# pananananas/MVD

Hardware: AMD Instinct MI355X
Metric: UNet forward-passes/sec @512x512 SD2.1+MV adapter (higher is better)
Workload: dtype bf16; 1 GPU; cfg4: configs[3]/[4]: 8 objects x 4 target views per GPU (32 pairs), camera FiLM + cross-view adapter; pairs_per_gpu=32, global_pairs=32, latent=64x64x4, image=512x512, forward=cold, hip_graph=False, q2_statistics=replica-local, parallelism=dp1 (pairs sharded by object), weights=synthetic seeded, SD2.1 shapes (865.9M UNet x2 + 99.2M adapter + 19.1M camera), encoder_weights=distinct

## Files before the change

### include/mvd_hip.h

```cpp
#ifndef MVD_HIP_H
#define MVD_HIP_H
#include <stddef.h>
#include <stdint.h>

#ifdef __cplusplus
extern "C" {
#endif

#define MVD_MAX_LEVELS 4

typedef struct {
  int in_channels;
  int out_channels;
  int num_levels;
  int block_out_channels[MVD_MAX_LEVELS];
  int num_heads[MVD_MAX_LEVELS];
  int layers_per_block;
  int cross_attention_dim;
  int norm_num_groups;
  float norm_eps;
  int cam_output_dim;
  int cam_hidden_dim;
  int simple_cam_encoder;
  float cam_modulation_strength;
} mvd_config_t;

typedef struct mvd_engine mvd_engine_t;

const char* mvd_last_error(void);

int mvd_engine_create(const mvd_config_t* cfg, mvd_engine_t** out);
int mvd_engine_destroy(mvd_engine_t* e);

int mvd_engine_set_weight(mvd_engine_t* e, int set, const char* slot, const void* ptr, int64_t numel, int dtype);
int mvd_engine_clear_weights(mvd_engine_t* e, int set);

int64_t mvd_engine_workspace_bytes(mvd_engine_t* e, int batch, int height, int width, int text_len, int ref_batch);
int64_t mvd_engine_refcache_bytes(mvd_engine_t* e, int ref_batch, int height, int width, int keep_features);
int mvd_engine_bind_workspace(mvd_engine_t* e, void* ws, int64_t ws_bytes, void* refcache, int64_t refcache_bytes);

enum {
  MVD_USE_CAMERA = 1,
  MVD_USE_IMAGE = 2,
  MVD_REUSE_REF = 4,
  MVD_KEEP_FEATURES = 8
};

typedef struct {
  int batch;
  int height, width;
  int text_len;
  const float* sample;
  const float* timesteps;
  const float* text;
  const float* source_camera;
  const float* target_camera;
  int cam_rows;
  int cam_batch;
  const float* fourier_proj;
  const float* source_latents;
  const float* encoder_text;
  int ref_batch;
  int flags;
  float* out;
} mvd_forward_args_t;

int mvd_unet_forward(mvd_engine_t* e, const mvd_forward_args_t* args, void* stream);

int64_t mvd_engine_reference_pixels(mvd_engine_t* e, int height, int width);
int mvd_engine_reference_encode(mvd_engine_t* e, const mvd_forward_args_t* args, float* local_stats, void* stream);
int mvd_engine_reference_finish(mvd_engine_t* e, const float* mean_k, void* stream);

int mvd_engine_set_graph(mvd_engine_t* e, int enable);

int mvd_engine_share_encoder_weights(mvd_engine_t* e, int enable);

int mvd_engine_set_profiling(mvd_engine_t* e, int enable);
int mvd_engine_profile_summary(mvd_engine_t* e, int cap, int* cls, int* launches, double* ms, double* flops, double* bytes);
int mvd_engine_profile_shapes(mvd_engine_t* e, char* buf_host, int cap);

int mvd_engine_num_features(mvd_engine_t* e);
int mvd_engine_feature_shape(mvd_engine_t* e, int idx, int* channels, int* height, int* width);
int mvd_engine_get_feature(mvd_engine_t* e, int idx, float* out_nchw, void* stream);
int mvd_engine_encode_cameras(mvd_engine_t* e, const float* source_camera, const float* target_camera, int cam_rows,
                              int batch, const float* fourier_proj, float* out_emb, void* stream);
int mvd_engine_apply_modulation(mvd_engine_t* e, const char* name, const float* emb, int batch, const float* x_nchw,
                                int channels, int hw, float* out_nchw, void* stream);
int mvd_engine_get_camera_embedding(mvd_engine_t* e, float* out, void* stream);

int mvd_op_linear(const void* a, const void* a2, int k1, int k2, const void* w, const float* bias, const float* rowvec,
                  int ld_rowvec, int rows_per_batch, const void* res, float alpha, int geglu, void* out, int out_f32,
                  int m, int n, int force_cfg, int splitk, float* splitk_ws ,
                  void* stream);
int mvd_op_ln_linear(const void* x, int k, const void* w_folded, const float* c1, const float* c2, float eps, int geglu,
                     void* out, int m, int n, void* stream);
int mvd_op_linear_xs(const void* x, int ldx, const void* w_packed, int m, int k, int units, int geglu, int ln, float ln_eps,
                     const void* res, int ldres, void* out, int ldo, int csplit, void* stream);
int mvd_op_conv3x3_ws(const void* x, int batch, int h, int w, int c, const void* w_packed, const float* bias, const float* rowvec,
                      int ld_rowvec, const void* res, const void* sc, const void* sc2, int sc_c1, int sc_c2, void* out, int n,
                      int variant, void* stream);
int mvd_op_conv3x3(const void* x, int batch, int in_h, int in_w, int cin, int stride, int upsample, int asym_pad, const void* w,
                   const float* bias, const float* rowvec, int ld_rowvec, const void* res, const void* sc, const void* sc2,
                   int sc_c1, int sc_c2, void* out, int cout, int force_cfg, int splitk, float* splitk_ws, void* stream);
int mvd_op_attention(const void* q, const void* k, const void* v, void* o, int batch, int heads, int nq, int nk, int ldq,
                     int ldk, int ldv, int ldo, float scale, void* stream);
int64_t mvd_op_attention_split_ws_bytes(int batch, int heads, int nq, int nsplit);
int mvd_op_attention_split(const void* q, const void* k, const void* v, void* o, int batch, int heads, int nq, int nk, int ldq,
                           int ldk, int ldv, int ldo, int nsplit, void* ws, void* stream);
int mvd_op_groupnorm(const void* x0, const void* x1, int c0, int c1, int batch, int hw, int groups, float eps,
                     const float* gamma, const float* beta, int silu, void* y, float* ws, void* stream);
int mvd_op_layernorm(const void* x, int rows, int c, float eps, const float* gamma, const float* beta, void* y,
                     void* stream);
int mvd_op_refnorm(const void* x, int batch, int hw, int c, void* y, void* stream);
int mvd_op_film(const void* x, int batch, int hw, int c, const float* scale, const float* shift, void* y, void* stream);
int mvd_op_conv_in(const void* x, int batch, int h, int w, int cin, const float* wt, const float* bias, int cout, void* y,
                   void* stream);
int mvd_op_conv_out(const void* x, int batch, int h, int w, int c, const void* wt, const float* bias, int cout, float* y,
                    void* stream);
int mvd_op_nchw_to_nhwc(const float* x, int batch, int c, int hw, const float* scale, const float* shift, void* y,
                        void* stream);
int mvd_op_nhwc_to_nchw(const void* x, int batch, int hw, int c, float* y, void* stream);
int mvd_op_f32_to_bf16(const float* x, int64_t n, void* y, void* stream);
int mvd_op_skinny_linear(const float* x, int ldx, int batch, int k, const void* w, int wbf16, const float* bias, int n, int act_in,
                         float* y, int ldy, void* stream);
int mvd_gemm_num_configs(void);
int mvd_debug_last_gemm_plan(int* out);
int mvd_debug_last_attention_plan(int* out);
int mvd_debug_last_gemm_nowait(void);
int mvd_debug_pick_splitk(int m, int n, int k, int geglu);
int mvd_debug_pick_splitk_conv(int m, int n, int k);
int mvd_gemm_sm_num_tiles(void);
int mvd_debug_set_attention_nw(int nw_log2);
int mvd_debug_set_flags(int flags);

int mvd_op_ddpm_step(const float* model_out, const float* sample, const float* noise, float c0, float c1, float c2,
                     float c3, float sigma, float* out, int64_t n, void* stream);
int mvd_op_cfg_combine(const float* uncond_cond, float guidance_scale, float* out, int64_t n_half, void* stream);
int mvd_op_sampler_step(const float* model_out, int guided, float guidance_scale, const float* sample, const float* x0_prev,
                        const float* noise, float a0, float a1, float p, float q, float r, float sigma, float* out,
                        float* x0_out, int64_t n, void* stream);

typedef struct {
  int in_channels;
  int latent_channels;
  int num_levels;
  int block_out_channels[MVD_MAX_LEVELS];
  int layers_per_block;
  int norm_num_groups;
  float norm_eps;
} mvd_vae_config_t;
typedef struct mvd_vae mvd_vae_t;
int mvd_vae_create(const mvd_vae_config_t* cfg, mvd_vae_t** out);
int mvd_vae_destroy(mvd_vae_t* v);
int mvd_vae_set_weight(mvd_vae_t* v, const char* slot, const void* ptr, int64_t numel, int dtype);
int64_t mvd_vae_workspace_bytes(mvd_vae_t* v, int batch, int height, int width, int decode);
int mvd_vae_bind_workspace(mvd_vae_t* v, void* ws, int64_t ws_bytes);
int mvd_vae_encode(mvd_vae_t* v, const float* image_nchw, int batch, int height, int width, float* moments, void* stream);
int mvd_vae_decode(mvd_vae_t* v, const float* latents_nchw, int batch, int height, int width, float* image, void* stream);
int64_t mvd_vae_mid_attention_workspace_bytes(mvd_vae_t* v, int decoder, int batch, int height, int width);
int mvd_vae_mid_attention(mvd_vae_t* v, int decoder, const void* x_nhwc_bf16, int batch, int height, int width, void* out_nhwc_bf16,
                          void* stream);
int mvd_op_softmax_rows(const float* s, int rows, int n, void* p_bf16, void* stream);
int mvd_op_gaussian_sample(const float* moments, const float* noise, int batch, int channels, int hw, float scale, float* out,
                           void* stream);

#ifdef __cplusplus
}
#endif
#endif
```

### mvd_amd/_lib.py

```python
from __future__ import annotations

import ctypes as C
import os

HERE = os.path.dirname(os.path.abspath(__file__))
LIB_PATH = os.environ.get("MVD_HIP_LIB") or os.path.join(HERE, "libmvd_hip.so")

MVD_MAX_LEVELS = 4
MVD_USE_CAMERA, MVD_USE_IMAGE, MVD_REUSE_REF, MVD_KEEP_FEATURES = 1, 2, 4, 8


class MvdError(RuntimeError):
    pass


class mvd_config_t(C.Structure):
    _fields_ = [
        ("in_channels", C.c_int), ("out_channels", C.c_int), ("num_levels", C.c_int),
        ("block_out_channels", C.c_int * MVD_MAX_LEVELS), ("num_heads", C.c_int * MVD_MAX_LEVELS),
        ("layers_per_block", C.c_int), ("cross_attention_dim", C.c_int), ("norm_num_groups", C.c_int),
        ("norm_eps", C.c_float), ("cam_output_dim", C.c_int), ("cam_hidden_dim", C.c_int),
        ("simple_cam_encoder", C.c_int), ("cam_modulation_strength", C.c_float),
    ]


class mvd_vae_config_t(C.Structure):
    _fields_ = [
        ("in_channels", C.c_int), ("latent_channels", C.c_int), ("num_levels", C.c_int),
        ("block_out_channels", C.c_int * MVD_MAX_LEVELS), ("layers_per_block", C.c_int), ("norm_num_groups", C.c_int),
        ("norm_eps", C.c_float),
    ]


class mvd_forward_args_t(C.Structure):
    _fields_ = [
        ("batch", C.c_int), ("height", C.c_int), ("width", C.c_int), ("text_len", C.c_int),
        ("sample", C.c_void_p), ("timesteps", C.c_void_p), ("text", C.c_void_p),
        ("source_camera", C.c_void_p), ("target_camera", C.c_void_p), ("cam_rows", C.c_int), ("cam_batch", C.c_int),
        ("fourier_proj", C.c_void_p), ("source_latents", C.c_void_p), ("encoder_text", C.c_void_p),
        ("ref_batch", C.c_int), ("flags", C.c_int), ("out", C.c_void_p),
    ]


_SIGS = {
    "mvd_last_error": (C.c_char_p, []),
    "mvd_engine_create": (C.c_int, [C.POINTER(mvd_config_t), C.POINTER(C.c_void_p)]),
    "mvd_engine_destroy": (C.c_int, [C.c_void_p]),
    "mvd_engine_set_weight": (C.c_int, [C.c_void_p, C.c_int, C.c_char_p, C.c_void_p, C.c_int64, C.c_int]),
    "mvd_engine_clear_weights": (C.c_int, [C.c_void_p, C.c_int]),
    "mvd_engine_workspace_bytes": (C.c_int64, [C.c_void_p, C.c_int, C.c_int, C.c_int, C.c_int, C.c_int]),
    "mvd_engine_refcache_bytes": (C.c_int64, [C.c_void_p, C.c_int, C.c_int, C.c_int, C.c_int]),
    "mvd_engine_bind_workspace": (C.c_int, [C.c_void_p, C.c_void_p, C.c_int64, C.c_void_p, C.c_int64]),
    "mvd_unet_forward": (C.c_int, [C.c_void_p, C.POINTER(mvd_forward_args_t), C.c_void_p]),
    "mvd_engine_set_profiling": (C.c_int, [C.c_void_p, C.c_int]),
    "mvd_engine_profile_summary": (C.c_int, [C.c_void_p, C.c_int, C.POINTER(C.c_int), C.POINTER(C.c_int),
                                             C.POINTER(C.c_double), C.POINTER(C.c_double), C.POINTER(C.c_double)]),
    "mvd_engine_profile_shapes": (C.c_int, [C.c_void_p, C.c_char_p, C.c_int]),
    "mvd_engine_set_graph": (C.c_int, [C.c_void_p, C.c_int]),
    "mvd_engine_reference_pixels": (C.c_int64, [C.c_void_p, C.c_int, C.c_int]),
    "mvd_engine_reference_encode": (C.c_int, [C.c_void_p, C.POINTER(mvd_forward_args_t), C.c_void_p, C.c_void_p]),
    "mvd_engine_reference_finish": (C.c_int, [C.c_void_p, C.c_void_p, C.c_void_p]),
    "mvd_engine_share_encoder_weights": (C.c_int, [C.c_void_p, C.c_int]),
    "mvd_engine_num_features": (C.c_int, [C.c_void_p]),
    "mvd_engine_feature_shape": (C.c_int, [C.c_void_p, C.c_int, C.POINTER(C.c_int), C.POINTER(C.c_int), C.POINTER(C.c_int)]),
    "mvd_engine_get_feature": (C.c_int, [C.c_void_p, C.c_int, C.c_void_p, C.c_void_p]),
    "mvd_engine_encode_cameras": (C.c_int, [C.c_void_p, C.c_void_p, C.c_void_p, C.c_int, C.c_int, C.c_void_p, C.c_void_p, C.c_void_p]),
    "mvd_engine_apply_modulation": (C.c_int, [C.c_void_p, C.c_char_p, C.c_void_p, C.c_int, C.c_void_p, C.c_int, C.c_int, C.c_void_p, C.c_void_p]),
    "mvd_engine_get_camera_embedding": (C.c_int, [C.c_void_p, C.c_void_p, C.c_void_p]),
    "mvd_op_linear": (C.c_int, [C.c_void_p, C.c_void_p, C.c_int, C.c_int, C.c_void_p, C.c_void_p, C.c_void_p, C.c_int,
                                C.c_int, C.c_void_p, C.c_float, C.c_int, C.c_void_p, C.c_int, C.c_int, C.c_int, C.c_int,
                                C.c_int, C.c_void_p, C.c_void_p]),
    "mvd_op_ln_linear": (C.c_int, [C.c_void_p, C.c_int, C.c_void_p, C.c_void_p, C.c_void_p, C.c_float, C.c_int, C.c_void_p,
                                   C.c_int, C.c_int, C.c_void_p]),
    "mvd_op_linear_xs": (C.c_int, [C.c_void_p, C.c_int, C.c_void_p, C.c_int, C.c_int, C.c_int, C.c_int, C.c_int, C.c_float,
                                   C.c_void_p, C.c_int, C.c_void_p, C.c_int, C.c_int, C.c_void_p]),
    "mvd_op_conv3x3_ws": (C.c_int, [C.c_void_p, C.c_int, C.c_int, C.c_int, C.c_int, C.c_void_p, C.c_void_p, C.c_void_p, C.c_int,
                                    C.c_void_p, C.c_void_p, C.c_void_p, C.c_int, C.c_int, C.c_void_p, C.c_int, C.c_int, C.c_void_p]),
    "mvd_op_conv3x3": (C.c_int, [C.c_void_p, C.c_int, C.c_int, C.c_int, C.c_int, C.c_int, C.c_int, C.c_int, C.c_void_p, C.c_void_p,
                                 C.c_void_p, C.c_int, C.c_void_p, C.c_void_p, C.c_void_p, C.c_int, C.c_int, C.c_void_p,
                                 C.c_int, C.c_int, C.c_int, C.c_void_p, C.c_void_p]),
    "mvd_op_attention": (C.c_int, [C.c_void_p, C.c_void_p, C.c_void_p, C.c_void_p, C.c_int, C.c_int, C.c_int, C.c_int,
                                   C.c_int, C.c_int, C.c_int, C.c_int, C.c_float, C.c_void_p]),
    "mvd_op_attention_split_ws_bytes": (C.c_int64, [C.c_int, C.c_int, C.c_int, C.c_int]),
    "mvd_op_attention_split": (C.c_int, [C.c_void_p, C.c_void_p, C.c_void_p, C.c_void_p, C.c_int, C.c_int, C.c_int, C.c_int, C.c_int,
                                         C.c_int, C.c_int, C.c_int, C.c_int, C.c_void_p, C.c_void_p]),
    "mvd_op_groupnorm": (C.c_int, [C.c_void_p, C.c_void_p, C.c_int, C.c_int, C.c_int, C.c_int, C.c_int, C.c_float,
                                   C.c_void_p, C.c_void_p, C.c_int, C.c_void_p, C.c_void_p, C.c_void_p]),
    "mvd_op_layernorm": (C.c_int, [C.c_void_p, C.c_int, C.c_int, C.c_float, C.c_void_p, C.c_void_p, C.c_void_p, C.c_void_p]),
    "mvd_op_refnorm": (C.c_int, [C.c_void_p, C.c_int, C.c_int, C.c_int, C.c_void_p, C.c_void_p]),
    "mvd_op_film": (C.c_int, [C.c_void_p, C.c_int, C.c_int, C.c_int, C.c_void_p, C.c_void_p, C.c_void_p, C.c_void_p]),
    "mvd_op_conv_in": (C.c_int, [C.c_void_p, C.c_int, C.c_int, C.c_int, C.c_int, C.c_void_p, C.c_void_p, C.c_int, C.c_void_p, C.c_void_p]),
    "mvd_op_conv_out": (C.c_int, [C.c_void_p, C.c_int, C.c_int, C.c_int, C.c_int, C.c_void_p, C.c_void_p, C.c_int, C.c_void_p, C.c_void_p]),
    "mvd_op_nchw_to_nhwc": (C.c_int, [C.c_void_p, C.c_int, C.c_int, C.c_int, C.c_void_p, C.c_void_p, C.c_void_p, C.c_void_p]),
    "mvd_op_nhwc_to_nchw": (C.c_int, [C.c_void_p, C.c_int, C.c_int, C.c_int, C.c_void_p, C.c_void_p]),
    "mvd_op_f32_to_bf16": (C.c_int, [C.c_void_p, C.c_int64, C.c_void_p, C.c_void_p]),
    "mvd_op_skinny_linear": (C.c_int, [C.c_void_p, C.c_int, C.c_int, C.c_int, C.c_void_p, C.c_int, C.c_void_p, C.c_int, C.c_int,
                                        C.c_void_p, C.c_int, C.c_void_p]),
    "mvd_gemm_num_configs": (C.c_int, []),
    "mvd_debug_last_gemm_plan": (C.c_int, [C.POINTER(C.c_int)]),
    "mvd_debug_last_gemm_nowait": (C.c_int, []),
    "mvd_debug_last_attention_plan": (C.c_int, [C.POINTER(C.c_int)]),
    "mvd_debug_pick_splitk": (C.c_int, [C.c_int, C.c_int, C.c_int, C.c_int]),
    "mvd_debug_pick_splitk_conv": (C.c_int, [C.c_int, C.c_int, C.c_int]),
    "mvd_gemm_sm_num_tiles": (C.c_int, []),
    "mvd_debug_set_attention_nw": (C.c_int, [C.c_int]),
    "mvd_debug_set_flags": (C.c_int, [C.c_int]),
    "mvd_op_ddpm_step": (C.c_int, [C.c_void_p, C.c_void_p, C.c_void_p, C.c_float, C.c_float, C.c_float, C.c_float,
                                   C.c_float, C.c_void_p, C.c_int64, C.c_void_p]),
    "mvd_op_cfg_combine": (C.c_int, [C.c_void_p, C.c_float, C.c_void_p, C.c_int64, C.c_void_p]),
    "mvd_op_sampler_step": (C.c_int, [C.c_void_p, C.c_int, C.c_float, C.c_void_p, C.c_void_p, C.c_void_p, C.c_float, C.c_float,
                                      C.c_float, C.c_float, C.c_float, C.c_float, C.c_void_p, C.c_void_p, C.c_int64, C.c_void_p]),
    "mvd_vae_create": (C.c_int, [C.POINTER(mvd_vae_config_t), C.POINTER(C.c_void_p)]),
    "mvd_vae_destroy": (C.c_int, [C.c_void_p]),
    "mvd_vae_set_weight": (C.c_int, [C.c_void_p, C.c_char_p, C.c_void_p, C.c_int64, C.c_int]),
    "mvd_vae_workspace_bytes": (C.c_int64, [C.c_void_p, C.c_int, C.c_int, C.c_int, C.c_int]),
    "mvd_vae_bind_workspace": (C.c_int, [C.c_void_p, C.c_void_p, C.c_int64]),
    "mvd_vae_encode": (C.c_int, [C.c_void_p, C.c_void_p, C.c_int, C.c_int, C.c_int, C.c_void_p, C.c_void_p]),
    "mvd_vae_decode": (C.c_int, [C.c_void_p, C.c_void_p, C.c_int, C.c_int, C.c_int, C.c_void_p, C.c_void_p]),
    "mvd_vae_mid_attention_workspace_bytes": (C.c_int64, [C.c_void_p, C.c_int, C.c_int, C.c_int, C.c_int]),
    "mvd_vae_mid_attention": (C.c_int, [C.c_void_p, C.c_int, C.c_void_p, C.c_int, C.c_int, C.c_int, C.c_void_p, C.c_void_p]),
    "mvd_op_softmax_rows": (C.c_int, [C.c_void_p, C.c_int, C.c_int, C.c_void_p, C.c_void_p]),
    "mvd_op_gaussian_sample": (C.c_int, [C.c_void_p, C.c_void_p, C.c_int, C.c_int, C.c_int, C.c_float, C.c_void_p, C.c_void_p]),
}

EXPORTED_SYMBOLS = tuple(_SIGS)

_lib = None


def lib() -> C.CDLL:
    global _lib
    if _lib is None:
        if not os.path.exists(LIB_PATH):
            raise MvdError(
                f"{LIB_PATH} not found: build the HIP extension first "
                "(python -c 'import __graft_entry__ as g; g.build()' or python mvd_amd/_build.py)")
        import torch
        l = C.CDLL(LIB_PATH)
        for name, (res, args) in _SIGS.items():
            fn = getattr(l, name)
            fn.restype = res
            fn.argtypes = args
        _lib = l
    return _lib


def last_error() -> str:
    return lib().mvd_last_error().decode()


def check(rc: int, what: str = "") -> int:
    if rc is None or rc < 0 or (rc != 0 and what.startswith("!")):
        raise MvdError(f"{what.lstrip('!')}: rc={rc}: {last_error()}")
    return rc


def call(name: str, *args):
    rc = getattr(lib(), name)(*args)
    if rc != 0:
        raise MvdError(f"{name} failed (rc={rc}): {last_error()}")
    return rc
```

### mvd_amd/csrc/engine.hip

```cpp
#include <math.h>
#include <stdio.h>
#include <stdlib.h>
#include <string.h>

#include <string>
#include <unordered_map>
#include <vector>

#include "../../include/mvd_hip.h"
#include "kernels.h"

int mvd_launch_silu_to_bf16(const float* x, int64_t n, bf16_t* y, hipStream_t s);

static int g_debug_flags = 0;
extern "C" int mvd_debug_set_flags(int flags) { g_debug_flags = flags; return 0; }
int mvd_debug_flags() { return g_debug_flags; }

namespace {

struct Weight { const void* p; int64_t numel; int dtype; };

struct Arena {
  char* base = nullptr;
  size_t cap = 0, off = 0, high = 0;
// ... 69 lines not shown
  int dual_late_from = MVD_ENV_INT("MVD_DUAL_LATE_FROM", 99);
  bool graph_on = false;
  std::vector<GraphEntry> graphs;
  std::vector<std::string> graph_seen;
  void drop_graphs() {
    for (auto& ge : graphs) { (void)hipGraphExecDestroy(ge.x); (void)hipGraphDestroy(ge.g); }
    graphs.clear(); graph_seen.clear();
  }
  ~mvd_engine() {
    drop_graphs();
    for (hipEvent_t ev : ev_pool) (void)hipEventDestroy(ev);
    for (hipEvent_t ev : feat_ev) if (ev) (void)hipEventDestroy(ev);
    if (fork_ev) (void)hipEventDestroy(fork_ev);
    if (join_ev) (void)hipEventDestroy(join_ev);
    if (side) (void)hipStreamDestroy(side);
  }
  std::vector<int> temb_off;
  int temb_total = 0;
  std::vector<int> tkv_off;
  int tkv_total = 0;
  bool prof = false;
  bool prof_overlap = false;
  struct ProfRec { int cls; double flops; double bytes; hipEvent_t e0, e1; int M, N, K, tag; };
  int prof_M = 0, prof_N = 0, prof_K = 0, prof_tag = 0;
  std::vector<ProfRec> prof_recs;
  std::vector<hipEvent_t> ev_pool; size_t ev_used = 0;
  hipEvent_t get_event() {
    if (ev_used == ev_pool.size()) { hipEvent_t ev = nullptr; (void)hipEventCreate(&ev); ev_pool.push_back(ev); }
    return ev_pool[ev_used++];
  }
};

static inline int gemm_class(const MvdGemmArgs& g, int cfg, int splitk) {
  if (cfg == 8) return 12;
  if (cfg == 7) return splitk > 1 ? 14 : (g.seg[0].mode == MVD_A_CONV3 ? 13 : (g.ln_c1 ? 15 : 7));
  return cfg;
}
int mvd_attention_pick_nw(const MvdAttnArgs& a);

namespace {

#define CHECK(x) do { int _r = (x); if (_r) return _r; } while (0)

#ifdef MVD_PROBE
struct WsCheckRec { std::string slot; int set; bool side; const char* p[4]; size_t n[4]; };
static std::vector<WsCheckRec> g_ws_recs;
static unsigned long long* g_ws_cnt = nullptr;
__global__ void ws_check_kernel(const bf16_t* __restrict__ a, const bf16_t* __restrict__ b, long n, unsigned long long* cnt_l, unsigned long long* cnt, unsigned long long launch) {
  unsigned long long bad = 0;
  for (long i = (long)blockIdx.x * blockDim.x + threadIdx.x; i < n; i += (long)gridDim.x * blockDim.x) {
    const float va = bflo((unsigned)a[i]), vb = bflo((unsigned)b[i]);
    if (!(fabsf(va - vb) <= 0.03f * fabsf(vb) + 0.05f)) {
      ++bad;
      const unsigned long long k = __hip_atomic_fetch_add(cnt + 8192 * 2 - 1, 1ull, __ATOMIC_RELAXED, __HIP_MEMORY_SCOPE_SYSTEM);
      if (k < 4096) { cnt[8192 * 2 + 2 * k] = (unsigned long long)i | (launch << 40); cnt[8192 * 2 + 2 * k + 1] = ((unsigned long long)__float_as_uint(va) << 32) | __float_as_uint(vb); }
    }
  }
  if (bad) __hip_atomic_fetch_add(cnt_l, bad, __ATOMIC_RELAXED, __HIP_MEMORY_SCOPE_SYSTEM);
  if (blockIdx.x == 0 && threadIdx.x == 0) __hip_atomic_fetch_add(cnt_l + 1, (unsigned long long)n, __ATOMIC_RELAXED, __HIP_MEMORY_SCOPE_SYSTEM);
}
extern "C" void mvd_debug_ws_check_report(void);
static const char* g_ws_ptrs[4]; static size_t g_ws_lens[4];
static void ws_check_launch(const std::string& slot, int set, bool side, const bf16_t* a, const bf16_t* b, long n, hipStream_t s) {
  if (!g_ws_cnt) {
    (void)hipHostMalloc(&g_ws_cnt, (8192 * 2 + 8192) * sizeof(unsigned long long), hipHostMallocMapped); memset(g_ws_cnt, 0, (8192 * 2 + 8192) * sizeof(unsigned long long));
    atexit(mvd_debug_ws_check_report);
  }
  if (g_ws_recs.size() >= 4096) return;
  g_ws_recs.push_back({slot, set, side, {g_ws_ptrs[0], g_ws_ptrs[1], g_ws_ptrs[2], g_ws_ptrs[3]}, {g_ws_lens[0], g_ws_lens[1], g_ws_lens[2], g_ws_lens[3]}});
  hipLaunchKernelGGL(ws_check_kernel, dim3(64), dim3(256), 0, s, a, b, n, g_ws_cnt + 2 * (g_ws_recs.size() - 1), g_ws_cnt, (unsigned long long)(g_ws_recs.size() - 1));
}
extern "C" void mvd_debug_ws_check_report(void) {
  (void)hipDeviceSynchronize();
  int nbad = 0;
  for (size_t i = 0; i < g_ws_recs.size(); ++i)
    if (g_ws_cnt[2 * i]) { ++nbad; fprintf(stderr, "ws check: launch %zu %s (set %d, %s stream): %llu of %llu elements beyond tolerance\n", i, g_ws_recs[i].slot.c_str(), g_ws_recs[i].set, g_ws_recs[i].side ? "side" : "main", g_ws_cnt[2 * i], g_ws_cnt[2 * i + 1]); }
  {
    const unsigned long long nlog = g_ws_cnt[8192 * 2 - 1] < 4096 ? g_ws_cnt[8192 * 2 - 1] : 4096;
    std::unordered_map<unsigned long long, int> tiles;
    for (unsigned long long k = 0; k < nlog; ++k) {
      const unsigned long long v = g_ws_cnt[8192 * 2 + 2 * k], launch = v >> 40, idx = v & ((1ull << 40) - 1);
      const int N = 0; (void)N;
      tiles[(launch << 40) | idx] = 1;
    }
    for (unsigned long long k = 0; k < nlog && k < 24; ++k) {
      const unsigned long long v = g_ws_cnt[8192 * 2 + 2 * k], w = g_ws_cnt[8192 * 2 + 2 * k + 1];
      const unsigned ua = (unsigned)(w >> 32), ub = (unsigned)w; float fa, fb; memcpy(&fa, &ua, 4); memcpy(&fb, &ub, 4);
      fprintf(stderr, "ws check: mismatch launch %llu idx %llu: ws %g tiled %g\n", v >> 40, v & ((1ull << 40) - 1), fa, fb);
    }
  }
  static const char* kind[4] = {"x", "sc0", "sc1", "out"};
  int nov = 0;
  for (size_t i = 0; i < g_ws_recs.size() && nov < 12; ++i)
    for (size_t j = i + 1; j < g_ws_recs.size() && j < i + 40 && nov < 12; ++j) {
      if (g_ws_recs[i].side == g_ws_recs[j].side) continue;
      for (int u = 0; u < 4; ++u) for (int v = 0; v < 4; ++v) {
        const char* a0 = g_ws_recs[i].p[u]; const char* b0 = g_ws_recs[j].p[v];
        if (!a0 || !b0 || (u != 3 && v != 3)) continue;
        if (a0 < b0 + g_ws_recs[j].n[v] && b0 < a0 + g_ws_recs[i].n[u]) {
          ++nov; fprintf(stderr, "ws check: OVERLAP launch %zu %s (%s stream) %s [%p, +%zu) with launch %zu %s (%s stream) %s [%p, +%zu)\n", i, g_ws_recs[i].slot.c_str(), g_ws_recs[i].side ? "side" : "main", kind[u], (const void*)a0, g_ws_recs[i].n[u], j, g_ws_recs[j].slot.c_str(), g_ws_recs[j].side ? "side" : "main", kind[v], (const void*)b0, g_ws_recs[j].n[v]);
        }
      }
    }
  fprintf(stderr, "ws check: %d operand overlaps between the two passes\n", nov);
  fprintf(stderr, "ws check: %zu conv_ws launches compared with the tiled kernel, %d with elements beyond tolerance\n", g_ws_recs.size(), nbad);
}
#endif

struct Ctx {
  mvd_engine* e;
  hipStream_t s;
  int set;
  bool dry;
  int err = 0;
  bool nowait = false;

  const Weight* W(const std::string& name, int dtype, int64_t numel, int set_override = -1) {
    if (dry) return nullptr;
    const int st = set_override >= 0 ? set_override : set;
    auto it = e->w[st].find(name);
    if (it == e->w[st].end()) { mvd_set_error("missing weight slot '%s' in set %d", name.c_str(), st); err = -10; return nullptr; }
    if (it->second.dtype != dtype || it->second.numel != numel) {
      mvd_set_error("weight slot '%s' (set %d): expected dtype %d numel %lld, got dtype %d numel %lld", name.c_str(), st, dtype,
                    (long long)numel, it->second.dtype, (long long)it->second.numel);
      err = -11; return nullptr;
    }
    return &it->second;
  }
  const bf16_t* WB(const std::string& n, int64_t numel, int so = -1) { auto* w = W(n, 1, numel, so); return w ? (const bf16_t*)w->p : nullptr; }
  const float* WF(const std::string& n, int64_t numel, int so = -1) { auto* w = W(n, 0, numel, so); return w ? (const float*)w->p : nullptr; }
  bool has(const std::string& n, int so = -1) { const int st = so >= 0 ? so : set; return e->w[st].count(n) != 0; }

  template <class T> T* talloc(size_t n) { return (T*)e->tmp.alloc(n * sizeof(T)); }
  template <class T> T* aalloc(size_t n) { return (T*)e->act.alloc(n * sizeof(T)); }
  Act new_act(int B, int H, int W_, int C, bool longlived) {
    Act a; a.B = B; a.H = H; a.W = W_; a.C = C;
    a.p = longlived ? aalloc<bf16_t>((size_t)B * H * W_ * C) : talloc<bf16_t>((size_t)B * H * W_ * C);
    return a;
  }

  template <class F> int profiled(int cls, double flops, double bytes, F&& launch) {
    if (!e->prof) return launch();
    hipEvent_t e0 = e->get_event(), e1 = e->get_event();
    (void)hipEventRecord(e0, s);
    const int r = launch();
    (void)hipEventRecord(e1, s);
    e->prof_recs.push_back({cls, flops, bytes, e0, e1, e->prof_M, e->prof_N, e->prof_K, e->prof_tag});
    return r;
  }
  static bool sm_enabled() {
    static const bool use_sm = MVD_ENV_INT("MVD_GEMM_SM", 1) != 0;
    return use_sm && !(g_debug_flags & 4);
  }
  int gemm(MvdGemmArgs& g) {
    if (err) return err;
    int sm_tile = 0, sm_ns = 0, sm_S = 1;
    if (sm_enabled() && mvd_gemm_sm_plan(g, &sm_tile, &sm_ns, &sm_S)) {
      if (g_debug_flags & 2) sm_S = 1;
      const size_t mark = e->tmp.off;
      if (sm_S > 1) {
        g.splitk = sm_S; g.splitk_nowait = nowait ? 1 : 0; g.part = talloc<float>((size_t)sm_S * g.M * g.N);
        const int tiles = ((g.M + 63) / 64) * (g.N / 64);
        g.tile_cnt = e->cnt_base + e->cnt_used;
        e->cnt_used += tiles;
        if (!dry && e->cnt_used > e->cnt_cap) { mvd_set_error("forward: split-K tile counters exhausted (%d > %d)", e->cnt_used, e->cnt_cap); return err = -15; }
      }
      int r = 0;
      if (!dry) {
        const double fl = 2.0 * g.M * (double)g.N * g.Ktot;
        e->prof_M = g.M; e->prof_N = g.N; e->prof_K = g.Ktot; e->prof_tag = g.seg[0].mode * 100 + g.geglu * 10 + (sm_S > 1 ? sm_S : 0);
        r = profiled(20 + sm_tile, fl, 0.0, [&] { return mvd_launch_gemm_sm(g, s, sm_tile, sm_ns); });
      }
      e->tmp.off = mark;
      return r;
    }
    int S = mvd_gemm_pick_splitk(g);
    int fc = -1;
    if (e->dual_now && !e->dual_late && !(g_debug_flags & 32) && !g.geglu && !g.ln_c1 && !g.out_f32 && g.N % 320 == 0 && mvd_gemm_pp_applicable(g)) {
      const int cfg = mvd_gemm_pick_config(g);
      const long t7 = (long)((g.M + 255) / 256) * (g.N / 320);
      if (t7 >= 100) { S = 1; if (cfg != 7) fc = 7; }
    }
    const size_t mark = e->tmp.off;
    if (S > 1) { g.splitk = S; g.part = talloc<float>((size_t)S * g.M * g.N); } else g.splitk = 1;
    static const bool trace = MVD_ENV_INT("MVD_TRACE_GEMM", 0) != 0;
    if (trace && !dry) fprintf(stderr, "gemm M=%d N=%d K=%d mode=%d nseg=%d geglu=%d cfg=%d splitk=%d\n", g.M, g.N, g.Ktot, g.seg[0].mode, g.nseg, g.geglu, mvd_gemm_pick_config(g), S);
    int r = 0;
    if (!dry) {
      const double fl = 2.0 * g.M * (double)g.N * g.Ktot;
      e->prof_M = g.M; e->prof_N = g.N; e->prof_K = g.Ktot; e->prof_tag = g.seg[0].mode * 100 + g.geglu * 10 + (S > 1 ? S : 0);
      r = profiled(e->prof ? gemm_class(g, mvd_gemm_pick_config(g), S) : 0, fl, 0.0, [&] { return mvd_launch_gemm(g, s, fc); });
      if (!r && S > 1) r = mvd_launch_splitk_reduce(g, s);
    }
    e->tmp.off = mark;
    return r;
  }

  int try_xs(const bf16_t* x, int K, int M, const std::string& slot, int64_t n_full, int N, bool geglu, bool ln,
             const bf16_t* res, int ldres, void* out, int ldo, int set_override = -1) {
    if (err) return err;
    if (dry || (g_debug_flags & 128) || K != 320 || slot.empty() || !has(slot, set_override)) return 0;
    MvdXsArgs a; memset(&a, 0, sizeof(a));
    a.x = x; a.ldx = K; a.M = M; a.K = K; a.units = N / 32; a.geglu = geglu; a.ln = ln; a.ln_eps = 1e-5f;
    a.res = res; a.ldres = ldres; a.out = (bf16_t*)out; a.ldo = ldo;
    if (N % 64 || !mvd_gemm_xs_applicable(a)) return 0;
    if ((long)((M + 255) / 256) * mvd_gemm_xs_pick_csplit(a) < 448) return 0;
    a.w = WB(slot, (n_full / 32) * 21 * 512, set_override);
    if (!a.w) return err;
    e->prof_M = M; e->prof_N = N; e->prof_K = K; e->prof_tag = geglu * 10 + (ln ? 1 : 0);
    const int r = profiled(geglu ? 33 : (res ? 31 : (ln ? 32 : 30)), 2.0 * M * (double)N * K, 0.0, [&] { return mvd_launch_gemm_xs(a, s); });
    return r ? r : 1;
  }

  int linear(const bf16_t* a, const bf16_t* a2, int k1, int k2, int M, const bf16_t* w, const float* bias, int N,
             const bf16_t* res, int ldres, void* out, int ldo, bool geglu = false, bool out_f32 = false, int ldw = 0,
             const std::string& xs = std::string(), int xs_set = -1) {
    if (!xs.empty() && !a2 && !k2 && !geglu && !out_f32) {
      const int r = try_xs(a, k1, M, xs, N, N, false, false, res, ldres, out, ldo, xs_set);
      if (r) return r < 0 ? r : 0;
    }
    MvdGemmArgs g; memset(&g, 0, sizeof(g));
    g.ldw = ldw ? ldw : k1 + k2;
    g.seg[0].p0 = a; g.seg[0].p1 = a2; g.seg[0].c0 = k1; g.seg[0].c1 = k2; g.seg[0].mode = MVD_A_DENSE; g.seg[0].ksize = k1 + k2;
    g.nseg = 1; g.W = w; g.M = M; g.N = N; g.Ktot = k1 + k2; g.rows_per_batch = M; g.outH = 1; g.outW = M;
    g.bias = bias; g.res = res; g.ldres = ldres; g.alpha = 1.f; g.geglu = geglu; g.out = out; g.ldo = ldo; g.out_f32 = out_f32;
    return gemm(g);
  }

  int ln_linear(const bf16_t* x, int M, int C, const std::string& ln_key, const std::string& slot, int64_t n_full, int N,
                const float* bias, bf16_t* ln_tmp, void* out, int ldo, bool geglu) {
    MvdGemmArgs g; memset(&g, 0, sizeof(g));
    g.ldw = C; g.seg[0].p0 = x; g.seg[0].c0 = C; g.seg[0].mode = MVD_A_DENSE; g.seg[0].ksize = C; g.nseg = 1;
    g.M = M; g.N = N; g.Ktot = C; g.rows_per_batch = M; g.outH = 1; g.outW = M; g.alpha = 1.f; g.geglu = geglu; g.out = out; g.ldo = ldo;
    {
      const int r = try_xs(x, C, M, slot + ".wx", n_full, N, geglu, true, nullptr, 0, out, ldo);
      if (r) return r < 0 ? r : 0;
    }
    static const bool use_fold = MVD_ENV_INT("MVD_LN_FOLD", 1) != 0;
    auto sm_fold_ok = [&]() {
      MvdGemmArgs t = g;
      static const float dummy = 0.f;
      t.ln_c1 = &dummy; t.bias = &dummy; t.W = reinterpret_cast<const bf16_t*>(&dummy);
      int a_, b_, c_;
      return sm_enabled() && !(g_debug_flags & 1) && mvd_gemm_sm_plan(t, &a_, &b_, &c_);
    };
    if (use_fold && !dry && has(slot + ".wf") && has(slot + ".cf") && (mvd_gemm_ln_fold_ok(g) || sm_fold_ok())) {
      const float* cf = WF(slot + ".cf", 2 * n_full);
      g.W = WB(slot + ".wf", n_full * C);
      g.ln_c1 = cf; g.bias = cf ? cf + n_full : nullptr; g.ln_eps = 1e-5f;
      return gemm(g);
    }
    CHECK(layernorm(x, M, C, WF(ln_key + ".g", C), WF(ln_key + ".b", C), ln_tmp));
    g.seg[0].p0 = ln_tmp; g.W = WB(slot + ".w", n_full * C); g.bias = bias;
    return gemm(g);
  }

  int try_ws(const Act& x, int ups, const std::string& slot, const float* bias, const float* rowvec, int ld_rowvec, const bf16_t* res,
             const bf16_t* sc0, const bf16_t* sc1, int scc0, int scc1, Act& out) {
    if (err) return err;
    if (dry || (g_debug_flags & 256) || slot.empty() || !has(slot)) return 0;
    MvdWsArgs a; memset(&a, 0, sizeof(a));
    a.x = x.p; a.B = x.B; a.H = x.H; a.W = x.W; a.C = x.C; a.ups = ups; a.sc0 = sc0; a.sc1 = sc1; a.scc0 = scc0; a.scc1 = scc1;
    a.bias = bias; a.rowvec = rowvec; a.ld_rowvec = ld_rowvec; a.res = res; a.ldres = out.C; a.out = out.p; a.ldo = out.C;
    a.M = out.rows(); a.N = out.C;
    if ((g_debug_flags & 512) && a.M > 256) return 0;
    if (g_debug_flags & 1024) a.variant = 1;
    if ((g_debug_flags & 2048) && scc0) return 0;
    if ((g_debug_flags & 4096) && nowait) return 0;
    if ((g_debug_flags & 8192) && !nowait) return 0;
    if (out.H != (ups ? 2 : 1) * x.H || out.W != (ups ? 2 : 1) * x.W || out.B != x.B || a.M > 1024) return 0;
    if ((long)(a.M / 64) * (a.N / 16) > 1000) return 0;
    a.w = reinterpret_cast<const bf16_t*>(&a);
    if (!mvd_conv_ws_applicable(a)) return 0;
    a.w = WB(slot, (int64_t)mvd_conv_ws_packed_elems(x.C, scc0 + scc1, out.C));
    if (!a.w) return err;
    e->prof_M = a.M; e->prof_N = a.N; e->prof_K = 9 * x.C + scc0 + scc1; e->prof_tag = 100 + (scc0 ? 1 : 0);
    const int r = profiled(34, 2.0 * a.M * (double)a.N * (9.0 * x.C + scc0 + scc1), 0.0, [&] { return mvd_launch_conv_ws(a, s); });
    if (!r && (g_debug_flags & 16384)) return 0;
#ifdef MVD_PROBE
    if (!r && (g_debug_flags & 32768)) {
      const size_t mark = e->tmp.off;
      Act chk = new_act(out.B, out.H, out.W, out.C, false);
      const bf16_t* wold = WB(slot.substr(0, slot.size() - 1), (int64_t)out.C * (9 * x.C + scc0 + scc1));
      if (wold) {
        const int saved = g_debug_flags; g_debug_flags |= 256;
        conv3(x, 1, ups, wold, bias, rowvec, ld_rowvec, res, sc0, sc1, scc0, scc1, chk);
        g_debug_flags = saved;
        g_ws_ptrs[0] = (const char*)x.p; g_ws_lens[0] = (size_t)x.rows() * x.C * 2;
        g_ws_ptrs[1] = (const char*)sc0; g_ws_lens[1] = (size_t)out.rows() * scc0 * 2;
        g_ws_ptrs[2] = (const char*)sc1; g_ws_lens[2] = (size_t)out.rows() * scc1 * 2;
        g_ws_ptrs[3] = (const char*)out.p; g_ws_lens[3] = (size_t)out.rows() * out.C * 2;
        ws_check_launch(slot, set, nowait, out.p, chk.p, (long)out.rows() * out.C, s);
      }
      e->tmp.off = mark;
    }
#endif
    return r ? r : 1;
  }

  int conv3(const Act& x, int stride, int ups, const bf16_t* w, const float* bias, const float* rowvec, int ld_rowvec,
            const bf16_t* res, const bf16_t* sc0, const bf16_t* sc1, int scc0, int scc1, Act& out, const std::string& ws = std::string()) {
    if (!ws.empty() && stride == 1) {
      const int r = try_ws(x, ups, ws, bias, rowvec, ld_rowvec, res, sc0, sc1, scc0, scc1, out);
      if (r) return r < 0 ? r : 0;
    }
    MvdGemmArgs g; memset(&g, 0, sizeof(g));
    g.seg[0].p0 = x.p; g.seg[0].c0 = x.C; g.seg[0].mode = MVD_A_CONV3; g.seg[0].ksize = 9 * x.C;
    g.seg[0].inH = x.H; g.seg[0].inW = x.W; g.seg[0].stride = stride; g.seg[0].ups = ups;
    g.nseg = 1; g.Ktot = 9 * x.C;
    if (sc0) {
      g.seg[1].p0 = sc0; g.seg[1].p1 = sc1; g.seg[1].c0 = scc0; g.seg[1].c1 = scc1; g.seg[1].mode = MVD_A_DENSE;
      g.seg[1].ksize = scc0 + scc1; g.nseg = 2; g.Ktot += scc0 + scc1;
    }
    g.W = w; g.ldw = g.Ktot; g.M = out.rows(); g.N = out.C; g.rows_per_batch = out.hw(); g.outH = out.H; g.outW = out.W;
    g.bias = bias; g.rowvec = rowvec; g.ld_rowvec = ld_rowvec; g.res = res; g.ldres = out.C; g.alpha = 1.f;
    g.out = out.p; g.ldo = out.C;
    return gemm(g);
  }

  int groupnorm(const bf16_t* x0, const bf16_t* x1, int c0, int c1, int B, int hw, float eps, const float* g, const float* b,
                int silu, bf16_t* y) {
    if (err) return err;
    const int groups = e->cfg.norm_num_groups;
    float* ws = talloc<float>((size_t)B * MVD_GN_MAXCHUNK * groups * 2);
    if (dry) return 0;
    const double by = 3.0 * B * (double)hw * (c0 + c1) * 2;
    e->prof_M = B * hw; e->prof_N = c0 + c1; e->prof_K = 0; e->prof_tag = 2000 + silu;
    return profiled(16, 0.0, by, [&] { return mvd_launch_groupnorm(x0, x1, c0, c1, B, hw, groups, eps, g, b, silu, y, ws, s); });
  }
  int layernorm(const bf16_t* x, int rows, int c, const float* g, const float* b, bf16_t* y) {
    if (err) return err; if (dry) return 0;
    e->prof_M = rows; e->prof_N = c; e->prof_K = 0; e->prof_tag = 3000;
    return profiled(17, 0.0, 2.0 * rows * (double)c * 2, [&] { return mvd_launch_layernorm(x, rows, c, 1e-5f, g, b, y, s); });
  }
  int attention(MvdAttnArgs& a) {
    if (err) return err;
    const size_t mark = e->tmp.off;
    const int ns = (g_debug_flags & 8) ? 1 : mvd_attention_pick_split(a);
    if (ns > 1) {
      a.nsplit = ns;
      a.split_ws = e->tmp.alloc(mvd_attention_split_ws_bytes(a, ns));
      a.split_cnt = e->cnt_base + e->cnt_used;
      e->cnt_used += mvd_attention_split_counters(a);
      if (!dry && e->cnt_used > e->cnt_cap) { mvd_set_error("forward: tile counters exhausted (%d > %d)", e->cnt_used, e->cnt_cap); return err = -15; }
    }
    e->tmp.off = mark;
    if (dry) return 0;
    double fl = 0;
    for (int i = 0; i < a.nprob; ++i) fl += 4.0 * a.batch * a.heads * (double)a.p[i].nq * a.p[i].nk * 64;
    e->prof_M = a.p[0].nq; e->prof_N = a.p[0].nk; e->prof_K = a.heads; e->prof_tag = 1000 + a.nprob;
    return profiled(e->prof ? 8 + mvd_attention_pick_nw(a) : 8, fl, 0.0, [&] { return mvd_launch_attention(a, s); });
  }
};

struct ResnetDesc { std::string key; int cin0, cin1, cout; };

std::vector<ResnetDesc> enumerate_resnets(const mvd_config_t& c) {
  std::vector<ResnetDesc> v;
  const int n = c.num_levels, L = c.layers_per_block;
  int prev = c.block_out_channels[0];
  for (int i = 0; i < n; ++i) {
    const int co = c.block_out_channels[i];
    for (int j = 0; j < L; ++j) v.push_back({"down_blocks." + std::to_string(i) + ".resnets." + std::to_string(j), j == 0 ? prev : co, 0, co});
    prev = co;
  }
  const int cm = c.block_out_channels[n - 1];
  v.push_back({"mid_block.resnets.0", cm, 0, cm});
  v.push_back({"mid_block.resnets.1", cm, 0, cm});
  int prev_out = cm;
  for (int i = 0; i < n; ++i) {
    const int out_c = c.block_out_channels[n - 1 - i];
    const int in_c = c.block_out_channels[n - 1 - (i + 1 < n ? i + 1 : n - 1)];
    for (int j = 0; j <= L; ++j) {
      const int skip = (j == L) ? in_c : out_c;
      const int hid = (j == 0) ? prev_out : out_c;
      v.push_back({"up_blocks." + std::to_string(i) + ".resnets." + std::to_string(j), hid, skip, out_c});
    }
    prev_out = out_c;
  }
  return v;
}

std::vector<FeatureInfo> enumerate_features(const mvd_config_t& c) {
  std::vector<FeatureInfo> f;
  const int n = c.num_levels, L = c.layers_per_block;
  for (int i = 0; i + 1 < n; ++i)
    for (int j = 0; j < L; ++j) f.push_back({"down_block_" + std::to_string(i) + "_attn_" + std::to_string(j), i, c.block_out_channels[i], c.num_heads[i],
                   "down_blocks." + std::to_string(i) + ".attentions." + std::to_string(j)});
  f.push_back({"mid_block_attn_0", n - 1, c.block_out_channels[n - 1], c.num_heads[n - 1], "mid_block.attentions.0"});
  for (int i = 1; i < n; ++i)
    for (int j = 0; j <= L; ++j) f.push_back({"up_block_" + std::to_string(i) + "_attn_" + std::to_string(j), n - 1 - i, c.block_out_channels[n - 1 - i], c.num_heads[n - 1 - i],
                   "up_blocks." + std::to_string(i) + ".attentions." + std::to_string(j)});
  return f;
}

struct PassOpts {
  bool adapter = false;
  bool film = false;
  bool capture = false;
  bool defer_norm = false;
  float* stats = nullptr;
  int ref_batch = 0;
  const std::unordered_map<std::string, std::pair<float*, float*>>* film_ss = nullptr;
};

struct UNetPass {
  Ctx& c;
  const mvd_config_t& cfg;
  PassOpts o;
  int B, H0, W0, L;
  const bf16_t* text;
  const float* tproj;
  bf16_t* tkv = nullptr;
  int resnet_idx = 0;
  int feat_idx = 0;

  int resnet(const std::string& key, const Act& x0, const Act* x1, int cout, Act& out) {
    const int cin0 = x0.C, cin1 = x1 ? x1->C : 0, cin = cin0 + cin1;
    const int B_ = x0.B, hw = x0.hw();
    const size_t mark = c.e->tmp.off;
    Act t1 = c.new_act(B_, x0.H, x0.W, cin, false);
    CHECK(c.groupnorm(x0.p, x1 ? x1->p : nullptr, cin0, cin1, B_, hw, cfg.norm_eps, c.WF(key + ".norm1.g", cin), c.WF(key + ".norm1.b", cin), 1, t1.p));
    Act h1 = c.new_act(B_, x0.H, x0.W, cout, false);
    const int toff = c.e->temb_off[resnet_idx++];
    CHECK(c.conv3(t1, 1, 0, c.WB(key + ".conv1.w", (int64_t)cout * 9 * cin), c.WF(key + ".conv1.b", cout), tproj + toff, c.e->temb_total,
                  nullptr, nullptr, nullptr, 0, 0, h1, key + ".conv1.ws"));
    Act t2 = c.new_act(B_, x0.H, x0.W, cout, false);
    CHECK(c.groupnorm(h1.p, nullptr, cout, 0, B_, hw, cfg.norm_eps, c.WF(key + ".norm2.g", cout), c.WF(key + ".norm2.b", cout), 1, t2.p));
    if (cin != cout) {
      CHECK(c.conv3(t2, 1, 0, c.WB(key + ".conv2.w", (int64_t)cout * (9 * cout + cin)), c.WF(key + ".conv2.b", cout), nullptr, 0, nullptr,
                    x0.p, x1 ? x1->p : nullptr, cin0, cin1, out, key + ".conv2.ws"));
    } else {
      CHECK(c.conv3(t2, 1, 0, c.WB(key + ".conv2.w", (int64_t)cout * 9 * cout), c.WF(key + ".conv2.b", cout), nullptr, 0, x0.p, nullptr,
                    nullptr, 0, 0, out, key + ".conv2.ws"));
    }
    c.e->tmp.off = mark;
    return c.err;
  }

  int transformer(const std::string& key, const Act& x, int heads, Act& out) {
    const int C = x.C, M = x.rows(), hw = x.hw(), B_ = x.B;
    const FeatureInfo& fi = c.e->feats[feat_idx];
    const bool ad = o.adapter;
    const bool packed = c.set == 0 && (c.dry || c.has(key + ".ref_kv.w", 0));
    if (ad && !packed) { mvd_set_error("adapter requested but no adapter weights registered for %s", key.c_str()); return -14; }
    const int ld_out = packed ? 2 * C : C;
    const char* bias_slot = (packed && !ad) ? ".out.b0" : ".out.b";
    const size_t mark = c.e->tmp.off;
    bf16_t* n0 = c.talloc<bf16_t>((size_t)M * C);
    CHECK(c.groupnorm(x.p, nullptr, C, 0, B_, hw, 1e-6f, c.WF(key + ".norm.g", C), c.WF(key + ".norm.b", C), 0, n0));
    bf16_t* h = c.talloc<bf16_t>((size_t)M * C);
    CHECK(c.linear(n0, nullptr, C, 0, M, c.WB(key + ".proj_in.w", (int64_t)C * C), c.WF(key + ".proj_in.b", C), C, nullptr, 0, h, C, false, false, 0, key + ".proj_in.wx"));
    bf16_t* ln = n0;
    const float scale = 0.125f;
    bf16_t* o_self = c.talloc<bf16_t>((size_t)M * C);
    bf16_t* o_ref = ad ? c.talloc<bf16_t>((size_t)M * C) : nullptr;
    const bf16_t* rkv = ad ? c.e->refkv[feat_idx] : nullptr;
    const int ref_nk = ad ? (int)((int64_t)o.ref_batch * hw / B_) : 0;
    if (ad && (int64_t)ref_nk * B_ != (int64_t)o.ref_batch * hw) { mvd_set_error("adapter: ref tokens %d x %d not divisible by batch %d", o.ref_batch, hw, B_); return -12; }

    if (ad && c.e->dual_now && !c.dry && !c.err && hipStreamWaitEvent(c.s, c.e->feat_ev[feat_idx], 0) != hipSuccess) { mvd_set_error("forward: hipStreamWaitEvent failed"); return -3; }
    {
      const int nq = ad ? 4 * C : 3 * C;
      bf16_t* qkv = c.talloc<bf16_t>((size_t)M * nq);
      CHECK(c.ln_linear(h, M, C, key + ".ln1", key + ".attn1.qkv", (int64_t)(packed ? 4 : 3) * C, nq, nullptr, ln, qkv, nq, false));
      MvdAttnArgs a; memset(&a, 0, sizeof(a));
      a.batch = B_; a.heads = heads; a.scale = scale; a.prescaled = 1; a.nprob = ad ? 2 : 1;
      a.p[0] = {qkv, qkv + C, qkv + 2 * C, o_self, nq, nq, nq, C, (int64_t)hw * nq, (int64_t)hw * nq, (int64_t)hw * nq, (int64_t)hw * C, hw, hw};
      if (ad) a.p[1] = {qkv + 3 * C, rkv, rkv + C, o_ref, nq, 4 * C, 4 * C, C, (int64_t)hw * nq, (int64_t)ref_nk * 4 * C, (int64_t)ref_nk * 4 * C, (int64_t)hw * C, hw, ref_nk};
      CHECK(c.attention(a));
      const int kout = ad ? 2 * C : C;
      (void)kout;
      CHECK(c.linear(o_self, o_ref, C, ad ? C : 0, M, c.WB(key + ".attn1.out.w", (int64_t)C * ld_out), c.WF(key + ".attn1" + bias_slot, C), C, h, C, h, C, false, false, ld_out,
                     ad ? std::string() : key + ".attn1.out.wx"));
    }
    {
      const int nq = ad ? 2 * C : C;
      bf16_t* q2 = c.talloc<bf16_t>((size_t)M * nq);
      const bf16_t* kv2 = tkv + c.e->tkv_off[feat_idx];
      const int ldkv = c.e->tkv_total;
      CHECK(c.ln_linear(h, M, C, key + ".ln2", key + ".attn2.q", (int64_t)(packed ? 2 : 1) * C, nq, nullptr, ln, q2, nq, false));
      MvdAttnArgs a; memset(&a, 0, sizeof(a));
      a.batch = B_; a.heads = heads; a.scale = scale; a.prescaled = 1; a.nprob = ad ? 2 : 1;
      a.p[0] = {q2, kv2, kv2 + C, o_self, nq, ldkv, ldkv, C, (int64_t)hw * nq, (int64_t)L * ldkv, (int64_t)L * ldkv, (int64_t)hw * C, hw, L};
      if (ad) a.p[1] = {q2 + C, rkv + 2 * C, rkv + 3 * C, o_ref, nq, 4 * C, 4 * C, C, (int64_t)hw * nq, (int64_t)ref_nk * 4 * C, (int64_t)ref_nk * 4 * C, (int64_t)hw * C, hw, ref_nk};
      CHECK(c.attention(a));
      const int kout = ad ? 2 * C : C;
      (void)kout;
      CHECK(c.linear(o_self, o_ref, C, ad ? C : 0, M, c.WB(key + ".attn2.out.w", (int64_t)C * ld_out), c.WF(key + ".attn2" + bias_slot, C), C, h, C, h, C, false, false, ld_out,
                     ad ? std::string() : key + ".attn2.out.wx"));
    }
    {
      bf16_t* ff = c.talloc<bf16_t>((size_t)M * 4 * C);
      CHECK(c.ln_linear(h, M, C, key + ".ln3", key + ".ff1", (int64_t)8 * C, 8 * C, c.WF(key + ".ff1.b", 8 * C), ln, ff, 4 * C, true));
      CHECK(c.linear(ff, nullptr, 4 * C, 0, M, c.WB(key + ".ff2.w", (int64_t)C * 4 * C), c.WF(key + ".ff2.b", C), C, h, C, h, C));
    }
    CHECK(c.linear(h, nullptr, C, 0, M, c.WB(key + ".proj_out.w", (int64_t)C * C), c.WF(key + ".proj_out.b", C), C, x.p, C, out.p, C, false, false, 0, key + ".proj_out.wx"));
    c.e->tmp.off = mark;

    if (o.capture) {
      const size_t mk = c.e->tmp.off;
      bf16_t* rn = c.talloc<bf16_t>((size_t)M * C);
      if (o.defer_norm) {
        if (!c.dry && !c.err) CHECK(mvd_launch_refstats(out.p, B_, hw, C, o.stats + 2 * c.e->feat_pixel_off(feat_idx), c.s));
      } else {
        if (!c.dry && !c.err) CHECK(mvd_launch_refnorm(out.p, B_, hw, C, rn, c.s));
        CHECK(c.linear(rn, nullptr, C, 0, M, c.WB(key + ".ref_kv.w", (int64_t)4 * C * C, 0), nullptr, 4 * C, nullptr, 0, c.e->refkv[feat_idx], 4 * C, false, false, 0,
                       key + ".ref_kv.wx", 0));
        if (c.e->dual_now && !c.dry && !c.err && hipEventRecord(c.e->feat_ev[feat_idx], c.s) != hipSuccess) { mvd_set_error("forward: hipEventRecord failed"); return -3; }
      }
      if (c.e->rc_keep && !c.dry && !c.err)
        CHECK((int)hipMemcpyAsync(c.e->feat_keep[feat_idx], out.p, (size_t)M * C * sizeof(bf16_t), hipMemcpyDeviceToDevice, c.s));
      c.e->tmp.off = mk;
    }
    (void)fi;
    ++feat_idx;
    return c.err;
  }

  int film(const std::string& name, const Act& x, Act& out) {
    auto it = o.film_ss->find(name);
    if (it == o.film_ss->end()) { out = x; return 0; }
    if (c.dry || c.err) return c.err;
    return mvd_launch_film(x.p, x.B, x.hw(), x.C, it->second.first, it->second.second, x.C, out.p, c.s);
  }

  int run(const Act& x_in, float* out_nchw) {
    const int n = cfg.num_levels, Lb = cfg.layers_per_block;
    const int C0 = cfg.block_out_channels[0];
    std::vector<Act> skips;
    tkv = c.aalloc<bf16_t>((size_t)B * L * c.e->tkv_total);
    CHECK(c.linear(text, nullptr, cfg.cross_attention_dim, 0, B * L, c.WB("text_kv.w", (int64_t)c.e->tkv_total * cfg.cross_attention_dim), nullptr,
                   c.e->tkv_total, nullptr, 0, tkv, c.e->tkv_total));
    Act h = c.new_act(B, H0, W0, C0, true);
    CHECK(c.linear(x_in.p, nullptr, 64, 0, B * H0 * W0, c.WB("conv_in.w", (int64_t)C0 * 64), c.WF("conv_in.b", C0), C0, nullptr, 0, h.p, C0));
    skips.push_back(h);
    for (int i = 0; i < n; ++i) {
      const int co = cfg.block_out_channels[i];
      const std::string bk = "down_blocks." + std::to_string(i);
      for (int j = 0; j < Lb; ++j) {
        Act r = c.new_act(B, h.H, h.W, co, true);
        CHECK(resnet(bk + ".resnets." + std::to_string(j), h, nullptr, co, r));
        h = r;
        if (i + 1 < n) {
          Act t = c.new_act(B, h.H, h.W, co, true);
          CHECK(transformer(bk + ".attentions." + std::to_string(j), h, cfg.num_heads[i], t));
          h = t;
        }
        skips.push_back(h);
      }
      if (i + 1 < n) {
        Act d = c.new_act(B, (h.H + 1) / 2, (h.W + 1) / 2, co, true);
        CHECK(c.conv3(h, 2, 0, c.WB(bk + ".down.w", (int64_t)co * 9 * co), c.WF(bk + ".down.b", co), nullptr, 0, nullptr, nullptr, nullptr, 0, 0, d));
        h = d;
        skips.push_back(h);
      }
      if (o.film) {
        Act m = c.new_act(B, h.H, h.W, h.C, true);
        Act res = m;
        CHECK(film("down_" + std::to_string(i), h, res));
        h = res;
      }
    }
    {
      const int cm = cfg.block_out_channels[n - 1];
      Act r = c.new_act(B, h.H, h.W, cm, true);
      CHECK(resnet("mid_block.resnets.0", h, nullptr, cm, r));
      Act t = c.new_act(B, h.H, h.W, cm, true);
      CHECK(transformer("mid_block.attentions.0", r, cfg.num_heads[n - 1], t));
      Act r2 = c.new_act(B, h.H, h.W, cm, true);
      CHECK(resnet("mid_block.resnets.1", t, nullptr, cm, r2));
      h = r2;
      if (o.film) { Act res = h; CHECK(film("mid_0", h, res)); h = res; }
    }
    for (int i = 0; i < n; ++i) {
      const int co = cfg.block_out_channels[n - 1 - i];
      const std::string bk = "up_blocks." + std::to_string(i);
      if (!o.capture && i >= c.e->dual_late_from) c.e->dual_late = true;
      for (int j = 0; j <= Lb; ++j) {
        Act skip = skips.back(); skips.pop_back();
        if (skip.H != h.H || skip.W != h.W) { mvd_set_error("up block %d: skip %dx%d vs hidden %dx%d (odd latent size unsupported)", i, skip.H, skip.W, h.H, h.W); return -13; }
        Act r = c.new_act(B, h.H, h.W, co, true);
        CHECK(resnet(bk + ".resnets." + std::to_string(j), h, &skip, co, r));
        h = r;
        if (i > 0) {
          Act t = c.new_act(B, h.H, h.W, co, true);
          CHECK(transformer(bk + ".attentions." + std::to_string(j), h, cfg.num_heads[n - 1 - i], t));
          h = t;
        }
      }
      if (i + 1 < n) {
        Act u = c.new_act(B, h.H * 2, h.W * 2, co, true);
        CHECK(c.conv3(h, 1, 1, c.WB(bk + ".up.w", (int64_t)co * 9 * co), c.WF(bk + ".up.b", co), nullptr, 0, nullptr, nullptr, nullptr, 0, 0, u, bk + ".up.ws"));
        h = u;
      }
      if (o.film) { Act res = h; CHECK(film("up_" + std::to_string(i), h, res)); h = res; }
    }
    if (out_nchw) {
      Act t = c.new_act(B, h.H, h.W, C0, false);
      CHECK(c.groupnorm(h.p, nullptr, C0, 0, B, h.hw(), cfg.norm_eps, c.WF("conv_norm_out.g", C0), c.WF("conv_norm_out.b", C0), 1, t.p));
      const bf16_t* wo = c.WB("conv_out.w", (int64_t)cfg.out_channels * 9 * C0);
      const float* bo = c.WF("conv_out.b", cfg.out_channels);
      if (!c.dry && !c.err) CHECK(mvd_launch_conv_out(t.p, B, h.H, h.W, C0, wo, bo, cfg.out_channels, out_nchw, c.s));
    }
    return c.err;
  }
};

int time_path(Ctx& c, const float* timesteps, int B, const float** tproj_out) {
  const mvd_config_t& cfg = c.e->cfg;
  const int C0 = cfg.block_out_channels[0], TD = 4 * C0;
  float* sinus = c.talloc<float>((size_t)B * C0);
  float* t1 = c.talloc<float>((size_t)B * TD);
  float* emb = c.talloc<float>((size_t)B * TD);
  bf16_t* act = c.talloc<bf16_t>((size_t)B * TD);
  float* tproj = c.aalloc<float>((size_t)B * c.e->temb_total);
  const bf16_t* w1 = c.WB("time.l1.w", (int64_t)TD * C0);
  const float* b1 = c.WF("time.l1.b", TD);
  const bf16_t* w2 = c.WB("time.l2.w", (int64_t)TD * TD);
  const float* b2 = c.WF("time.l2.b", TD);
  const bf16_t* wp = c.WB("temb_proj.w", (int64_t)c.e->temb_total * TD);
  const float* bp = c.WF("temb_proj.b", c.e->temb_total);
  *tproj_out = tproj;
  if (c.err) return c.err;
  if (c.dry) return 0;
  CHECK(mvd_launch_timestep_embedding(timesteps, B, C0, sinus, c.s));
  CHECK(mvd_launch_skinny_linear(sinus, C0, B, C0, w1, 1, b1, TD, 0, t1, TD, c.s));
  CHECK(mvd_launch_skinny_linear(t1, TD, B, TD, w2, 1, b2, TD, 1, emb, TD, c.s));
  CHECK(mvd_launch_silu_to_bf16(emb, (int64_t)B * TD, act, c.s));
  CHECK(c.linear(act, nullptr, TD, 0, B, wp, bp, c.e->temb_total, nullptr, 0, tproj, c.e->temb_total, false, true));
  return 0;
}

int camera_embed(Ctx& c, const float* src, const float* tgt, int cam_rows, const float* proj, int B, float* emb) {
  const mvd_config_t& cfg = c.e->cfg;
  const int D = cfg.cam_output_dim, Hd = cfg.cam_hidden_dim;
  const int nfreq = (D / 2) / 3, encd = 6 * nfreq;
  const bool simple = cfg.simple_cam_encoder != 0;
  float* rflat = c.talloc<float>((size_t)B * 9);
  float* enc = c.talloc<float>((size_t)B * encd);
  float* encp = c.talloc<float>((size_t)B * D);
  float* cat = c.talloc<float>((size_t)B * 2 * D);
  float* bufa = c.talloc<float>((size_t)B * (D > Hd ? D : Hd));
  float* bufb = c.talloc<float>((size_t)B * (D > Hd ? D : Hd));
  auto lin = [&](const std::string& k, const float* x, int ldx, int kin, int nout, float* y, int ldy) -> int {
    const float* w = c.WF("cam." + k + ".weight", (int64_t)nout * kin, 0);
    const float* b = c.WF("cam." + k + ".bias", nout, 0);
    if (c.err) return c.err; if (c.dry) return 0;
    return mvd_launch_skinny_linear(x, ldx, B, kin, w, 0, b, nout, 0, y, ldy, c.s);
  };
  auto lnorm = [&](const std::string& k, const float* x, int n, int silu, float* y) -> int {
    const float* g = c.WF("cam." + k + ".weight", n, 0);
    const float* b = c.WF("cam." + k + ".bias", n, 0);
    if (c.err) return c.err; if (c.dry) return 0;
    return mvd_launch_layernorm_f32(x, B, n, 1e-5f, g, b, silu, y, c.s);
  };
  if (!c.dry && !c.err) {
    CHECK(mvd_launch_camera_features(src, tgt, B, cam_rows, nfreq, 10.0f, rflat, enc, c.s));
    CHECK(mvd_launch_skinny_linear(enc, encd, B, encd, proj, 0, nullptr, D, 0, encp, D, c.s));
  }
  const char* encs[2] = {"rotation_encoder", "translation_encoder"};
  for (int t = 0; t < 2; ++t) {
    const std::string p = encs[t];
    const float* x = t == 0 ? rflat : encp;
    const int kin = t == 0 ? 9 : D;
    CHECK(lin(p + ".0", x, kin, kin, Hd, bufa, Hd));
    CHECK(lnorm(p + ".1", bufa, Hd, 1, bufb));
    if (simple) {
      CHECK(lin(p + ".3", bufb, Hd, Hd, D, cat + t * D, 2 * D));
    } else {
      CHECK(lin(p + ".3", bufb, Hd, Hd, Hd, bufa, Hd));
      CHECK(lnorm(p + ".4", bufa, Hd, 1, bufb));
      CHECK(lin(p + ".6", bufb, Hd, Hd, D, cat + t * D, 2 * D));
    }
  }
  CHECK(lin("final_projection.0", cat, 2 * D, 2 * D, D, bufa, D));
  CHECK(lnorm("final_projection.1", bufa, D, 1, bufb));
  CHECK(lin("final_projection.3", bufb, D, D, D, bufa, D));
  CHECK(lnorm("final_projection.4", bufa, D, 0, bufb));
  CHECK(lnorm("output_norm", bufb, D, 0, emb));
  return c.err;
}

int modulator(Ctx& c, const std::string& name, int dim, const float* emb, int B, float* sc, float* sh, int out_rows = 0) {
  const mvd_config_t& cfg = c.e->cfg;
  const int D = cfg.cam_output_dim;
  float* mh = c.talloc<float>((size_t)B * (D / 2));
  float* mh2 = c.talloc<float>((size_t)B * (D / 2));
  float* raw = c.talloc<float>((size_t)B * 2 * dim);
  const std::string k = "cam.modulators." + name;
  const float* w0 = c.WF(k + ".0.weight", (int64_t)(D / 2) * D, 0);
  const float* b0 = c.WF(k + ".0.bias", D / 2, 0);
  const float* g1 = c.WF(k + ".1.weight", D / 2, 0);
  const float* b1 = c.WF(k + ".1.bias", D / 2, 0);
  const float* w3 = c.WF(k + ".3.weight", (int64_t)2 * dim * (D / 2), 0);
  const float* b3 = c.WF(k + ".3.bias", 2 * dim, 0);
  if (c.err) return c.err;
  if (c.dry) return 0;
  CHECK(mvd_launch_skinny_linear(emb, D, B, D, w0, 0, b0, D / 2, 0, mh, D / 2, c.s));
  CHECK(mvd_launch_layernorm_f32(mh, B, D / 2, 1e-5f, g1, b1, 1, mh2, c.s));
  CHECK(mvd_launch_skinny_linear(mh2, D / 2, B, D / 2, w3, 0, b3, 2 * dim, 0, raw, 2 * dim, c.s));
  return mvd_launch_film_params(raw, B, dim, cfg.cam_modulation_strength, sc, sh, out_rows > B ? out_rows : B, c.s);
}

std::vector<std::pair<std::string, int>> modulator_dims(const mvd_config_t& cfg, bool include_mid) {
  std::vector<std::pair<std::string, int>> mods;
  for (int i = 0; i < cfg.num_levels; ++i) mods.push_back({"down_" + std::to_string(i), cfg.block_out_channels[i]});
  for (int i = 0; i < cfg.num_levels; ++i) mods.push_back({"up_" + std::to_string(i), cfg.block_out_channels[cfg.num_levels - 1 - i]});
  if (include_mid) mods.push_back({"mid", cfg.block_out_channels[cfg.num_levels - 1]});
  mods.push_back({"output", 4});
  return mods;
}

int camera_path(Ctx& c, const mvd_forward_args_t& a, std::unordered_map<std::string, std::pair<float*, float*>>& ss) {
  const mvd_config_t& cfg = c.e->cfg;
  const int B = a.batch, D = cfg.cam_output_dim;
  const int Bc = a.cam_batch > 0 ? a.cam_batch : B;
  float* emb = c.aalloc<float>((size_t)Bc * D);
  c.e->cam_emb = emb; c.e->cam_batch = Bc;
  CHECK(camera_embed(c, a.source_camera, a.target_camera, a.cam_rows, a.fourier_proj, Bc, emb));
  const auto mods = modulator_dims(cfg, false);
  if ((c.dry || c.has("cam.modcat.w0", 0)) && mods.size() <= 16) {
    const int nm = (int)mods.size(), Hh = D / 2;
    MvdSegTable seg; memset(&seg, 0, sizeof(seg));
    seg.n = nm;
    int tot = 0;
    for (int i = 0; i < nm; ++i) { tot += 2 * mods[i].second; seg.end[i] = tot; }
    float* ssbuf = c.aalloc<float>((size_t)B * tot);
    const size_t mk = c.e->tmp.off;
    float* h1 = c.talloc<float>((size_t)Bc * nm * Hh);
    float* h2 = c.talloc<float>((size_t)Bc * nm * Hh);
    float* raw = c.talloc<float>((size_t)Bc * tot);
    const float* w0 = c.WF("cam.modcat.w0", (int64_t)nm * Hh * D, 0);
    const float* b0 = c.WF("cam.modcat.b0", (int64_t)nm * Hh, 0);
    const float* g1 = c.WF("cam.modcat.g1", (int64_t)nm * Hh, 0);
    const float* be1 = c.WF("cam.modcat.be1", (int64_t)nm * Hh, 0);
    const float* w3 = c.WF("cam.modcat.w3", (int64_t)tot * Hh, 0);
    const float* b3 = c.WF("cam.modcat.b3", tot, 0);
    if (!c.dry && !c.err) {
      CHECK(mvd_launch_skinny_linear(emb, D, Bc, D, w0, 0, b0, nm * Hh, 0, h1, nm * Hh, c.s));
      CHECK(mvd_launch_layernorm_f32(h1, Bc * nm, Hh, 1e-5f, g1, be1, 1, h2, c.s, nm));
      CHECK(mvd_launch_skinny_linear_grouped(h2, nm * Hh, Hh, Bc, Hh, w3, b3, tot, seg, raw, tot, c.s));
      CHECK(mvd_launch_film_params_grouped(raw, Bc, seg, cfg.cam_modulation_strength, ssbuf, B, c.s));
    }
    c.e->tmp.off = mk;
    int c0 = 0;
// ... 405 lines not shown
  for (auto& r : e->prof_recs) {
    if (hipEventSynchronize(r.e1) != hipSuccess) { mvd_set_error("profile_shapes: event sync failed"); return -2; }
    float t = 0.f; (void)hipEventElapsedTime(&t, r.e0, r.e1);
    size_t j = 0;
    while (j < v.size() && !(v[j].cls == r.cls && v[j].M == r.M && v[j].N == r.N && v[j].K == r.K && v[j].tag == r.tag)) ++j;
    if (j == v.size()) v.push_back({r.cls, r.M, r.N, r.K, r.tag, 0, 0.0, 0.0});
    v[j].n++; v[j].ms += t; v[j].fl += r.flops;
  }
  int off = 0;
  for (auto& x : v) {
    const int w = snprintf(buf + off, (size_t)(cap - off), "cls=%d M=%d N=%d K=%d tag=%d launches=%d ms=%.3f tflops=%.0f\n", x.cls, x.M, x.N, x.K,
                           x.tag, x.n, x.ms, x.ms > 0 ? x.fl / x.ms / 1e9 : 0.0);
    if (w < 0 || off + w >= cap) break;
    off += w;
  }
  return off;
}

int mvd_engine_share_encoder_weights(mvd_engine_t* e, int enable) {
  if (e) e->drop_graphs();
  if (!e) { mvd_set_error("share_encoder_weights: null engine"); return -1; }
  e->share_encoder = enable != 0;
  return 0;
}

int mvd_engine_num_features(mvd_engine_t* e) { return e ? (int)e->feats.size() : -1; }
int mvd_engine_feature_shape(mvd_engine_t* e, int idx, int* channels, int* height, int* width) {
  if (!e || idx < 0 || idx >= (int)e->feats.size() || !e->rc_h) { mvd_set_error("feature_shape: bad index or no reference pass yet"); return -1; }
  *channels = e->feats[idx].C; *height = e->rc_h >> e->feats[idx].level; *width = e->rc_w >> e->feats[idx].level;
  return 0;
}
int mvd_engine_get_feature(mvd_engine_t* e, int idx, float* out_nchw, void* stream) {
  if (!e || idx < 0 || idx >= (int)e->feats.size() || !out_nchw) { mvd_set_error("get_feature: bad argument"); return -1; }
  if (!e->rc_valid || !e->rc_keep || !e->feat_keep[idx]) { mvd_set_error("get_feature: no kept features (run forward with MVD_KEEP_FEATURES)"); return -1; }
  const int lv = e->feats[idx].level;
  return mvd_launch_nhwc_to_nchw_f32(e->feat_keep[idx], e->rc_batch, (e->rc_h >> lv) * (e->rc_w >> lv), e->feats[idx].C, out_nchw, (hipStream_t)stream);
}
int mvd_engine_encode_cameras(mvd_engine_t* e, const float* source_camera, const float* target_camera, int cam_rows,
                              int batch, const float* fourier_proj, float* out_emb, void* stream) {
  if (!e || !source_camera || !target_camera || !fourier_proj || !out_emb || batch <= 0 || (cam_rows != 3 && cam_rows != 4)) { mvd_set_error("encode_cameras: bad argument"); return -1; }
  if (!e->ws_ptr) { mvd_set_error("encode_cameras: workspace not bound"); return -1; }
  {
    e->tmp.dry = true; e->tmp.off = e->tmp.high = 0;
    Ctx d{e, nullptr, 0, true};
    if (int r = camera_embed(d, source_camera, target_camera, cam_rows, fourier_proj, batch, out_emb)) return r;
    if (e->tmp.high > (size_t)e->ws_bytes) { mvd_set_error("encode_cameras: workspace too small (%zu > %lld bytes)", e->tmp.high, (long long)e->ws_bytes); return -4; }
  }
  e->tmp.dry = false; e->tmp.base = (char*)e->ws_ptr; e->tmp.cap = (size_t)e->ws_bytes; e->tmp.off = e->tmp.high = 0;
  Ctx c{e, (hipStream_t)stream, 0, false};
  return camera_embed(c, source_camera, target_camera, cam_rows, fourier_proj, batch, out_emb);
}

int mvd_engine_apply_modulation(mvd_engine_t* e, const char* name, const float* emb, int batch, const float* x_nchw,
                                int channels, int hw, float* out_nchw, void* stream) {
  if (!e || !name || !emb || !x_nchw || !out_nchw || batch <= 0 || channels <= 0 || hw <= 0) { mvd_set_error("apply_modulation: bad argument"); return -1; }
  if (!e->ws_ptr) { mvd_set_error("apply_modulation: workspace not bound"); return -1; }
  int dim = -1;
  for (auto& m : modulator_dims(e->cfg, true)) if (m.first == name) dim = m.second;
  if (dim < 0) return 1;
  if (dim != channels) { mvd_set_error("apply_modulation: modulator '%s' has %d channels, tensor has %d", name, dim, channels); return -1; }
  {
    e->tmp.dry = true; e->tmp.off = e->tmp.high = 0;
    Ctx d{e, nullptr, 0, true};
    float* sc0 = d.talloc<float>((size_t)batch * dim);
    float* sh0 = d.talloc<float>((size_t)batch * dim);
    if (int r = modulator(d, name, dim, emb, batch, sc0, sh0)) return r;
    if (e->tmp.high > (size_t)e->ws_bytes) { mvd_set_error("apply_modulation: workspace too small (%zu > %lld bytes)", e->tmp.high, (long long)e->ws_bytes); return -4; }
  }
  e->tmp.dry = false; e->tmp.base = (char*)e->ws_ptr; e->tmp.cap = (size_t)e->ws_bytes; e->tmp.off = e->tmp.high = 0;
  Ctx c{e, (hipStream_t)stream, 0, false};
  float* sc = c.talloc<float>((size_t)batch * dim);
  float* sh = c.talloc<float>((size_t)batch * dim);
  if (int r = modulator(c, name, dim, emb, batch, sc, sh)) return r;
  return mvd_launch_film_nchw_f32(x_nchw, batch, channels, hw, sc, sh, out_nchw, (hipStream_t)stream);
}

int mvd_engine_get_camera_embedding(mvd_engine_t* e, float* out, void* stream) {
  if (!e || !out || !e->cam_emb) { mvd_set_error("get_camera_embedding: no camera pass yet"); return -1; }
  return (int)hipMemcpyAsync(out, e->cam_emb, (size_t)e->cam_batch * e->cfg.cam_output_dim * sizeof(float), hipMemcpyDeviceToDevice, (hipStream_t)stream);
}

static int op_sm_splitk(MvdGemmArgs& g, hipStream_t s, int force_cfg) {
  g.tile_cnt = reinterpret_cast<unsigned int*>(g.part + (size_t)g.splitk * g.M * g.N);
  hipError_t e = hipMemsetAsync(g.tile_cnt, 0, MVD_OP_SPLITK_COUNTERS * sizeof(unsigned int), s);
  if (e != hipSuccess) { mvd_set_error("op split-K: hipMemsetAsync: %s", hipGetErrorString(e)); return -3; }
  if ((long)((g.M + 63) / 64) * (g.N / 64) > MVD_OP_SPLITK_COUNTERS) { mvd_set_error("op split-K: more than %d output tiles", MVD_OP_SPLITK_COUNTERS); return -1; }
  return mvd_launch_gemm(g, s, force_cfg);
}
int mvd_op_linear(const void* a, const void* a2, int k1, int k2, const void* w, const float* bias, const float* rowvec,
                  int ld_rowvec, int rows_per_batch, const void* res, float alpha, int geglu, void* out, int out_f32, int m,
                  int n, int force_cfg, int splitk, float* splitk_ws, void* stream) {
  MvdGemmArgs g; memset(&g, 0, sizeof(g));
  g.seg[0].p0 = (const bf16_t*)a; g.seg[0].p1 = (const bf16_t*)a2; g.seg[0].c0 = k1; g.seg[0].c1 = k2;
  g.seg[0].mode = MVD_A_DENSE; g.seg[0].ksize = k1 + k2; g.nseg = 1;
  g.W = (const bf16_t*)w; g.M = m; g.N = n; g.Ktot = k1 + k2; g.ldw = k1 + k2;
  g.rows_per_batch = rows_per_batch > 0 ? rows_per_batch : m; g.outH = 1; g.outW = g.rows_per_batch;
  g.bias = bias; g.rowvec = rowvec; g.ld_rowvec = ld_rowvec; g.res = (const bf16_t*)res;
  const int on = geglu ? n / 2 : n;
  g.ldres = on; g.alpha = alpha; g.geglu = geglu; g.out = out; g.ldo = on; g.out_f32 = out_f32;
  g.part = splitk_ws;
  if (splitk > 1) {
    g.splitk = splitk; g.part = splitk_ws;
    if (force_cfg >= 100) return op_sm_splitk(g, (hipStream_t)stream, force_cfg);
    if (int r = mvd_launch_gemm(g, (hipStream_t)stream, force_cfg)) return r;
    return mvd_launch_splitk_reduce(g, (hipStream_t)stream);
  }
  g.splitk = 1;
  return mvd_launch_gemm(g, (hipStream_t)stream, force_cfg);
}

int mvd_op_ln_linear(const void* x, int k, const void* w_folded, const float* c1, const float* c2, float eps, int geglu,
                     void* out, int m, int n, void* stream) {
  MvdGemmArgs g; memset(&g, 0, sizeof(g));
  g.seg[0].p0 = (const bf16_t*)x; g.seg[0].c0 = k; g.seg[0].mode = MVD_A_DENSE; g.seg[0].ksize = k; g.nseg = 1;
  g.W = (const bf16_t*)w_folded; g.M = m; g.N = n; g.Ktot = k; g.ldw = k; g.rows_per_batch = m; g.outH = 1; g.outW = m;
  g.bias = c2; g.ln_c1 = c1; g.ln_eps = eps; g.alpha = 1.f; g.geglu = geglu; g.out = out; g.ldo = geglu ? n / 2 : n; g.ldres = g.ldo;
  if (!c1 || !c2) { mvd_set_error("mvd_op_ln_linear: c1 and c2 are required"); return -1; }
  if (!mvd_gemm_ln_fold_ok(g)) {
    int tile = 0, ns = 0, S = 1;
    if (mvd_gemm_sm_plan(g, &tile, &ns, &S) && S == 1) return mvd_launch_gemm_sm(g, (hipStream_t)stream, tile, ns);
    mvd_set_error("mvd_op_ln_linear: M=%d N=%d K=%d geglu=%d is not a shape of the fused LayerNorm GEMMs", m, n, k, geglu);
    return -1;
  }
  return mvd_launch_gemm(g, (hipStream_t)stream);
}

int mvd_op_conv3x3(const void* x, int batch, int in_h, int in_w, int cin, int stride, int upsample, int asym_pad, const void* w,
                   const float* bias, const float* rowvec, int ld_rowvec, const void* res, const void* sc, const void* sc2,
                   int sc_c1, int sc_c2, void* out, int cout, int force_cfg, int splitk, float* splitk_ws, void* stream) {
  MvdGemmArgs g; memset(&g, 0, sizeof(g));
  const int oh = upsample ? in_h * 2 : (stride == 2 ? (in_h + 1) / 2 : in_h);
  const int ow = upsample ? in_w * 2 : (stride == 2 ? (in_w + 1) / 2 : in_w);
  g.seg[0].p0 = (const bf16_t*)x; g.seg[0].c0 = cin; g.seg[0].mode = MVD_A_CONV3; g.seg[0].ksize = 9 * cin;
  g.seg[0].inH = in_h; g.seg[0].inW = in_w; g.seg[0].stride = stride; g.seg[0].ups = upsample; g.seg[0].asym = asym_pad;
  g.nseg = 1; g.Ktot = 9 * cin;
  if (sc) {
    g.seg[1].p0 = (const bf16_t*)sc; g.seg[1].p1 = (const bf16_t*)sc2; g.seg[1].c0 = sc_c1; g.seg[1].c1 = sc_c2;
    g.seg[1].mode = MVD_A_DENSE; g.seg[1].ksize = sc_c1 + sc_c2; g.nseg = 2; g.Ktot += sc_c1 + sc_c2;
  }
  g.W = (const bf16_t*)w; g.ldw = g.Ktot; g.M = batch * oh * ow; g.N = cout; g.rows_per_batch = oh * ow; g.outH = oh; g.outW = ow;
  g.bias = bias; g.rowvec = rowvec; g.ld_rowvec = ld_rowvec; g.res = (const bf16_t*)res; g.ldres = cout; g.alpha = 1.f;
  g.out = out; g.ldo = cout;
  g.part = splitk_ws;
  if (splitk > 1) {
    g.splitk = splitk; g.part = splitk_ws;
    if (force_cfg >= 100) return op_sm_splitk(g, (hipStream_t)stream, force_cfg);
    if (int r = mvd_launch_gemm(g, (hipStream_t)stream, force_cfg)) return r;
    return mvd_launch_splitk_reduce(g, (hipStream_t)stream);
  }
  g.splitk = 1;
  return mvd_launch_gemm(g, (hipStream_t)stream, force_cfg);
}

int mvd_op_attention(const void* q, const void* k, const void* v, void* o, int batch, int heads, int nq, int nk, int ldq,
                     int ldk, int ldv, int ldo, float scale, void* stream) {
  MvdAttnArgs a; memset(&a, 0, sizeof(a));
  a.nprob = 1; a.batch = batch; a.heads = heads; a.scale = scale;
  a.prescaled = scale == 0.f;
  a.p[0] = {(const bf16_t*)q, (const bf16_t*)k, (const bf16_t*)v, (bf16_t*)o, ldq, ldk, ldv, ldo,
            (int64_t)nq * ldq, (int64_t)nk * ldk, (int64_t)nk * ldv, (int64_t)nq * ldo, nq, nk};
  return mvd_launch_attention(a, (hipStream_t)stream);
}

int64_t mvd_op_attention_split_ws_bytes(int batch, int heads, int nq, int nsplit) {
  MvdAttnArgs a; memset(&a, 0, sizeof(a));
  a.nprob = 1; a.batch = batch; a.heads = heads; a.p[0].nq = nq;
  return (int64_t)mvd_attention_split_ws_bytes(a, nsplit) + (int64_t)mvd_attention_split_counters(a) * 4 + 256;
}
int mvd_op_attention_split(const void* q, const void* k, const void* v, void* o, int batch, int heads, int nq, int nk, int ldq,
                           int ldk, int ldv, int ldo, int nsplit, void* ws, void* stream) {
  MvdAttnArgs a; memset(&a, 0, sizeof(a));
  a.nprob = 1; a.batch = batch; a.heads = heads; a.scale = 0.f; a.prescaled = 1;
  a.p[0] = {(const bf16_t*)q, (const bf16_t*)k, (const bf16_t*)v, (bf16_t*)o, ldq, ldk, ldv, ldo,
            (int64_t)nq * ldq, (int64_t)nk * ldk, (int64_t)nk * ldv, (int64_t)nq * ldo, nq, nk};
  if (nsplit > 1) {
    if (!ws) { mvd_set_error("op_attention_split: null workspace"); return -1; }
    const size_t pb = (mvd_attention_split_ws_bytes(a, nsplit) + 255) & ~size_t(255);
    a.nsplit = nsplit; a.split_ws = ws; a.split_cnt = reinterpret_cast<unsigned int*>(reinterpret_cast<char*>(ws) + pb);
    if (hipMemsetAsync(a.split_cnt, 0, (size_t)mvd_attention_split_counters(a) * 4, (hipStream_t)stream) != hipSuccess) { mvd_set_error("op_attention_split: hipMemsetAsync failed"); return -3; }
  }
  return mvd_launch_attention(a, (hipStream_t)stream);
}

int mvd_op_groupnorm(const void* x0, const void* x1, int c0, int c1, int batch, int hw, int groups, float eps,
                     const float* gamma, const float* beta, int silu, void* y, float* ws, void* stream) {
  return mvd_launch_groupnorm((const bf16_t*)x0, (const bf16_t*)x1, c0, c1, batch, hw, groups, eps, gamma, beta, silu, (bf16_t*)y, ws, (hipStream_t)stream);
}
int mvd_op_layernorm(const void* x, int rows, int c, float eps, const float* gamma, const float* beta, void* y, void* stream) {
  return mvd_launch_layernorm((const bf16_t*)x, rows, c, eps, gamma, beta, (bf16_t*)y, (hipStream_t)stream);
}
int mvd_op_refnorm(const void* x, int batch, int hw, int c, void* y, void* stream) {
  return mvd_launch_refnorm((const bf16_t*)x, batch, hw, c, (bf16_t*)y, (hipStream_t)stream);
}
int mvd_op_film(const void* x, int batch, int hw, int c, const float* scale, const float* shift, void* y, void* stream) {
  return mvd_launch_film((const bf16_t*)x, batch, hw, c, scale, shift, c, (bf16_t*)y, (hipStream_t)stream);
}
int mvd_op_conv_in(const void* x, int batch, int h, int w, int cin, const float* wt, const float* bias, int cout, void* y, void* stream) {
  return mvd_launch_conv_in((const bf16_t*)x, batch, h, w, cin, wt, bias, cout, (bf16_t*)y, (hipStream_t)stream);
}
int mvd_op_conv_out(const void* x, int batch, int h, int w, int c, const void* wt, const float* bias, int cout, float* y, void* stream) {
  return mvd_launch_conv_out((const bf16_t*)x, batch, h, w, c, (const bf16_t*)wt, bias, cout, y, (hipStream_t)stream);
}
int mvd_op_nchw_to_nhwc(const float* x, int batch, int c, int hw, const float* scale, const float* shift, void* y, void* stream) {
  return mvd_launch_nchw_to_nhwc(x, batch, c, hw, scale, shift, c, (bf16_t*)y, (hipStream_t)stream);
}
int mvd_op_nhwc_to_nchw(const void* x, int batch, int hw, int c, float* y, void* stream) {
  return mvd_launch_nhwc_to_nchw_f32((const bf16_t*)x, batch, hw, c, y, (hipStream_t)stream);
}
int mvd_op_f32_to_bf16(const float* x, int64_t n, void* y, void* stream) {
  return mvd_launch_f32_to_bf16(x, n, (bf16_t*)y, (hipStream_t)stream);
}
int mvd_op_skinny_linear(const float* x, int ldx, int batch, int k, const void* w, int wbf16, const float* bias, int n, int act_in,
                         float* y, int ldy, void* stream) {
  return mvd_launch_skinny_linear(x, ldx, batch, k, w, wbf16, bias, n, act_in, y, ldy, (hipStream_t)stream);
}

}
```

### mvd_amd/csrc/gemm.hip

```cpp
#include <stdlib.h>
#include <string.h>
#include "kernels.h"

thread_local MvdLaunchPlan g_mvd_last_gemm = {-1, 1, 0, 0, 0, 0};

namespace {

template <int BM_, int BN_, int WM_, int WN_>
struct Cfg {
  static constexpr int BM = BM_, BN = BN_, WM = WM_, WN = WN_;
  static constexpr int NT = 64 * WM * WN;
  static constexpr int WTM = BM / WM, WTN = BN / WN;
  static constexpr int TM = WTM / 16, TN = WTN / 16;
  static constexpr int A_CHUNKS = BM * 8, B_CHUNKS = BN * 8;
  static constexpr int A_IT = (A_CHUNKS + NT - 1) / NT;
  static constexpr int B_IT = (B_CHUNKS + NT - 1) / NT;
  static constexpr int ROWS_PER_IT = NT / 8;
  static constexpr int A_BYTES = BM * 128, B_BYTES = BN * 128;
  static constexpr int STAGE_BYTES = A_BYTES + B_BYTES;
  static constexpr int LDS_BYTES = 2 * STAGE_BYTES;
  static constexpr int WG_PER_CU = (160 * 1024 / LDS_BYTES) > 4 ? 4 : (160 * 1024 / LDS_BYTES);
  static constexpr int MIN_WAVES = (WG_PER_CU * NT / 256) < 1 ? 1 : (WG_PER_CU * NT / 256 > 4 ? 4 : WG_PER_CU * NT / 256);
  static_assert(WTM % 16 == 0 && WTN % 16 == 0, "wave tile must be a multiple of the MFMA tile");
  static_assert(A_CHUNKS % NT == 0, "A slab must divide evenly over the threads");
// ... 331 lines not shown
            if (q + 1 < 2 * NP) { n0 = w_at(q + 1, 0); n1 = w_at(q + 1, 1); }
            __builtin_amdgcn_sched_barrier(0);
            __builtin_amdgcn_s_setprio(1);
#pragma unroll
            for (int i = 0; i < C::TM; ++i) acc[i][j] = __builtin_amdgcn_mfma_f32_16x16x32_bf16(w0, af[i], acc[i][j], 0, 0, 0);
#pragma unroll
            for (int i = 0; i < C::TM; ++i) {
              acc[i][j + 1] = __builtin_amdgcn_mfma_f32_16x16x32_bf16(w1, af[i], acc[i][j + 1], 0, 0, 0);
              if (q == NP - 1)
                af[i] = *reinterpret_cast<const bf16x8*>(sa + swz_off(wm * C::WTM + i * 16 + fr, 4 + fq));
            }
            __builtin_amdgcn_s_setprio(0);
            __builtin_amdgcn_sched_barrier(0);
            w0 = n0; w1 = n1;
          }
          continue;
        }
        bf16x8 af[C::TM], wf[C::TN];
#pragma unroll
        for (int i = 0; i < C::TM; ++i)
          af[i] = *reinterpret_cast<const bf16x8*>(sa + swz_off(wm * C::WTM + i * 16 + fr, s2 * 4 + fq));
#pragma unroll
        for (int j = 0; j < C::TN; ++j)
          wf[j] = *reinterpret_cast<const bf16x8*>(sb + swz_off(wn * C::WTN + j * 16 + fr, s2 * 4 + fq));
        if (!(DBG && (a.dbg & 2))) {
#pragma unroll
          for (int i = 0; i < C::TM; ++i)
#pragma unroll
            for (int j = 0; j < C::TN; ++j)
              acc[i][j] = __builtin_amdgcn_mfma_f32_16x16x32_bf16(wf[j], af[i], acc[i][j], 0, 0, 0);
        } else {
#pragma unroll
          for (int i = 0; i < C::TM; ++i) asm volatile("" :: "v"(af[i]));
#pragma unroll
          for (int j = 0; j < C::TN; ++j) asm volatile("" :: "v"(wf[j]));
        }
      }
      if (last_k) {
        epilogue(m0, n0, ks);
        if (have_next) {
          const int tn = S == 1 ? next_tile : next_tile / S;
          init_acc((tn / ntn) * C::BM, (tn % ntn) * C::BN);
        }
      }
      if (more) commit_slab(cur ^ 1);
      __syncthreads();
      cur ^= 1;
    }
    if (!have_next) break;
    tile = next_tile; kt0 = nkt0; kt1 = nkt1;
  }
}

__global__ __launch_bounds__(256) void splitk_reduce_kernel(const MvdGemmArgs a) {
  const long nvec = (long)a.M * (a.N >> 2);
  const int nv = a.N >> 2;
  for (long e = (long)blockIdx.x * blockDim.x + threadIdx.x; e < nvec; e += (long)gridDim.x * blockDim.x) {
    const int m = (int)(e / nv), n = (int)(e - (long)m * nv) * 4;
    f32x4 v = *reinterpret_cast<const f32x4*>(a.part + (size_t)m * a.N + n);
    for (int s = 1; s < a.splitk; ++s) v += *reinterpret_cast<const f32x4*>(a.part + ((size_t)s * a.M + m) * a.N + n);
    if (a.bias) v += *reinterpret_cast<const f32x4*>(a.bias + n);
    if (a.rowvec) v += *reinterpret_cast<const f32x4*>(a.rowvec + (size_t)(m / a.rows_per_batch) * a.ld_rowvec + n);
    v *= a.alpha;
    if (a.res) {
      const u32x2 r = *reinterpret_cast<const u32x2*>(a.res + (size_t)m * a.ldres + n);
      v[0] += bflo(r[0]); v[1] += bfhi(r[0]); v[2] += bflo(r[1]); v[3] += bfhi(r[1]);
    }
    if (a.out_f32) {
      *reinterpret_cast<f32x4*>(reinterpret_cast<float*>(a.out) + (size_t)m * a.ldo + n) = v;
    } else {
      u32x2 o = {pack2bf(v[0], v[1]), pack2bf(v[2], v[3])};
      *reinterpret_cast<u32x2*>(reinterpret_cast<bf16_t*>(a.out) + (size_t)m * a.ldo + n) = o;
    }
  }
}

struct CfgInfo { int bm, bn, tn_even; };

template <class C, int AMODE, bool GLDS, bool SPLITK, bool DBG>
int launch_mode3(const MvdGemmArgs& a, hipStream_t s) {
  static int per_cu = 0;
  if (!per_cu) {
    hipError_t e = hipFuncSetAttribute(reinterpret_cast<const void*>(&gemm_kernel<C, AMODE, GLDS, SPLITK, DBG>),
                                       hipFuncAttributeMaxDynamicSharedMemorySize, C::LDS_BYTES);
    if (e != hipSuccess) { mvd_set_error("gemm: hipFuncSetAttribute: %s", hipGetErrorString(e)); return -2; }
    int nb = 0;
    e = hipOccupancyMaxActiveBlocksPerMultiprocessor(&nb, gemm_kernel<C, AMODE, GLDS, SPLITK, DBG>, C::NT, C::LDS_BYTES);
    if (e != hipSuccess || nb < 1) nb = 1;
    per_cu = nb > 4 ? 4 : nb;
  }
  const int ntm = (a.M + C::BM - 1) / C::BM, ntn = a.N / C::BN;
  int grid = 256 * per_cu;
  const int ntiles = ntm * ntn * (a.splitk > 1 ? a.splitk : 1);
  if (ntiles < grid) grid = ((ntiles + 7) / 8) * 8;
  g_mvd_last_gemm.tiles = ntiles; g_mvd_last_gemm.grid = grid; g_mvd_last_gemm.per_cu = per_cu;
  hipLaunchKernelGGL((gemm_kernel<C, AMODE, GLDS, SPLITK, DBG>), dim3(grid), dim3(C::NT), C::LDS_BYTES, s, a);
  hipError_t e = hipGetLastError();
  if (e != hipSuccess) { mvd_set_error("gemm launch: %s", hipGetErrorString(e)); return -3; }
  return 0;
}

template <class C, int AMODE, bool GLDS, bool SPLITK>
int launch_mode2(const MvdGemmArgs& a, hipStream_t s) {
#ifdef MVD_PROBE
  if (a.dbg) return launch_mode3<C, AMODE, GLDS, SPLITK, true>(a, s);
#endif
  return launch_mode3<C, AMODE, GLDS, SPLITK, false>(a, s);
}

template <class C, int AMODE, bool GLDS>
int launch_mode(const MvdGemmArgs& a, hipStream_t s) {
  if constexpr (GLDS) { if (a.splitk > 1) return launch_mode2<C, AMODE, true, true>(a, s); }
  return launch_mode2<C, AMODE, GLDS, false>(a, s);
}

template <class C, bool DMA_ONLY = false>
int launch_cfg(const MvdGemmArgs& a, hipStream_t s, bool glds) {
  if (a.splitk > 1) glds = true;
  if (glds || DMA_ONLY) {
    if (a.seg[0].mode == MVD_A_DENSE) return launch_mode<C, 0, true>(a, s);
    return a.nseg == 1 ? launch_mode<C, 1, true>(a, s) : launch_mode<C, 2, true>(a, s);
  }
  if constexpr (!DMA_ONLY) {
    if (a.seg[0].mode == MVD_A_DENSE) return launch_mode<C, 0, false>(a, s);
    return a.nseg == 1 ? launch_mode<C, 1, false>(a, s) : launch_mode<C, 2, false>(a, s);
  }
  return -1;
}

using C0 = Cfg<256, 160, 4, 2>;
using C1 = Cfg<256, 128, 4, 2>;
using C2 = Cfg<128, 160, 2, 2>;
using C3 = Cfg<128, 128, 2, 2>;
using C4 = Cfg<128, 64, 2, 2>;
using C5 = Cfg<64, 64, 2, 2>;
using C7 = Cfg<256, 320, 2, 4>;
using C6 = Cfg<256, 320, 4, 2>;
using C8 = Cfg<128, 320, 2, 4>;
const CfgInfo kCfgs[] = {{256, 160, 0}, {256, 128, 1}, {128, 160, 0}, {128, 128, 1}, {128, 64, 1}, {64, 64, 1}, {256, 320, 1}, {256, 320, 0},
                         {128, 320, 0}};
constexpr int kNumCfgs = 9;

}

extern "C" int mvd_gemm_num_configs(void) { return kNumCfgs; }

extern "C" int mvd_debug_last_gemm_plan(int* out) {
  if (!out) { mvd_set_error("last_gemm_plan: null argument"); return -1; }
  out[0] = g_mvd_last_gemm.cfg; out[1] = g_mvd_last_gemm.splitk; out[2] = g_mvd_last_gemm.tiles;
  out[3] = g_mvd_last_gemm.grid; out[4] = g_mvd_last_gemm.per_cu;
  return 0;
}

extern "C" int mvd_debug_last_gemm_nowait(void) { return g_mvd_last_gemm.nowait; }

static int deep_conv_split(const MvdGemmArgs& a, long t7) {
  static const int on = MVD_ENV_INT("MVD_GEMM_DEEP_CONV_SPLIT", 1);
  if (!on || (mvd_debug_flags() & 262144) || a.seg[0].mode == MVD_A_DENSE || a.geglu || a.out_f32 || t7 < 24 || t7 > 64 || a.Ktot < 8192 || (a.splitk > 0 && a.splitk < 4)) return 1;
  int s = (int)(256 / t7);
  while (s > 1 && a.Ktot / 64 / s < 16) --s;
  return s > 16 ? 16 : s;
}

int mvd_gemm_pick_config(const MvdGemmArgs& a) {
  static const int use7 = MVD_ENV_INT("MVD_GEMM_BIG", 1);
  static const int split_min_slabs = MVD_ENV_INT("MVD_GEMM_SPLIT_MINK", 4096) / 64;
  static const int use8 = MVD_ENV_INT("MVD_GEMM_C8", 0);
  if (use7 && a.N % 320 == 0 && a.M >= 1024) {
    const long t7 = (long)((a.M + 255) / 256) * (a.N / 320);
    if (a.geglu) { if (t7 >= 200) return 6; }
    else if (t7 >= 200) return 7;
    else if (use8 && t7 * 2 >= 200) return 8;
    else if (a.Ktot / 64 >= split_min_slabs && t7 * 2 >= 200) return 7;
    else if (deep_conv_split(a, t7) > 1) return 7;
  }
  static const int order[] = {2, 3, 4, 5};
  int cfg = -1, first_valid = -1;
  long best_blocks = -1;
  for (int c : order) {
    if (a.N % kCfgs[c].bn) continue;
    if (a.geglu && !kCfgs[c].tn_even) continue;
    const long blocks = (long)((a.M + kCfgs[c].bm - 1) / kCfgs[c].bm) * (a.N / kCfgs[c].bn);
    if (first_valid < 0) {
      first_valid = c;
      if (blocks < 300 && !a.geglu && a.Ktot / 64 >= 16 && c <= 3 && a.M >= 512) return c;
    }
    if (blocks >= 300) return c;
    if (blocks > best_blocks) { best_blocks = blocks; cfg = c; }
  }
  return cfg;
}

int mvd_launch_gemm(const MvdGemmArgs& a, hipStream_t s, int force_cfg) {
  if (a.M <= 0 || a.N <= 0 || a.Ktot <= 0 || a.nseg < 1 || a.nseg > 2) { mvd_set_error("gemm: bad dims M=%d N=%d K=%d nseg=%d", a.M, a.N, a.Ktot, a.nseg); return -1; }
  int ksum = 0;
  for (int i = 0; i < a.nseg; ++i) {
    const MvdASeg& g = a.seg[i];
    if (g.mode == MVD_A_DENSE) {
      if (g.c0 % 64 || g.c1 % 64 || g.ksize != g.c0 + g.c1 || !g.p0 || (g.c1 && !g.p1)) { mvd_set_error("gemm: bad dense segment %d (c0=%d c1=%d ksize=%d)", i, g.c0, g.c1, g.ksize); return -1; }
    } else if (g.mode == MVD_A_CONV3) {
      if (g.c0 % 64 || g.c1 != 0 || g.ksize != 9 * g.c0 || !g.p0 || (g.stride != 1 && g.stride != 2) || (g.ups && g.stride != 1)) { mvd_set_error("gemm: bad conv segment %d", i); return -1; }
      if (g.asym && (g.asym != 1 || g.stride != 2 || (g.inH & 1) || (g.inW & 1))) { mvd_set_error("gemm: bottom/right-only padding needs stride 2 and an even input size"); return -1; }
      const int eh = g.ups ? 2 * g.inH : (g.stride == 2 ? (g.inH + 1) / 2 : g.inH);
      const int ew = g.ups ? 2 * g.inW : (g.stride == 2 ? (g.inW + 1) / 2 : g.inW);
      if (eh != a.outH || ew != a.outW || a.rows_per_batch != a.outH * a.outW || a.M % a.rows_per_batch) { mvd_set_error("gemm: conv geometry mismatch (in %dx%d out %dx%d rpb %d M %d)", g.inH, g.inW, a.outH, a.outW, a.rows_per_batch, a.M); return -1; }
    } else { mvd_set_error("gemm: bad mode"); return -1; }
    ksum += g.ksize;
  }
  if (a.nseg == 2 && !(a.seg[0].mode == MVD_A_CONV3 && a.seg[1].mode == MVD_A_DENSE)) { mvd_set_error("gemm: a second segment must be a dense segment after a conv segment"); return -1; }
  if (ksum != a.Ktot) { mvd_set_error("gemm: segment K sum %d != Ktot %d", ksum, a.Ktot); return -1; }
  if (a.ldw < a.Ktot || (a.ldw % 8) || !a.W) { mvd_set_error("gemm: bad weight stride ldw=%d (K=%d)", a.ldw, a.Ktot); return -1; }
  if (a.rows_per_batch <= 0) { mvd_set_error("gemm: rows_per_batch must be > 0"); return -1; }
  if (a.N % 64) { mvd_set_error("gemm: N=%d must be a multiple of 64", a.N); return -1; }
  if (a.splitk > 1 && (!a.part || a.geglu || a.splitk > (force_cfg >= 100 ? 64 : 16) || a.splitk > a.Ktot / 64)) { mvd_set_error("gemm: bad split-K request (splitk=%d)", a.splitk); return -1; }
  if (a.geglu && (a.out_f32 || a.res || a.rowvec)) { mvd_set_error("gemm: unsupported GEGLU epilogue combination"); return -1; }
  const int on = a.geglu ? a.N / 2 : a.N;
  if (a.ldo < on || (a.ldo % 4) || (a.res && (a.ldres % 4))) { mvd_set_error("gemm: bad leading dims"); return -1; }

  static const int default_glds = MVD_ENV_INT("MVD_GEMM_GLDS", 1);
  bool glds = default_glds != 0;
#ifdef MVD_PROBE
  static const int dbg = MVD_ENV_INT("MVD_GEMM_DEBUG", 0);
  if (dbg) const_cast<MvdGemmArgs&>(a).dbg = dbg;
#endif
  int cfg = force_cfg;
  if (cfg >= 1000) { const_cast<MvdGemmArgs&>(a).w_blocked = 1; cfg -= 1000; }
  if (a.w_blocked && cfg < 100) { mvd_set_error("gemm: the blocked weight layout is read by the small-M kernels only"); return -1; }
  if (cfg >= 100) {
    const int tile = (cfg - 100) / 10, ns = (cfg - 100) % 10;
    if (a.splitk > 1 && !a.tile_cnt) { mvd_set_error("gemm: the small-M kernels combine split-K in the kernel and need tile counters"); return -1; }
    g_mvd_last_gemm.cfg = cfg; g_mvd_last_gemm.splitk = a.splitk > 1 ? a.splitk : 1;
    return mvd_launch_gemm_sm(a, s, tile, ns ? ns : 4);
  }
#ifdef MVD_PROBE
  static const int use_ring = MVD_ENV_INT("MVD_GEMM_RING", 0);
  if (cfg == 15) {
    if (a.N % 320 || a.geglu || a.out_f32) { mvd_set_error("gemm: the ring kernel needs N %% 320 == 0, bf16 output, no GEGLU"); return -1; }
    return mvd_launch_gemm_ring(a, s);
  }
#endif
  bool legacy = MVD_ENV_INT("MVD_GEMM_LEGACY", 0) != 0;
  if (cfg == 16 || cfg == 17) { legacy = true; cfg -= 10; }
  if (cfg == 14) { glds = true; cfg = 8; }
  else if (cfg >= 8 && cfg < 14) { glds = true; cfg -= 8; } else if (cfg >= 0 && cfg < 6) { glds = false; }
  if (cfg < 0) cfg = mvd_gemm_pick_config(a);
  if (a.ln_c1) {
    if ((cfg != 6 && cfg != 7) || legacy || a.dbg || !mvd_gemm_ln_fold_ok(a)) { mvd_set_error("gemm: LayerNorm fold not available for M=%d N=%d K=%d cfg=%d", a.M, a.N, a.Ktot, cfg); return -1; }
  }
  if (cfg < 0 || cfg >= kNumCfgs || a.N % kCfgs[cfg].bn || (a.geglu && !kCfgs[cfg].tn_even)) { mvd_set_error("gemm: no tile config for N=%d geglu=%d cfg=%d", a.N, a.geglu, cfg); return -1; }
  g_mvd_last_gemm.cfg = cfg; g_mvd_last_gemm.splitk = a.splitk > 1 ? a.splitk : 1;
#ifndef MVD_PROBE
  if (cfg == 0 || cfg == 1 || cfg == 8 || force_cfg == 16 || force_cfg == 17) { mvd_set_error("gemm: tile config %d exists in probe builds only", force_cfg >= 0 ? force_cfg : cfg); return -1; }
#endif
  switch (cfg) {
#ifdef MVD_PROBE
    case 0: return launch_cfg<C0>(a, s, glds);
    case 1: return launch_cfg<C1>(a, s, glds);
    case 8: return launch_cfg<C8>(a, s, true);
#endif
    case 2: return launch_cfg<C2>(a, s, glds);
    case 3: return launch_cfg<C3>(a, s, glds);
    case 4: return launch_cfg<C4>(a, s, glds);
    case 6:
      if (!a.geglu || a.seg[0].mode != MVD_A_DENSE || a.splitk > 1) { mvd_set_error("gemm: tile config 6 is GEGLU-only"); return -1; }
      if (!legacy && !(a.dbg & ~32) && mvd_gemm_pp_applicable(a)) return mvd_launch_gemm_pp(a, s);
      return launch_mode2<C6, 0, true, false>(a, s);
    case 7:
      if (!legacy && !(a.dbg & ~32) && !a.geglu && mvd_gemm_pp_applicable(a)) return mvd_launch_gemm_pp(a, s);
#ifdef MVD_PROBE
      if (use_ring && !a.out_f32 && !a.dbg) return mvd_launch_gemm_ring(a, s);
#endif
      return launch_cfg<C7, true>(a, s, true);
    default: return launch_cfg<C5>(a, s, glds);
  }
}

int mvd_gemm_pick_splitk(const MvdGemmArgs& a) {
  if (a.geglu) return 1;
  const int cfg = mvd_gemm_pick_config(a);
  if (cfg < 0) return 1;
  const long tiles = (long)((a.M + kCfgs[cfg].bm - 1) / kCfgs[cfg].bm) * (a.N / kCfgs[cfg].bn);
  const int nkt = a.Ktot / 64;
  if (cfg == 7 && deep_conv_split(a, tiles) > 1) return deep_conv_split(a, tiles);
  if (cfg == 7 || cfg == 8) return (tiles >= 200 || nkt < 16) ? 1 : 2;
  if (tiles >= 256 || nkt < 16) return 1;
  long s = 512 / tiles;
  if (s > nkt / 8) s = nkt / 8;
  long cap = (long)a.Ktot / (4L * a.M);
  cap = cap < 4 ? 4 : (cap > 16 ? 16 : cap);
  if (s > cap) s = cap;
  return s < 2 ? 1 : (int)s;
}

extern "C" int mvd_debug_pick_splitk(int m, int n, int k, int geglu) {
  MvdGemmArgs a; memset(&a, 0, sizeof(a));
  a.M = m; a.N = n; a.Ktot = k; a.geglu = geglu;
  return mvd_gemm_pick_splitk(a);
}
extern "C" int mvd_debug_pick_splitk_conv(int m, int n, int k) {
  MvdGemmArgs a; memset(&a, 0, sizeof(a));
  a.M = m; a.N = n; a.Ktot = k; a.seg[0].mode = MVD_A_CONV3;
  return mvd_gemm_pick_splitk(a);
}

int mvd_launch_splitk_reduce(const MvdGemmArgs& a, hipStream_t s) {
  if (a.splitk < 2 || !a.part || (a.N & 3)) { mvd_set_error("splitk_reduce: bad arguments"); return -1; }
  const long nvec = (long)a.M * (a.N >> 2);
  int grid = (int)((nvec + 255) / 256);
  if (grid > 2048) grid = 2048;
  hipLaunchKernelGGL(splitk_reduce_kernel, dim3(grid), dim3(256), 0, s, a);
  hipError_t e = hipGetLastError();
  if (e != hipSuccess) { mvd_set_error("splitk_reduce launch: %s", hipGetErrorString(e)); return -3; }
  return 0;
}
```

### mvd_amd/csrc/gemm_pp.hip

```cpp
#include <stdlib.h>
#include <string.h>
#include "kernels.h"

namespace {

constexpr int BN = 320, NT = 512;
constexpr int B_BYTES = BN * 128, B_IT = BN * 8 / NT;
constexpr unsigned OOB = 0x80000000u;

typedef __attribute__((address_space(3))) void lds_void;

MVD_DEVINL int fresh_lane() {
  int l = (int)__builtin_amdgcn_mbcnt_hi(~0u, __builtin_amdgcn_mbcnt_lo(~0u, 0u));
  asm volatile("" : "+v"(l));
  return l;
}

MVD_DEVINL void store16(u32x4 v, __amdgpu_buffer_rsrc_t rsrc, int voff, int soff) {
  __builtin_amdgcn_raw_buffer_store_b128(v, rsrc, voff, soff, 0);
  asm volatile("s_nop 1" :: "v"(v));
}

MVD_DEVINL int swz_off(int row, int chunk) { return row * 128 + ((chunk ^ ((row >> 1) & 7)) << 4); }

MVD_DEVINL void dma16(__amdgpu_buffer_rsrc_t rsrc, unsigned char* lds_wave_base, unsigned voff, unsigned soff) {
  __builtin_amdgcn_raw_ptr_buffer_load_lds(rsrc, (lds_void*)lds_wave_base, 16, (int)voff, (int)soff, 0, 0);
}

constexpr int XCH_C1 = 0, XCH_C2 = 2048, XCH_STATS = 4096, XCH_BYTES = 6144;

template <int BM, int WM, int WN, int AMODE, bool SPLITK, bool LNF = false>
__global__ __launch_bounds__(NT, 2) void gemm_pp_kernel(const MvdGemmArgs a) {
  static_assert(!LNF || (AMODE == 0 && !SPLITK), "the LayerNorm fold is a dense, unsplit form");
  constexpr int A_BYTES = BM * 128, STAGE_BYTES = A_BYTES + B_BYTES;
  constexpr int A_IT = BM * 8 / NT;
  static_assert(A_IT == 4, "the A loader below is written for 256-row tiles");
  constexpr int WTM = BM / WM, WTN = BN / WN, TM = WTM / 16, TN = WTN / 16;
  constexpr bool GEGLU = WM == 4;
  constexpr bool HAS_CONV = AMODE != 0;
  constexpr bool UPS = AMODE == 3;
  static_assert((WTM * 128) % 2048 == 0 && (WTN % 16) == 0, "fragment rows of a wave share one swizzle pattern");
  extern __shared__ __attribute__((aligned(16))) unsigned char smem[];
  const int tid = threadIdx.x, lane = tid & 63;
  const int wave = __builtin_amdgcn_readfirstlane(tid >> 6);
  const int grp = wave >> 2;
  const int wm = wave / WN, wn = wave % WN;
  const int ntn = a.N / BN;
  const int ntm = (a.M + BM - 1) / BM;
  const int lrow = tid >> 3;
  const int kc = (tid & 7) ^ ((lrow >> 1) & 7);
  const int w4 = wave & 3;
  const int arow = w4 * 8 + (lane >> 3);

  const int S = SPLITK ? a.splitk : 1;
  const int ntiles = ntn * ntm * S;
  const int xcd = blockIdx.x & 7, xj = blockIdx.x >> 3;
  const int gx = (gridDim.x >> 3) + ((int)(gridDim.x & 7) > xcd ? 1 : 0);
  const int tq = ntiles >> 3, tr = ntiles & 7;
  const int tstart = xcd < tr ? xcd * (tq + 1) : tr * (tq + 1) + (xcd - tr) * tq;
  const int tend = tstart + tq + (xcd < tr ? 1 : 0);
  const int wcg = SPLITK ? 0 : a.walk_cg;
  const int xrows = (tend - tstart) / ntn, xrow0 = tstart / ntn;
  auto tile_mn = [&](int t, int& m0, int& n0) {
    if (wcg) {
      const int li = t - tstart, per = xrows * wcg;
      const int g = li / per, rem = li - g * per;
      const int r = rem / wcg;
      m0 = (xrow0 + r) * BM; n0 = (g * wcg + (rem - r * wcg)) * BN;
    } else { m0 = (t / ntn) * BM; n0 = (t % ntn) * BN; }
  };
  const int tile_first = tstart + xj, tile_end = tend, tile_step = gx;
  int tile = tile_first;
  if (tile >= tile_end) return;

  const MvdASeg& cs = a.seg[0];
  const MvdASeg& ds = a.seg[AMODE == 2 ? 1 : 0];
  const int nkt_conv = HAS_CONV ? (9 * cs.c0) / 64 : 0;
  const int nkt = a.Ktot / 64;
  const int conv_c2 = cs.c0 * 2;
  const int conv_rowB = cs.inW * conv_c2;
  constexpr bool conv_ups = UPS;
  const int limH = conv_ups ? 2 * cs.inH : cs.inH, limW = conv_ups ? 2 * cs.inW : cs.inW;
  const int dc0 = ds.c0, dc1 = LNF ? 0 : ds.c1;

  __amdgpu_buffer_rsrc_t rs_w = __builtin_amdgcn_make_buffer_rsrc(const_cast<bf16_t*>(a.W), 0, (int)((size_t)a.N * a.ldw * 2), 0x00020000);
  __amdgpu_buffer_rsrc_t rs_c = rs_w, rs_d0 = rs_w, rs_d1 = rs_w;
  if (HAS_CONV) {
    const int shift = conv_rowB + conv_c2;
    const size_t bytes = (size_t)(a.M / a.rows_per_batch) * cs.inH * cs.inW * conv_c2;
    rs_c = __builtin_amdgcn_make_buffer_rsrc(reinterpret_cast<char*>(const_cast<bf16_t*>(cs.p0)) - shift, 0, (int)(bytes + shift), 0x00020000);
  }
  if (AMODE == 0 || AMODE == 2) {
    rs_d0 = __builtin_amdgcn_make_buffer_rsrc(const_cast<bf16_t*>(ds.p0), 0, (int)((size_t)a.M * dc0 * 2), 0x00020000);
    if (dc1) rs_d1 = __builtin_amdgcn_make_buffer_rsrc(const_cast<bf16_t*>(ds.p1), 0, (int)((size_t)a.M * dc1 * 2), 0x00020000);
  }
  const unsigned voff_w = (unsigned)lrow * (unsigned)a.ldw * 2u + kc * 16;
  const unsigned voff_d0 = (unsigned)arow * (unsigned)dc0 * 2u + kc * 16;
  const unsigned voff_d1 = (unsigned)arow * (unsigned)dc1 * 2u + kc * 16;

  int ld_m0 = 0, ld_n0 = 0;
  unsigned a_base[A_IT];
  int a_yx[A_IT];
  auto setup_loader = [&](int work) {
    const int t = S == 1 ? work : work / S;
    tile_mn(t, ld_m0, ld_n0);
    if (HAS_CONV) {
#pragma unroll
      for (int i = 0; i < A_IT; ++i) {
        int m = ld_m0 + (2 * grp + (i & 1)) * 64 + arow + (i >> 1) * 32;
        m = m < a.M ? m : a.M - 1;
        const int b = m / a.rows_per_batch;
        const int rem = m - b * a.rows_per_batch;
        const int oy = rem / a.outW, ox = rem - oy * a.outW;
        const int ys = oy * cs.stride + cs.asym, xs = ox * cs.stride + cs.asym;
        int okm = 0;
#pragma unroll
        for (int t = 0; t < 9; ++t) {
          const int iy = ys - 1 + t / 3, ix = xs - 1 + t % 3;
          okm |= ((unsigned)iy < (unsigned)limH && (unsigned)ix < (unsigned)limW) ? (1 << t) : 0;
        }
        a_yx[i] = (ys & 0x7ff) | ((xs & 0x7ff) << 11) | (okm << 22);
        const int ty = conv_ups ? ((ys - 1) >> 1) : ys - 1, tx = conv_ups ? ((xs - 1) >> 1) : xs - 1;
        a_base[i] = (unsigned)((b * cs.inH * cs.inW + (ty + 1) * cs.inW + (tx + 1)) * conv_c2 + kc * 16);
      }
    }
  };

  auto issue_a = [&](int st, int lk, int i0, int i1) {
    unsigned char* sa = smem + st * STAGE_BYTES + (2 * grp) * 8192 + w4 * 1024;
    if (HAS_CONV && (AMODE != 2 || lk < nkt_conv)) {
      const int sl = lk / 9, tap = lk - sl * 9;
#ifdef PP_ABLATE_A_TAPS
      if (tap != 0) return;
#endif
      const int dy = tap / 3, dx = tap - dy * 3;
      unsigned soff = (unsigned)(sl * 128);
      if (!conv_ups) soff += (unsigned)(dy * conv_rowB + dx * conv_c2);
      else soff += (unsigned)((dy == 2 ? conv_rowB : 0) + (dx == 2 ? conv_c2 : 0));
#pragma unroll
      for (int i = 0; i < A_IT; ++i) {
        const bool ok = (a_yx[i] >> (22 + tap)) & 1;
        unsigned vo = a_base[i];
        if (conv_ups) {
          if (dy == 1) vo += (a_yx[i] & 1) ? 0u : (unsigned)conv_rowB;
          if (dx == 1) vo += (a_yx[i] & 0x800) ? 0u : (unsigned)conv_c2;
        }
        if (i >= i0 && i < i1) dma16(rs_c, sa + (i & 1) * 8192 + (i >> 1) * 4096, ok ? vo : OOB, soff);
      }
    } else {
      const int cc = (lk - nkt_conv) << 6;
      const bool first = LNF || cc < dc0;
      const int pitch = (first ? dc0 : dc1) * 2;
      const unsigned col2 = (unsigned)((first ? cc : cc - dc0) * 2);
#pragma unroll
      for (int i = 0; i < A_IT; ++i) {
        if (i < i0 || i >= i1) continue;
        const unsigned soff = (unsigned)(ld_m0 + (2 * grp + (i & 1)) * 64 + (i >> 1) * 32) * (unsigned)pitch + col2;
        if (first) dma16(rs_d0, sa + (i & 1) * 8192 + (i >> 1) * 4096, voff_d0, soff);
        else dma16(rs_d1, sa + (i & 1) * 8192 + (i >> 1) * 4096, voff_d1, soff);
      }
    }
  };
  constexpr int W_Q = 2 * B_IT, W_Q_R0 = 3;
  auto issue_w = [&](int st, int lk, int q0, int q1) {
    unsigned char* sb = smem + st * STAGE_BYTES + A_BYTES + wave * 1024;
    const unsigned ldw2 = (unsigned)a.ldw * 2u;
    const unsigned so = (unsigned)ld_n0 * ldw2 + (unsigned)lk * 128u;
#pragma unroll
    for (int q = 0; q < W_Q; ++q)
      if (q >= q0 && q < q1) dma16(rs_w, sb + (q >> 1) * 8192 + (q & 1) * 4096, voff_w, so + (unsigned)((q >> 1) * 64 + (q & 1) * 32) * ldw2);
  };

  f32x4 acc[TM][TN];
  constexpr int TS = TM / WN;
  static_assert(!LNF || (TS * WN == TM && WM * TM * 16 * 8 <= XCH_BYTES - XCH_STATS && BN * 4 <= XCH_C2 - XCH_C1), "exchange area layout");
  float row_s[LNF ? TS : 1], row_q[LNF ? TS : 1];
  unsigned char* const xch = smem + 2 * STAGE_BYTES;
  const int fr = lane & 15, fq = lane >> 4;
  const float alpha = a.alpha;

  auto init_acc = [&]() {
#pragma unroll
    for (int i = 0; i < TM; ++i)
#pragma unroll
      for (int j = 0; j < TN; ++j) acc[i][j] = f32x4{0.f, 0.f, 0.f, 0.f};
    if constexpr (LNF) {
#pragma unroll
      for (int t = 0; t < TS; ++t) { row_s[t] = 0.f; row_q[t] = 0.f; }
    }
  };
  auto issue_consts = [&](int n0) {
    if constexpr (LNF) {
      if (wave < 2) {
        __amdgpu_buffer_rsrc_t rs_k = __builtin_amdgcn_make_buffer_rsrc(const_cast<float*>(wave == 0 ? a.ln_c1 : a.bias), 0, a.N * 4, 0x00020000);
        unsigned char* dst = xch + (wave == 0 ? XCH_C1 : XCH_C2);
        const unsigned vo = (unsigned)fresh_lane() * 16u;
        dma16(rs_k, dst, vo, n0 * 4);
        dma16(rs_k, dst + 1024, vo, n0 * 4 + 1024);
      }
    }
  };
  auto stats_publish = [&]() {
    if constexpr (LNF) {
      const float invk = __builtin_bit_cast(float, __builtin_amdgcn_readfirstlane(__builtin_bit_cast(int, 1.f / (float)a.Ktot)));
#pragma unroll
      for (int t = 0; t < TS; ++t) {
        float sm = row_s[t], sq = row_q[t];
        sm += __shfl_xor(sm, 16); sq += __shfl_xor(sq, 16);
        sm += __shfl_xor(sm, 32); sq += __shfl_xor(sq, 32);
        const float mean = sm * invk;
        const float var = fmaxf(sq * invk - mean * mean, 0.f);
        const float sc = rsqrtf(var + a.ln_eps);
        if (fq == 0) *reinterpret_cast<float2*>(xch + XCH_STATS + (((wm * TM + wn * TS + t) * 16 + fr) << 3)) = float2{sc, -sc * mean};
      }
      asm volatile("s_waitcnt lgkmcnt(0)" ::: "memory");
    }
  };
  auto load_colconst = [&](int m0, int n0, f32x4 (&cb)[TN]) {
    const int nb = n0 + wn * WTN + fq * 4;
#pragma unroll
    for (int j = 0; j < TN; ++j) cb[j] = f32x4{0.f, 0.f, 0.f, 0.f};
    if (a.bias) {
#pragma unroll
      for (int j = 0; j < TN; ++j) cb[j] = *reinterpret_cast<const f32x4*>(a.bias + nb + j * 16);
    }
    if (!GEGLU && a.rowvec && a.rows_per_batch % BM == 0) {
      const float* rv = a.rowvec + (size_t)(m0 / a.rows_per_batch) * a.ld_rowvec + nb;
#pragma unroll
      for (int j = 0; j < TN; ++j) cb[j] += *reinterpret_cast<const f32x4*>(rv + j * 16);
    }
  };

  auto swap_pair = [&](u32x2& x, u32x2& y) {
    auto r0 = __builtin_amdgcn_permlane16_swap(x[0], y[0], false, false);
    auto r1 = __builtin_amdgcn_permlane16_swap(x[1], y[1], false, false);
    x[0] = r0[0]; y[0] = r0[1]; x[1] = r1[0]; y[1] = r1[1];
  };
  const int pair_col = (fq & 1) * 16 + (fq >> 1) * 8;
  auto epilogue = [&](int m0, int n0, int ks) {
    asm volatile("" : "+s"(m0), "+s"(n0));
    const int row0 = m0 + wm * WTM;
    if (SPLITK) {
      __amdgpu_buffer_rsrc_t rs_p = __builtin_amdgcn_make_buffer_rsrc(a.part + (size_t)ks * a.M * a.N, 0, (int)((size_t)a.M * a.N * 4), 0x00020000);
      const int vo = (fr * a.N + fq * 4) * 4;
#pragma unroll
      for (int i = 0; i < TM; ++i)
#pragma unroll
        for (int j = 0; j < TN; ++j)
          store16(__builtin_bit_cast(u32x4, acc[i][j]), rs_p, vo, ((row0 + i * 16) * a.N + n0 + wn * WTN + j * 16) * 4);
      return;
    }
    __amdgpu_buffer_rsrc_t rs_o = __builtin_amdgcn_make_buffer_rsrc(a.out, 0, (int)((size_t)a.M * a.ldo * 2), 0x00020000);
    int vo16, vo8, efr = fr, efq = fq;
    if constexpr (LNF) {
      const int el = fresh_lane();
      efr = el & 15; efq = el >> 4;
      vo16 = (efr * a.ldo + (efq & 1) * 16 + (efq >> 1) * 8) * 2; vo8 = (efr * a.ldo + efq * 4) * 2;
    } else {
      vo16 = (fr * a.ldo + pair_col) * 2; vo8 = (fr * a.ldo + fq * 4) * 2;
    }
    if constexpr (GEGLU) {
      constexpr int NO = TN / 2;
      const int oc0 = (n0 + wn * WTN) / 2;
      auto gate = [&](const f32x4& v, const f32x4& g) -> u32x2 {
        return u32x2{pack2bf(v[0] * gelu_erf_f(g[0]), v[1] * gelu_erf_f(g[1])), pack2bf(v[2] * gelu_erf_f(g[2]), v[3] * gelu_erf_f(g[3]))};
      };
      if constexpr (LNF) {
        const unsigned char* cc = xch + (wn * WTN + efq * 4) * 4;
#pragma unroll
        for (int i = 0; i < TM; ++i) {
          const float2 st = *reinterpret_cast<const float2*>(xch + XCH_STATS + (((wm * TM + i) * 16 + efr) << 3));
          auto lin = [&](int j) -> f32x4 {
            return acc[i][j] * st.x + (*reinterpret_cast<const f32x4*>(cc + XCH_C1 + j * 64) * st.y + *reinterpret_cast<const f32x4*>(cc + XCH_C2 + j * 64));
          };
          u32x2 o[NO];
#pragma unroll
          for (int q = 0; q < NO; ++q) o[q] = gate(lin(2 * q), lin(2 * q + 1));
          const int so = ((row0 + i * 16) * a.ldo + oc0) * 2;
#pragma unroll
          for (int q = 0; q + 1 < NO; q += 2) {
            swap_pair(o[q], o[q + 1]);
            store16(u32x4{o[q][0], o[q][1], o[q + 1][0], o[q + 1][1]}, rs_o, vo16, so + q * 32);
          }
          if (NO & 1) __builtin_amdgcn_raw_buffer_store_b64(o[NO - 1], rs_o, vo8, so + (NO - 1) * 32, 0);
        }
      } else {
        f32x4 cb[TN];
        load_colconst(m0, n0, cb);
#pragma unroll
        for (int i = 0; i < TM; ++i) {
          u32x2 o[NO];
#pragma unroll
          for (int q = 0; q < NO; ++q) o[q] = gate(acc[i][2 * q] + cb[2 * q], acc[i][2 * q + 1] + cb[2 * q + 1]);
          const int so = ((row0 + i * 16) * a.ldo + oc0) * 2;
#pragma unroll
          for (int q = 0; q + 1 < NO; q += 2) {
            swap_pair(o[q], o[q + 1]);
            store16(u32x4{o[q][0], o[q][1], o[q + 1][0], o[q + 1][1]}, rs_o, vo16, so + q * 32);
          }
          if (NO & 1) __builtin_amdgcn_raw_buffer_store_b64(o[NO - 1], rs_o, vo8, so + (NO - 1) * 32, 0);
        }
      }
    } else if constexpr (LNF) {
      const unsigned char* cc = xch + (wn * WTN + efq * 4) * 4;
      f32x4 k1[TN], k2[TN];
#pragma unroll
      for (int j = 0; j < TN; ++j) {
        k1[j] = *reinterpret_cast<const f32x4*>(cc + XCH_C1 + j * 64);
        k2[j] = *reinterpret_cast<const f32x4*>(cc + XCH_C2 + j * 64);
      }
#pragma unroll
      for (int i = 0; i < TM; ++i) {
        const float2 st = *reinterpret_cast<const float2*>(xch + XCH_STATS + (((wm * TM + i) * 16 + efr) << 3));
        const int so = ((row0 + i * 16) * a.ldo + n0 + wn * WTN) * 2;
        auto one = [&](int j) -> u32x2 {
          const f32x4 v = (acc[i][j] * st.x + (k1[j] * st.y + k2[j])) * alpha;
          return u32x2{pack2bf(v[0], v[1]), pack2bf(v[2], v[3])};
        };
#pragma unroll
        for (int j = 0; j + 1 < TN; j += 2) {
          u32x2 oa = one(j), ob = one(j + 1);
          swap_pair(oa, ob);
          store16(u32x4{oa[0], oa[1], ob[0], ob[1]}, rs_o, vo16, so + j * 32);
        }
        if (TN & 1) __builtin_amdgcn_raw_buffer_store_b64(one(TN - 1), rs_o, vo8, so + (TN - 1) * 32, 0);
      }
    } else {
      const bool has_res = a.res != nullptr;
      __amdgpu_buffer_rsrc_t rs_r = rs_o;
      if (has_res) rs_r = __builtin_amdgcn_make_buffer_rsrc(const_cast<bf16_t*>(a.res), 0, (int)((size_t)a.M * a.ldres * 2), 0x00020000);
      const int vr16 = (fr * a.ldres + pair_col) * 2, vr8 = (fr * a.ldres + fq * 4) * 2;
      constexpr int NP = TN / 2;
      f32x4 cb[TN];
      load_colconst(m0, n0, cb);
      const bool row_rv = a.rowvec && a.rows_per_batch % BM != 0;
      constexpr int RG = HAS_CONV ? 2 : 4;
#pragma unroll
      for (int i0 = 0; i0 < TM; i0 += RG) {
        u32x4 rp[RG][NP > 0 ? NP : 1];
        u32x2 rs1[RG];
        if (has_res) {
#pragma unroll
          for (int g = 0; g < RG; ++g) {
            const int so = ((row0 + (i0 + g) * 16) * a.ldres + n0 + wn * WTN) * 2;
#pragma unroll
            for (int q = 0; q < NP; ++q) rp[g][q] = __builtin_amdgcn_raw_buffer_load_b128(rs_r, vr16, so + q * 64, 0);
            if (TN & 1) rs1[g] = __builtin_amdgcn_raw_buffer_load_b64(rs_r, vr8, so + (TN - 1) * 32, 0);
          }
        }
#pragma unroll
        for (int g = 0; g < RG; ++g) {
          const int i = i0 + g;
          const int so = ((row0 + i * 16) * a.ldo + n0 + wn * WTN) * 2;
          int mrow = row0 + i * 16 + fr;
          mrow = mrow < a.M ? mrow : a.M - 1;
          const float* rvp = row_rv ? a.rowvec + (size_t)(mrow / a.rows_per_batch) * a.ld_rowvec + n0 + wn * WTN + fq * 4 : nullptr;
          auto finish = [&](f32x4 v, int j, u32x2 r) -> u32x2 {
            v += cb[j];
            if (row_rv) v += *reinterpret_cast<const f32x4*>(rvp + j * 16);
            v *= alpha;
            if (has_res) { v[0] += bflo(r[0]); v[1] += bfhi(r[0]); v[2] += bflo(r[1]); v[3] += bfhi(r[1]); }
            return u32x2{pack2bf(v[0], v[1]), pack2bf(v[2], v[3])};
          };
#pragma unroll
          for (int q = 0; q < NP; ++q) {
            u32x2 ra = {0u, 0u}, rb = {0u, 0u};
            if (has_res) {
              ra = u32x2{rp[g][q][0], rp[g][q][1]}; rb = u32x2{rp[g][q][2], rp[g][q][3]};
              swap_pair(ra, rb);
            }
            u32x2 oa = finish(acc[i][2 * q], 2 * q, ra), ob = finish(acc[i][2 * q + 1], 2 * q + 1, rb);
            swap_pair(oa, ob);
            store16(u32x4{oa[0], oa[1], ob[0], ob[1]}, rs_o, vo16, so + q * 64);
          }
          if (TN & 1) __builtin_amdgcn_raw_buffer_store_b64(finish(acc[i][TN - 1], TN - 1, has_res ? rs1[g] : u32x2{0u, 0u}), rs_o, vo8, so + (TN - 1) * 32, 0);
        }
      }
    }
  };

  auto slab_range = [&](int work, int& k0, int& k1) {
    if (S == 1) { k0 = 0; k1 = nkt; return; }
    const int ks = work % S;
    k0 = (ks * nkt) / S;
    k1 = ((ks + 1) * nkt) / S;
  };

  bf16x8 af[TM], wf[TN];
  u32x4 sf[LNF ? TS : 1];
  const int frag_off = fr * 128 + ((fq ^ ((fr >> 1) & 7)) << 4);
  auto read_frags = [&](int st, int half) {
    const unsigned char* sa = smem + st * STAGE_BYTES + wm * (WTM * 128) + (frag_off ^ (half * 64));
    const unsigned char* sb = smem + st * STAGE_BYTES + A_BYTES + wn * (WTN * 128) + (frag_off ^ (half * 64));
#pragma unroll
    for (int j = 0; j < TN; ++j) wf[j] = *reinterpret_cast<const bf16x8*>(sb + j * 2048);
#pragma unroll
    for (int i = 0; i < TM; ++i) af[i] = *reinterpret_cast<const bf16x8*>(sa + i * 2048);
    if constexpr (LNF) {
#pragma unroll
      for (int t = 0; t < TS; ++t) sf[t] = *reinterpret_cast<const u32x4*>(sa + (wn * TS + t) * 2048);
    }
  };
  auto mfma_half = [&]() {
    __builtin_amdgcn_s_setprio(1);
#pragma unroll
    for (int i = 0; i < TM; ++i)
#pragma unroll
      for (int j = 0; j < TN; ++j)
        acc[i][j] = __builtin_amdgcn_mfma_f32_16x16x32_bf16(wf[j], af[i], acc[i][j], 0, 0, 0);
    if constexpr (LNF) {
      typedef __attribute__((ext_vector_type(2))) __bf16 bf16x2;
      const bf16x2 ones = __builtin_bit_cast(bf16x2, 0x3f803f80u);
#pragma unroll
      for (int t = 0; t < TS; ++t) {
        const unsigned d[4] = {sf[t].x, sf[t].y, sf[t].z, sf[t].w};
#pragma unroll
        for (int e = 0; e < 4; ++e) {
          const bf16x2 x = __builtin_bit_cast(bf16x2, d[e]);
          row_q[t] = __builtin_amdgcn_fdot2_f32_bf16(x, x, row_q[t], false);
          row_s[t] = __builtin_amdgcn_fdot2_f32_bf16(x, ones, row_s[t], false);
        }
        asm volatile("" : "+v"(row_q[t]), "+v"(row_s[t]));
      }
    }
    __builtin_amdgcn_s_setprio(0);
  };
#ifdef MVD_PROBE
  int stamp_n = 0;
  long long* stamp_p = ((a.dbg & 32) && a.part && blockIdx.x < 64 && (wave & 3) == 0 && lane == 0)
                           ? reinterpret_cast<long long*>(a.part) + ((size_t)blockIdx.x * 2 + grp) * 512 : nullptr;
#endif
  auto phase_end = [&]() {
    __builtin_amdgcn_sched_barrier(0);
#ifdef MVD_PROBE
    if (stamp_p && stamp_n < 511) stamp_p[1 + stamp_n++] = (long long)__builtin_amdgcn_s_memtime();
#endif
    __builtin_amdgcn_s_barrier();
#ifdef MVD_PROBE
    if (stamp_p && stamp_n < 511) { stamp_p[1 + stamp_n++] = (long long)__builtin_amdgcn_s_memtime(); stamp_p[0] = stamp_n; }
#endif
    __builtin_amdgcn_sched_barrier(0);
  };

  int kt0, kt1;
  slab_range(tile, kt0, kt1);
  setup_loader(tile);
  issue_a(0, kt0, 0, A_IT);
  if (grp == 0) issue_w(0, kt0, 0, W_Q);
  issue_consts(ld_n0);
  init_acc();
  asm volatile("s_waitcnt vmcnt(0)" ::: "memory");
  phase_end();
  if (grp == 1) phase_end();

  int cur = 0;
  bool pend = false;
  int pm0 = 0, pn0 = 0, pks = 0;
  for (;;) {
    const int tl = S == 1 ? tile : tile / S;
    const int ks = S == 1 ? 0 : tile - tl * S;
    int m0, n0;
    tile_mn(tl, m0, n0);
    const int next_tile = tile + tile_step;
    const bool have_next = next_tile < tile_end;
    int nkt0 = 0, nkt1 = 0;
    if (have_next) slab_range(next_tile, nkt0, nkt1);
    for (int kt = kt0; kt < kt1; ++kt) {
      const bool last_k = kt + 1 == kt1;
      const bool more = !last_k || have_next;
      const int nlk = last_k ? nkt0 : kt + 1;
      if (pend) {
        if (grp == 0) phase_end();
        if constexpr (LNF) { stats_publish(); phase_end(); }
        epilogue(pm0, pn0, pks);
        init_acc();
        phase_end();
        if (grp == 1) phase_end();
        pend = false;
      }
      if (LNF && kt == kt0 && tile != tile_first) issue_consts(n0);
      read_frags(cur, 0);
      if (more) {
        if (last_k) setup_loader(next_tile);
        if (grp == 0) { issue_a(cur ^ 1, nlk, 0, A_IT); issue_w(cur ^ 1, nlk, 0, W_Q_R0); }
        else issue_a(cur ^ 1, nlk, 0, A_IT / 2);
      }
      asm volatile("s_waitcnt lgkmcnt(0)" ::: "memory");
      phase_end();
      mfma_half();
      phase_end();
      read_frags(cur, 1);
      if (grp == 0) {
        if (more) issue_w(cur ^ 1, nlk, W_Q_R0, W_Q);
        asm volatile("s_waitcnt lgkmcnt(0)" ::: "memory");
      } else {
        if (more) issue_a(cur ^ 1, nlk, A_IT / 2, A_IT);
        asm volatile("s_waitcnt lgkmcnt(0)" ::: "memory");
      }
      phase_end();
      mfma_half();
      asm volatile("s_waitcnt vmcnt(0)" ::: "memory");
      phase_end();
      if (last_k) { pend = true; pm0 = m0; pn0 = n0; pks = ks; }
      cur ^= 1;
    }
    if (!have_next) break;
    tile = next_tile; kt0 = nkt0; kt1 = nkt1;
  }
  if constexpr (LNF) { stats_publish(); phase_end(); }
  epilogue(pm0, pn0, pks);
  if (grp == 0) phase_end();
}

template <int BM, int WM, int WN, int AMODE, bool SPLITK, bool LNF = false>
int launch_pp(const MvdGemmArgs& a, hipStream_t s) {
  constexpr int LDS_BYTES = 2 * (BM * 128 + B_BYTES) + (LNF ? XCH_BYTES : 0);
  static bool init[16] = {};
  int dev = 0;
  (void)hipGetDevice(&dev);
  if (!init[dev & 15]) {
    hipError_t e = hipFuncSetAttribute(reinterpret_cast<const void*>(&gemm_pp_kernel<BM, WM, WN, AMODE, SPLITK, LNF>),
                                       hipFuncAttributeMaxDynamicSharedMemorySize, LDS_BYTES);
    if (e != hipSuccess) { mvd_set_error("gemm_pp: hipFuncSetAttribute: %s", hipGetErrorString(e)); return -2; }
    init[dev & 15] = true;
  }
  const int ntm = (a.M + BM - 1) / BM, ntn = a.N / BN;
  MvdGemmArgs b = a;
  b.walk_cg = SPLITK ? 0 : mvd_gemm_pp_walk(a);
  int grid = 256;
  const int ntiles = ntm * ntn * (a.splitk > 1 ? a.splitk : 1);
  if (ntiles < grid) grid = ((ntiles + 7) / 8) * 8;
  g_mvd_last_gemm.tiles = ntiles; g_mvd_last_gemm.grid = grid; g_mvd_last_gemm.per_cu = 1;
  hipLaunchKernelGGL((gemm_pp_kernel<BM, WM, WN, AMODE, SPLITK, LNF>), dim3(grid), dim3(NT), LDS_BYTES, s, b);
  hipError_t e = hipGetLastError();
  if (e != hipSuccess) { mvd_set_error("gemm_pp launch: %s", hipGetErrorString(e)); return -3; }
  return 0;
}

template <int BM, int WM, int WN>
int launch_pp_mode(const MvdGemmArgs& a, hipStream_t s) {
  const bool sk = a.splitk > 1;
  if (a.seg[0].mode == MVD_A_DENSE) return sk ? launch_pp<BM, WM, WN, 0, true>(a, s) : launch_pp<BM, WM, WN, 0, false>(a, s);
  if (a.seg[0].ups) {
    if (a.nseg != 1) { mvd_set_error("gemm_pp: an upsampling convolution takes no shortcut segment"); return -1; }
    return sk ? launch_pp<BM, WM, WN, 3, true>(a, s) : launch_pp<BM, WM, WN, 3, false>(a, s);
  }
  if (a.nseg == 1) return sk ? launch_pp<BM, WM, WN, 1, true>(a, s) : launch_pp<BM, WM, WN, 1, false>(a, s);
  return sk ? launch_pp<BM, WM, WN, 2, true>(a, s) : launch_pp<BM, WM, WN, 2, false>(a, s);
}

}

int mvd_gemm_pp_walk(const MvdGemmArgs& a) {
  static const int on = MVD_ENV_INT("MVD_GEMM_PP_WALK", 1);
  if (!on || (mvd_debug_flags() & 131072) || a.walk_cg < 0) return 0;
  if (a.walk_cg > 0) return a.walk_cg;
  if (a.seg[0].mode != MVD_A_DENSE || a.nseg != 1 || a.splitk > 1) return 0;
  const int ntm = (a.M + 255) / 256, ntn = a.N / BN;
  if (ntm % 8 || ntm < 64 || ntn < 8) return 0;
  const size_t panel = (size_t)BN * a.Ktot * 2;
  if (panel * ntn <= (size_t)(5 << 19)) return 0;
  int c = (int)(((size_t)7 << 18) / panel);
  if (c < 2) return 0;
  while (c > 1 && (ntn % c || 32 % c)) --c;
  return c >= 2 ? c : 0;
}

bool mvd_gemm_pp_applicable(const MvdGemmArgs& a) {
  constexpr int BM = 256;
  const size_t lim = (size_t)1 << 31;
  if (a.N % BN || a.Ktot % 64 || a.out_f32) return false;
  if ((size_t)a.N * a.ldw * 2 >= lim) return false;
  if ((size_t)(a.M + BM) * a.ldo * 2 >= lim || (a.res && (size_t)(a.M + BM) * a.ldres * 2 >= lim)) return false;
  if (a.splitk > 1 && (size_t)(a.M + BM) * a.N * 4 >= lim) return false;
  for (int i = 0; i < a.nseg; ++i) {
    const MvdASeg& g = a.seg[i];
    if (g.mode == MVD_A_DENSE) {
      if ((size_t)(a.M + BM) * (g.c0 > g.c1 ? g.c0 : g.c1) * 2 >= lim) return false;
    } else {
      const size_t bytes = (size_t)(a.M / a.rows_per_batch) * g.inH * g.inW * g.c0 * 2 + (size_t)(g.inW + 1) * g.c0 * 2;
      if (bytes + (size_t)3 * g.inW * g.c0 * 2 >= lim) return false;
      if (2 * g.inH >= 32768 || 2 * g.inW >= 32768) return false;
    }
  }
  return true;
}

int mvd_launch_gemm_pp(const MvdGemmArgs& a, hipStream_t s) {
  if (a.ln_c1) {
    const MvdASeg& g = a.seg[0];
    if (a.nseg != 1 || g.mode != MVD_A_DENSE || g.c1 || a.splitk > 1 || a.res || a.rowvec || !a.bias) {
      mvd_set_error("gemm_pp: the LayerNorm fold takes one dense source, a bias, no residual / row vector / split-K"); return -1;
    }
    return a.geglu ? launch_pp<256, 4, 2, 0, false, true>(a, s) : launch_pp<256, 2, 4, 0, false, true>(a, s);
  }
  if (a.geglu) {
    if (a.seg[0].mode != MVD_A_DENSE || a.splitk > 1) { mvd_set_error("gemm_pp: GEGLU needs a dense, unsplit problem"); return -1; }
    return launch_pp<256, 4, 2, 0, false>(a, s);
  }
  return launch_pp_mode<256, 2, 4>(a, s);
}

bool mvd_gemm_ln_fold_ok(const MvdGemmArgs& a) {
  const MvdASeg& g = a.seg[0];
  if (a.nseg != 1 || g.mode != MVD_A_DENSE || g.c1 || a.splitk > 1 || a.res || a.rowvec || a.out_f32) return false;
  if (a.Ktot != g.c0 || a.Ktot > 640) return false;
  if (a.geglu && a.Ktot > 320) return false;
  const int cfg = mvd_gemm_pick_config(a);
  return (a.geglu ? cfg == 6 : cfg == 7) && mvd_gemm_pp_applicable(a);
}
```

### mvd_amd/csrc/kernels.h

```cpp
#pragma once
#include <hip/hip_runtime.h>
#include <stdint.h>
#include "common.h"

enum { MVD_A_DENSE = 0, MVD_A_CONV3 = 1 };

struct MvdASeg {
  const bf16_t* p0;
  const bf16_t* p1;
  int c0, c1;
  int mode;
  int ksize;
  int inH, inW;
  int stride;
  int ups;
  int asym;
};

struct MvdGemmArgs {
  MvdASeg seg[2];
  int nseg;
  const bf16_t* W;
  int ldw;
  int M, N, Ktot;
  int rows_per_batch;
  int outH, outW;
  const float* bias;
  const float* rowvec;
  int ld_rowvec;
  const bf16_t* res;
  int ldres;
  float alpha;
  int geglu;
  void* out;
  int ldo;
  int out_f32;
  int splitk;
  float* part;
  int w_blocked;
  int splitk_nowait;
  unsigned int* tile_cnt;
  int dbg;
  const float* ln_c1;
  float ln_eps;
  int walk_cg;
};

int mvd_launch_gemm(const MvdGemmArgs& a, hipStream_t s, int force_cfg = -1);
int mvd_gemm_pick_config(const MvdGemmArgs& a);
struct MvdLaunchPlan { int cfg, splitk, tiles, grid, per_cu, nowait; };
extern thread_local MvdLaunchPlan g_mvd_last_gemm;
bool mvd_gemm_pp_applicable(const MvdGemmArgs& a);
int mvd_gemm_pp_walk(const MvdGemmArgs& a);
int mvd_debug_flags();
bool mvd_gemm_ln_fold_ok(const MvdGemmArgs& a);
int mvd_launch_gemm_pp(const MvdGemmArgs& a, hipStream_t s);
int mvd_launch_gemm_ring(const MvdGemmArgs& a, hipStream_t s);
bool mvd_gemm_sm_applicable(const MvdGemmArgs& a, int tile);
int mvd_launch_gemm_sm(const MvdGemmArgs& a, hipStream_t s, int tile, int nstage);
bool mvd_gemm_sm_plan(const MvdGemmArgs& a, int* tile, int* nstage, int* splitk);
struct MvdXsArgs {
  const bf16_t* x; int ldx;
  const bf16_t* w;
  int M, K, units;
  int geglu;
  int ln; float ln_eps;
  const bf16_t* res; int ldres;
  bf16_t* out; int ldo;
  int csplit;
};
bool mvd_gemm_xs_applicable(const MvdXsArgs& a);
int mvd_gemm_xs_pick_csplit(const MvdXsArgs& a);
int mvd_launch_gemm_xs(const MvdXsArgs& a, hipStream_t s);
struct MvdWsArgs {
  const bf16_t* x; int B, H, W, C;
  int ups;
  const bf16_t* sc0; const bf16_t* sc1; int scc0, scc1;
  const bf16_t* w;
  const float* bias;
  const float* rowvec; int ld_rowvec;
  const bf16_t* res; int ldres;
  bf16_t* out; int ldo;
  int M, N;
  int variant;
};
bool mvd_conv_ws_applicable(const MvdWsArgs& a);
size_t mvd_conv_ws_packed_elems(int C, int sc, int N);
int mvd_launch_conv_ws(const MvdWsArgs& a, hipStream_t s);
#define MVD_OP_SPLITK_COUNTERS 4096
int mvd_launch_splitk_reduce(const MvdGemmArgs& a, hipStream_t s);
int mvd_gemm_pick_splitk(const MvdGemmArgs& a);

struct MvdAttnProblem {
  const bf16_t* q; const bf16_t* k; const bf16_t* v; bf16_t* o;
  int ldq, ldk, ldv, ldo;
  int64_t bsq, bsk, bsv, bso;
  int nq, nk;
};
struct MvdAttnArgs {
  MvdAttnProblem p[2];
  int nprob;
  int batch, heads;
  float scale;
  int prescaled;
  int dbg;
  int nsplit;
  void* split_ws;
  unsigned int* split_cnt;
};
int mvd_attention_pick_split(const MvdAttnArgs& a);
size_t mvd_attention_split_ws_bytes(const MvdAttnArgs& a, int nsplit);
int mvd_attention_split_counters(const MvdAttnArgs& a);
int mvd_launch_attention(const MvdAttnArgs& a, hipStream_t s);

#define MVD_GN_MAXCHUNK 256
int mvd_launch_groupnorm(const bf16_t* x0, const bf16_t* x1, int c0, int c1, int batch, int hw, int groups,
                         float eps, const float* gamma, const float* beta, int silu, bf16_t* y, float* ws,
                         hipStream_t s);
int mvd_launch_layernorm(const bf16_t* x, int rows, int c, float eps, const float* gamma, const float* beta,
                         bf16_t* y, hipStream_t s);
int mvd_launch_refnorm(const bf16_t* x, int batch, int hw, int c, bf16_t* y, hipStream_t s);
int mvd_launch_refstats(const bf16_t* x, int batch, int hw, int c, float* stats , hipStream_t s);
int mvd_launch_refapply(const bf16_t* x, int batch, int hw, int c, const float* mean_k , bf16_t* y, hipStream_t s);

int mvd_launch_nchw_to_nhwc(const float* x, int batch, int c, int hw, const float* scale, const float* shift,
                            int ld_ss, bf16_t* y, hipStream_t s);
int mvd_launch_film(const bf16_t* x, int batch, int hw, int c, const float* scale, const float* shift, int ld_ss,
                    bf16_t* y, hipStream_t s);
int mvd_launch_conv_in(const bf16_t* x, int batch, int h, int w, int cin, const float* wt, const float* bias,
                       int cout, bf16_t* y, hipStream_t s);
int mvd_launch_conv_out(const bf16_t* x, int batch, int h, int w, int c, const bf16_t* wt, const float* bias,
                        int cout, float* y, hipStream_t s);
int mvd_launch_im2col_in(const float* x, int batch, int c, int h, int w, const float* scale, const float* shift, int ld_ss,
                         bf16_t* y, hipStream_t s);
int mvd_launch_f32_to_bf16(const float* x, int64_t n, bf16_t* y, hipStream_t s);
int mvd_launch_nhwc_to_nchw_f32(const bf16_t* x, int batch, int hw, int c, float* y, hipStream_t s);

int mvd_launch_skinny_linear(const float* x, int ldx, int batch, int k, const void* w, int wbf16, const float* bias,
                             int n, int act_in, float* y, int ldy, hipStream_t s);
struct MvdSegTable { int n; int end[16]; };
int mvd_launch_skinny_linear_grouped(const float* x, int ldx, int xseg, int batch, int k, const float* w, const float* bias, int n,
                                     const MvdSegTable& seg, float* y, int ldy, hipStream_t s);
int mvd_launch_film_params_grouped(const float* raw, int batch, const MvdSegTable& seg, float strength, float* out, int out_rows,
                                   hipStream_t s);
int mvd_launch_layernorm_f32(const float* x, int rows, int c, float eps, const float* gamma, const float* beta,
                             int silu, float* y, hipStream_t s, int nseg = 1);
int mvd_launch_timestep_embedding(const float* t, int batch, int dim, float* y, hipStream_t s);
int mvd_launch_camera_features(const float* src, const float* tgt, int batch, int cam_rows, int nfreq,
                               float max_freq, float* rflat, float* enc, hipStream_t s);
int mvd_launch_film_params(const float* raw, int batch, int dim, float strength, float* scale, float* shift, int out_rows,
                           hipStream_t s);

int mvd_launch_film_nchw_f32(const float* x, int batch, int c, int hw, const float* scale, const float* shift, float* y,
                             hipStream_t s);

void mvd_set_error(const char* fmt, ...);
```

### mvd_amd/ops.py

```python
from __future__ import annotations

import ctypes as C
from typing import Optional

import torch

from . import _lib as L


def _p(t: Optional[torch.Tensor]):
    if t is None:
        return None
    assert t.is_cuda and t.is_contiguous(), "ops expect contiguous CUDA tensors"
    return C.c_void_p(t.data_ptr())


def _s():
    return C.c_void_p(torch.cuda.current_stream().cuda_stream)


def _bf16(*ts):
    for t in ts:
        if t is not None:
            assert t.dtype == torch.bfloat16, "expected bf16"


def linear(a, w, bias=None, a2=None, rowvec=None, rows_per_batch=0, res=None, alpha=1.0, geglu=False,
           out_f32=False, force_cfg=-1, splitk=1):
    _bf16(a, a2, w, res)
    m, k1 = a.shape
    k2 = a2.shape[1] if a2 is not None else 0
    n = w.shape[0]
    assert w.shape[1] == k1 + k2
    on = n // 2 if geglu else n
    out = torch.empty(m, on, device=a.device, dtype=torch.float32 if out_f32 else torch.bfloat16)
    ws = torch.empty(splitk * m * n + 4096, device=a.device, dtype=torch.float32) if splitk > 1 else None
    L.call("mvd_op_linear", _p(a), _p(a2), k1, k2, _p(w), _p(bias), _p(rowvec),
           rowvec.shape[1] if rowvec is not None else 0, rows_per_batch, _p(res), float(alpha), int(geglu),
           _p(out), int(out_f32), m, n, force_cfg, splitk, _p(ws), _s())
    return out


def ln_linear(x, w_folded, cf, eps=1e-5, geglu=False):
    _bf16(x, w_folded)
    m, k = x.shape
    n = w_folded.shape[0]
    assert w_folded.shape[1] == k and cf.shape == (2, n) and cf.dtype == torch.float32 and cf.is_contiguous()
    out = torch.empty(m, n // 2 if geglu else n, device=x.device, dtype=torch.bfloat16)
    L.call("mvd_op_ln_linear", _p(x), k, _p(w_folded), _p(cf[0]), _p(cf[1]), float(eps), int(geglu), _p(out), m, n, _s())
    return out


def linear_xs(x, w_packed, geglu=False, ln=False, eps=1e-5, res=None, csplit=0, k=None):
    _bf16(x, w_packed, res)
    m = x.shape[0]
    units, ks1 = w_packed.shape[0], w_packed.shape[1]
    k = (ks1 - 1) * 16 if k is None else k
    n_out = units * 16 if geglu else units * 32
    out = torch.empty(m, n_out, device=x.device, dtype=torch.bfloat16)
    assert x.stride(1) == 1 and (res is None or res.stride(1) == 1)
    L.call("mvd_op_linear_xs", C.c_void_p(x.data_ptr()), x.stride(0), _p(w_packed), m, k, units, int(geglu), int(ln), float(eps),
           C.c_void_p(res.data_ptr()) if res is not None else None, res.stride(0) if res is not None else 0, _p(out), n_out,
           csplit, _s())
    return out


def conv3x3_ws(x, w_packed, bias, n, rowvec=None, res=None, shortcut=None, shortcut2=None, variant=0, upsample=False):
    _bf16(x, w_packed, res, shortcut, shortcut2)
    b, h, w, c = x.shape
    out = torch.empty(b, 2 * h if upsample else h, 2 * w if upsample else w, n, device=x.device, dtype=torch.bfloat16)
    assert bias.dtype == torch.float32 and bias.numel() == n and x.is_contiguous()
    assert rowvec is None or (rowvec.dtype == torch.float32 and rowvec.stride(1) == 1)
    pp = lambda t: C.c_void_p(t.data_ptr()) if t is not None else None
    L.call("mvd_op_conv3x3_ws", _p(x), b, h, w, c, _p(w_packed), _p(bias), pp(rowvec), rowvec.stride(0) if rowvec is not None else 0,
           pp(res), pp(shortcut), pp(shortcut2), shortcut.shape[-1] if shortcut is not None else 0,
           shortcut2.shape[-1] if shortcut2 is not None else 0, _p(out), n, int(variant) + (16 if upsample else 0), _s())
    return out


def conv3x3(x, w_packed, bias=None, stride=1, upsample=False, rowvec=None, res=None, shortcut=None,
            shortcut2=None, force_cfg=-1, splitk=1, asym_pad=False):
    _bf16(x, w_packed, res, shortcut, shortcut2)
    B, H, W, Cin = x.shape
    cout = w_packed.shape[0]
    oh = H * 2 if upsample else (H + 1) // 2 if stride == 2 else H
    ow = W * 2 if upsample else (W + 1) // 2 if stride == 2 else W
    out = torch.empty(B, oh, ow, cout, device=x.device, dtype=torch.bfloat16)
    c1 = shortcut.shape[-1] if shortcut is not None else 0
    c2 = shortcut2.shape[-1] if shortcut2 is not None else 0
    ws = torch.empty(splitk * B * oh * ow * cout + 4096, device=x.device, dtype=torch.float32) if splitk > 1 else None
    L.call("mvd_op_conv3x3", _p(x), B, H, W, Cin, stride, int(upsample), int(asym_pad), _p(w_packed), _p(bias), _p(rowvec),
           rowvec.shape[1] if rowvec is not None else 0, _p(res), _p(shortcut), _p(shortcut2), c1, c2, _p(out), cout,
           force_cfg, splitk, _p(ws), _s())
    return out


def attention(q, k, v, heads, scale=0.125):
    _bf16(q, k, v)
    B, nq, _ = q.shape
    nk = k.shape[1]
    assert q.stride(2) == 1 and k.stride(2) == 1 and v.stride(2) == 1
    assert q.stride(0) == nq * q.stride(1) and k.stride(0) == nk * k.stride(1) and v.stride(0) == nk * v.stride(1)
    out = torch.empty(B, nq, heads * 64, device=q.device, dtype=torch.bfloat16)
    L.call("mvd_op_attention", C.c_void_p(q.data_ptr()), C.c_void_p(k.data_ptr()), C.c_void_p(v.data_ptr()), _p(out),
           B, heads, nq, nk, q.stride(1), k.stride(1), v.stride(1), heads * 64, float(scale), _s())
    return out


def attention_split(q, k, v, heads, nsplit):
    _bf16(q, k, v)
    B, nq, _ = q.shape
    nk = k.shape[1]
    out = torch.empty(B, nq, heads * 64, device=q.device, dtype=torch.bfloat16)
    ws = torch.empty(int(L.lib().mvd_op_attention_split_ws_bytes(B, heads, nq, nsplit)), device=q.device, dtype=torch.uint8)
    L.call("mvd_op_attention_split", C.c_void_p(q.data_ptr()), C.c_void_p(k.data_ptr()), C.c_void_p(v.data_ptr()), _p(out),
           B, heads, nq, nk, q.stride(1), k.stride(1), v.stride(1), heads * 64, nsplit, _p(ws), _s())
    return out


def groupnorm(x, gamma, beta, groups=32, eps=1e-5, silu=False, x2=None):
    _bf16(x, x2)
    B, hw, c0 = x.shape
    c1 = x2.shape[2] if x2 is not None else 0
    y = torch.empty(B, hw, c0 + c1, device=x.device, dtype=torch.bfloat16)
    ws = torch.empty(B * 256 * groups * 2, device=x.device, dtype=torch.float32)
    L.call("mvd_op_groupnorm", _p(x), _p(x2), c0, c1, B, hw, groups, float(eps), _p(gamma), _p(beta), int(silu), _p(y),
           _p(ws), _s())
    return y


def layernorm(x, gamma, beta, eps=1e-5):
    _bf16(x)
    rows, c = x.shape
    y = torch.empty_like(x)
    L.call("mvd_op_layernorm", _p(x), rows, c, float(eps), _p(gamma), _p(beta), _p(y), _s())
    return y


def refnorm(x):
    _bf16(x)
    B, hw, c = x.shape
    y = torch.empty_like(x)
    L.call("mvd_op_refnorm", _p(x), B, hw, c, _p(y), _s())
    return y


def film(x, scale, shift):
    _bf16(x)
    B, hw, c = x.shape
    y = torch.empty_like(x)
    L.call("mvd_op_film", _p(x), B, hw, c, _p(scale), _p(shift), _p(y), _s())
    return y


def conv_in(x, w, bias):
    B, H, W, cin = x.shape
    cout = w.shape[0]
    y = torch.empty(B, H, W, cout, device=x.device, dtype=torch.bfloat16)
    L.call("mvd_op_conv_in", _p(x), B, H, W, cin, _p(w), _p(bias), cout, _p(y), _s())
    return y


def conv_out(x, w, bias):
    B, H, W, c = x.shape
    cout = w.shape[0]
    y = torch.empty(B, cout, H, W, device=x.device, dtype=torch.float32)
    L.call("mvd_op_conv_out", _p(x), B, H, W, c, _p(w), _p(bias), cout, _p(y), _s())
    return y


def softmax_rows(s):
    assert s.dtype == torch.float32 and s.dim() == 2
    out = torch.empty(s.shape, device=s.device, dtype=torch.bfloat16)
    L.call("mvd_op_softmax_rows", _p(s), s.shape[0], s.shape[1], _p(out), _s())
    return out


def ddpm_step(model_out, sample, noise, c0, c1, c2, c3, sigma):
    assert model_out.dtype == torch.float32 and sample.dtype == torch.float32
    out = torch.empty_like(sample)
    L.call("mvd_op_ddpm_step", _p(model_out), _p(sample), _p(noise), float(c0), float(c1), float(c2), float(c3),
           float(sigma), _p(out), sample.numel(), _s())
    return out


def cfg_combine(uncond_cond, guidance_scale):
    assert uncond_cond.dtype == torch.float32 and uncond_cond.shape[0] % 2 == 0
    out = torch.empty((uncond_cond.shape[0] // 2,) + tuple(uncond_cond.shape[1:]), device=uncond_cond.device,
                      dtype=torch.float32)
    L.call("mvd_op_cfg_combine", _p(uncond_cond), float(guidance_scale), _p(out), out.numel(), _s())
    return out


def sampler_step(model_out, sample, a0, a1, p, q, r=0.0, sigma=0.0, x0_prev=None, noise=None, guidance_scale=None,
                 out=None, x0_out=None):
    guided = guidance_scale is not None
    assert model_out.dtype == torch.float32 and sample.dtype == torch.float32
    assert model_out.numel() == sample.numel() * (2 if guided else 1), (tuple(model_out.shape), tuple(sample.shape))
    for t in (x0_prev, noise, out, x0_out):
        assert t is None or (t.dtype == torch.float32 and t.numel() == sample.numel())
    if out is None:
        out = torch.empty_like(sample)
    L.call("mvd_op_sampler_step", _p(model_out), int(guided), float(guidance_scale) if guided else 0.0, _p(sample), _p(x0_prev),
           _p(noise), float(a0), float(a1), float(p), float(q), float(r), float(sigma), _p(out), _p(x0_out), sample.numel(), _s())
    return out


def skinny_linear(x, w, bias=None, silu_in=False):
    assert x.dtype == torch.float32 and x.is_cuda and x.dim() == 2 and w.dim() == 2 and w.shape[1] == x.shape[1]
    assert w.dtype in (torch.float32, torch.bfloat16) and x.is_contiguous() and w.is_contiguous()
    b, k = x.shape
    n = w.shape[0]
    y = torch.empty(b, n, device=x.device, dtype=torch.float32)
    L.call("mvd_op_skinny_linear", _p(x), k, b, k, _p(w), int(w.dtype == torch.bfloat16), _p(bias), n, int(silu_in), _p(y), n, _s())
    return y


def nchw_to_nhwc(x, scale=None, shift=None):
    B, c, H, W = x.shape
    y = torch.empty(B, H, W, c, device=x.device, dtype=torch.bfloat16)
    L.call("mvd_op_nchw_to_nhwc", _p(x), B, c, H * W, _p(scale), _p(shift), _p(y), _s())
    return y


def last_gemm_plan():
    out = (C.c_int * 5)()
    L.call("mvd_debug_last_gemm_plan", out)
    return dict(cfg=out[0], splitk=out[1], tiles=out[2], grid=out[3], per_cu=out[4], nowait=L.lib().mvd_debug_last_gemm_nowait())


def last_attention_plan():
    out = (C.c_int * 2)()
    L.call("mvd_debug_last_attention_plan", out)
    return dict(waves=out[0], workgroups=out[1])


def engine_splitk(m, n, k, geglu=False, conv=False):
    if conv:
        return L.lib().mvd_debug_pick_splitk_conv(m, n, k)
    return L.lib().mvd_debug_pick_splitk(m, n, k, int(geglu))
```

### mvd_amd/packing.py

```python
from __future__ import annotations

from typing import Dict


import torch

from .config import UNetConfig

QSCALE = 64 ** -0.5 * 1.4426950408889634


def _bf(t: torch.Tensor, device) -> torch.Tensor:
    return t.detach().to(device=device, dtype=torch.float32).to(torch.bfloat16).contiguous()


def _f32(t: torch.Tensor, device) -> torch.Tensor:
    return t.detach().to(device=device, dtype=torch.float32).contiguous()


def _conv_w(w: torch.Tensor, tap_major: bool = False) -> torch.Tensor:
    co, ci, kh, kw = w.shape
    w = w.detach().float()
    if tap_major or ci % 64:
        return w.permute(0, 2, 3, 1).reshape(co, kh * kw * ci)
    return w.reshape(co, ci // 64, 64, kh, kw).permute(0, 1, 3, 4, 2).reshape(co, kh * kw * ci)


def block_weight(w: torch.Tensor) -> torch.Tensor:
    n, k = w.shape
    assert n % 32 == 0 and k % 64 == 0, (n, k)
    b = w.reshape(n // 32, 32, k // 64, 8, 8).permute(0, 2, 1, 3, 4)
    r = torch.arange(32, device=w.device)
    slot = torch.arange(8, device=w.device)
    src = slot[None, :] ^ ((r[:, None] >> 1) & 7)
    idx = src[None, None, :, :, None].expand(n // 32, k // 64, 32, 8, 8)
    return torch.gather(b, 3, idx).contiguous().reshape(n, k)


def _geglu_rows(w: torch.Tensor) -> torch.Tensor:
    half = w.shape[0] // 2
    val, gate = w[:half], w[half:]
    rest = w.shape[1:]
    v = val.reshape(half // 16, 1, 16, *rest)
    g = gate.reshape(half // 16, 1, 16, *rest)
    return torch.cat([v, g], dim=1).reshape(w.shape)


XS_K = 320


def _xs_row_perm(device) -> torch.Tensor:
    m = torch.arange(32, device=device)
    return 16 * ((m >> 2) & 1) + 4 * (m >> 3) + (m & 3)


def pack_xs(w: torch.Tensor, bias, geglu: bool = False, device=None) -> torch.Tensor:
    device = device if device is not None else w.device
    w = w.detach().to(device=device, dtype=torch.float32)
    n, k = w.shape
    assert k % 16 == 0 and n % (64 if geglu else 32) == 0, (n, k)
    b = torch.zeros(n, device=device) if bias is None else bias.detach().to(device=device, dtype=torch.float32)
    if geglu:
        half = n // 2
        order = torch.stack([torch.arange(half, n, device=device).reshape(-1, 32),
                             torch.arange(0, half, device=device).reshape(-1, 32)], 1).reshape(-1)
        w, b = w[order], b[order]
    units, ks = n // 32, k // 16
    perm = _xs_row_perm(device)
    wu = w.reshape(units, 32, k)[:, perm]
    bu = b.reshape(units, 32)[:, perm]
    frag = wu.reshape(units, 32, ks, 2, 8).permute(0, 2, 3, 1, 4)
    out = torch.zeros(units, ks + 1, 2, 32, 8, device=device, dtype=torch.bfloat16)
    out[:, :ks] = frag.to(torch.bfloat16)
    hi = bu.to(torch.bfloat16)
    lo = (bu - hi.float()).to(torch.bfloat16)
    out[:, ks, 0, :, 0] = hi
    out[:, ks, 0, :, 1] = lo
    return out.reshape(units, ks + 1, 64, 8).contiguous()


def pack_ws(w4: torch.Tensor, wsc=None, device=None) -> torch.Tensor:
    device = device if device is not None else w4.device
    w4 = w4.detach().to(device=device, dtype=torch.float32)
    n, c = w4.shape[0], w4.shape[1]
    assert n % 16 == 0 and c % 128 == 0 and tuple(w4.shape[2:]) == (3, 3), tuple(w4.shape)
    t = w4.permute(0, 2, 3, 1).reshape(n // 16, 16, 9, c // 128, 4, 4, 8)
    conv = t.permute(0, 3, 4, 2, 5, 1, 6).reshape(n // 16, -1)
    parts = [conv]
    if wsc is not None:
        wsc = wsc.detach().to(device=device, dtype=torch.float32).reshape(n, -1)
        sc = wsc.shape[1]
        assert sc % 128 == 0, sc
        u = wsc.reshape(n // 16, 16, sc // 128, 4, 4, 8)
        parts.append(u.permute(0, 2, 3, 4, 1, 5).reshape(n // 16, -1))
    return torch.cat(parts, 1).to(torch.bfloat16).contiguous().reshape(-1)


LN_FOLD_MAX_C = 1 << 30
LN_FOLD_LARGE_BATCH_MAX_C = 640


def fold_layernorm(w: torch.Tensor, gamma: torch.Tensor, beta: torch.Tensor, bias, device):
    w, gamma, beta = w.detach().float(), gamma.detach().float(), beta.detach().float()
    wf = (w * gamma[None, :]).to(torch.bfloat16)
    c1 = wf.float().sum(1)
    c2 = w @ beta
    if bias is not None:
        c2 = c2 + bias.detach().float()
    return wf.to(device).contiguous(), torch.stack([c1, c2], 0).to(device=device, dtype=torch.float32).contiguous()


def ws_twin_shapes_ok(c: int, n: int, scc0: int, scc1: int) -> bool:
    return c > 0 and c % 128 == 0 and n > 0 and n % 16 == 0 and scc0 % 128 == 0 and scc1 % 128 == 0 and not (scc1 and not scc0)


def pack_unet(sd: Dict[str, torch.Tensor], cfg: UNetConfig, device, adapter: bool, ref_scale: float = 0.0,
              small_batch_twins: bool = True) -> Dict[str, torch.Tensor]:
    fold_max_c = LN_FOLD_MAX_C if small_batch_twins else LN_FOLD_LARGE_BATCH_MAX_C
    out: Dict[str, torch.Tensor] = {}
    w_in = _conv_w(sd["conv_in.weight"], tap_major=True)
    out["conv_in.w"] = _bf(torch.nn.functional.pad(w_in, (0, 64 - w_in.shape[1])), device)
    out["conv_in.b"] = _f32(sd["conv_in.bias"], device)
    out["time.l1.w"] = _bf(sd["time_embedding.linear_1.weight"], device)
    out["time.l1.b"] = _f32(sd["time_embedding.linear_1.bias"], device)
    out["time.l2.w"] = _bf(sd["time_embedding.linear_2.weight"], device)
    out["time.l2.b"] = _f32(sd["time_embedding.linear_2.bias"], device)
    tw, tb = [], []
    split = cfg.resnet_input_split()
    for key, cin, cout in cfg.resnets():
        out[f"{key}.norm1.g"] = _f32(sd[f"{key}.norm1.weight"], device)
        out[f"{key}.norm1.b"] = _f32(sd[f"{key}.norm1.bias"], device)
        out[f"{key}.conv1.w"] = _bf(_conv_w(sd[f"{key}.conv1.weight"]), device)
        out[f"{key}.conv1.b"] = _f32(sd[f"{key}.conv1.bias"], device)
        out[f"{key}.norm2.g"] = _f32(sd[f"{key}.norm2.weight"], device)
        out[f"{key}.norm2.b"] = _f32(sd[f"{key}.norm2.bias"], device)
        w2 = _conv_w(sd[f"{key}.conv2.weight"])
        b2 = sd[f"{key}.conv2.bias"].detach().float()
        if cin != cout:
            w2 = torch.cat([w2, sd[f"{key}.conv_shortcut.weight"].detach().float().reshape(cout, cin)], dim=1)
            b2 = b2 + sd[f"{key}.conv_shortcut.bias"].detach().float()
        out[f"{key}.conv2.w"] = _bf(w2, device)
        out[f"{key}.conv2.b"] = _f32(b2, device)
        if small_batch_twins and cout > cfg.block_out_channels[0]:
            if ws_twin_shapes_ok(cin, cout, 0, 0):
                out[f"{key}.conv1.ws"] = pack_ws(sd[f"{key}.conv1.weight"], None, device)
            if cin == cout:
                if ws_twin_shapes_ok(cout, cout, 0, 0):
                    out[f"{key}.conv2.ws"] = pack_ws(sd[f"{key}.conv2.weight"], None, device)
            elif ws_twin_shapes_ok(cout, cout, *split[key]):
                out[f"{key}.conv2.ws"] = pack_ws(sd[f"{key}.conv2.weight"], sd[f"{key}.conv_shortcut.weight"].reshape(cout, cin), device)
        tw.append(sd[f"{key}.time_emb_proj.weight"].detach().float())
        tb.append(sd[f"{key}.time_emb_proj.bias"].detach().float())
    out["temb_proj.w"] = _bf(torch.cat(tw, 0), device)
    out["temb_proj.b"] = _f32(torch.cat(tb, 0), device)

    tkv = []
    for key, _feat, C, _heads in cfg.transformers():
        b = f"{key}.transformer_blocks.0"
        out[f"{key}.norm.g"] = _f32(sd[f"{key}.norm.weight"], device)
        out[f"{key}.norm.b"] = _f32(sd[f"{key}.norm.bias"], device)
        out[f"{key}.proj_in.w"] = _bf(sd[f"{key}.proj_in.weight"], device)
        out[f"{key}.proj_in.b"] = _f32(sd[f"{key}.proj_in.bias"], device)
        out[f"{key}.proj_out.w"] = _bf(sd[f"{key}.proj_out.weight"], device)
        out[f"{key}.proj_out.b"] = _f32(sd[f"{key}.proj_out.bias"], device)
        for i in (1, 2, 3):
            out[f"{key}.ln{i}.g"] = _f32(sd[f"{b}.norm{i}.weight"], device)
            out[f"{key}.ln{i}.b"] = _f32(sd[f"{b}.norm{i}.bias"], device)
        f = lambda k: sd[k].detach().float()
        qkv = [QSCALE * f(f"{b}.attn1.to_q.weight"), f(f"{b}.attn1.to_k.weight"), f(f"{b}.attn1.to_v.weight")]
        q2 = [QSCALE * f(f"{b}.attn2.to_q.weight")]
        for a in ("attn1", "attn2"):
            wo, bo = f(f"{b}.{a}.to_out.0.weight"), f(f"{b}.{a}.to_out.0.bias")
            if adapter:
                pr = f"{b}.{a}.processor"
                out[f"{key}.{a}.out.b0"] = _f32(bo, device)
                wo = torch.cat([wo, ref_scale * f(f"{pr}.to_out_ref.0.weight")], dim=1)
                bo = bo + ref_scale * f(f"{pr}.to_out_ref.0.bias")
            out[f"{key}.{a}.out.w"] = _bf(wo, device)
            out[f"{key}.{a}.out.b"] = _f32(bo, device)
        if adapter:
            p1, p2 = f"{b}.attn1.processor", f"{b}.attn2.processor"
            qkv.append(QSCALE * f(f"{p1}.to_q_ref.weight"))
            q2.append(QSCALE * f(f"{p2}.to_q_ref.weight"))
            out[f"{key}.ref_kv.w"] = _bf(torch.cat([f(f"{p1}.to_k_ref.weight"), f(f"{p1}.to_v_ref.weight"),
                                                    f(f"{p2}.to_k_ref.weight"), f(f"{p2}.to_v_ref.weight")], 0), device)
        out[f"{key}.attn1.qkv.w"] = _bf(torch.cat(qkv, 0), device)
        out[f"{key}.attn2.q.w"] = _bf(torch.cat(q2, 0), device)
        tkv.append(torch.cat([f(f"{b}.attn2.to_k.weight"), f(f"{b}.attn2.to_v.weight")], 0))
        ff1_w, ff1_b = _geglu_rows(f(f"{b}.ff.net.0.proj.weight")), _geglu_rows(f(f"{b}.ff.net.0.proj.bias"))
        out[f"{key}.ff1.w"] = _bf(ff1_w, device)
        out[f"{key}.ff1.b"] = _f32(ff1_b, device)
        if C <= fold_max_c:
            for slot, w, bias, i in ((f"{key}.attn1.qkv", torch.cat(qkv, 0), None, 1), (f"{key}.attn2.q", torch.cat(q2, 0), None, 2),
                                     (f"{key}.ff1", ff1_w, ff1_b, 3)):
                out[f"{slot}.wf"], out[f"{slot}.cf"] = fold_layernorm(w, f(f"{b}.norm{i}.weight"), f(f"{b}.norm{i}.bias"), bias, device)
        if C == XS_K:
            out[f"{key}.proj_in.wx"] = pack_xs(f(f"{key}.proj_in.weight"), f(f"{key}.proj_in.bias"), device=device)
            out[f"{key}.proj_out.wx"] = pack_xs(f(f"{key}.proj_out.weight"), f(f"{key}.proj_out.bias"), device=device)
            for a in ("attn1", "attn2"):
                out[f"{key}.{a}.out.wx"] = pack_xs(f(f"{b}.{a}.to_out.0.weight"), f(f"{b}.{a}.to_out.0.bias"), device=device)
            if adapter:
                out[f"{key}.ref_kv.wx"] = pack_xs(out[f"{key}.ref_kv.w"].float(), None, device=device)
            for slot, geglu in ((f"{key}.attn1.qkv", False), (f"{key}.attn2.q", False), (f"{key}.ff1", True)):
                wf, cf = out[f"{slot}.wf"].float(), out[f"{slot}.cf"]
                if geglu:
                    inv = torch.argsort(_geglu_rows(torch.arange(wf.shape[0], device=wf.device)))
                    wf, cf = wf[inv], cf[:, inv]
                out[f"{slot}.wx"] = pack_xs(wf, cf[1], geglu=geglu, device=device)
        out[f"{key}.ff2.w"] = _bf(sd[f"{b}.ff.net.2.weight"], device)
        out[f"{key}.ff2.b"] = _f32(sd[f"{b}.ff.net.2.bias"], device)

    out["text_kv.w"] = _bf(torch.cat(tkv, 0), device)
    n = cfg.num_levels
    for i in range(n - 1):
        out[f"down_blocks.{i}.down.w"] = _bf(_conv_w(sd[f"down_blocks.{i}.downsamplers.0.conv.weight"]), device)
        out[f"down_blocks.{i}.down.b"] = _f32(sd[f"down_blocks.{i}.downsamplers.0.conv.bias"], device)
        out[f"up_blocks.{i}.up.w"] = _bf(_conv_w(sd[f"up_blocks.{i}.upsamplers.0.conv.weight"]), device)
        wu = sd[f"up_blocks.{i}.upsamplers.0.conv.weight"]
        if small_batch_twins and wu.shape[0] > cfg.block_out_channels[0] and wu.shape[0] % 128 == 0 and wu.shape[1] % 128 == 0:
            out[f"up_blocks.{i}.up.ws"] = pack_ws(wu, None, device)
        out[f"up_blocks.{i}.up.b"] = _f32(sd[f"up_blocks.{i}.upsamplers.0.conv.bias"], device)
    out["conv_norm_out.g"] = _f32(sd["conv_norm_out.weight"], device)
    out["conv_norm_out.b"] = _f32(sd["conv_norm_out.bias"], device)
    out["conv_out.w"] = _bf(_conv_w(sd["conv_out.weight"], tap_major=True), device)
    out["conv_out.b"] = _f32(sd["conv_out.bias"], device)
    return out


def pack_camera(sd: Dict[str, torch.Tensor], device, num_levels: int = 4) -> Dict[str, torch.Tensor]:
    out = {f"cam.{k}": _f32(v, device) for k, v in sd.items()}
    names = [f"down_{i}" for i in range(num_levels)] + [f"up_{i}" for i in range(num_levels)] + ["output"]
    keys = [f"modulators.{n}.{j}.{t}" for n in names for j in (0, 1, 3) for t in ("weight", "bias")]
    if all(k in sd for k in keys):
        cat = lambda j, t: torch.cat([sd[f"modulators.{n}.{j}.{t}"].detach().float() for n in names], 0)
        out["cam.modcat.w0"], out["cam.modcat.b0"] = _f32(cat(0, "weight"), device), _f32(cat(0, "bias"), device)
        out["cam.modcat.g1"], out["cam.modcat.be1"] = _f32(cat(1, "weight"), device), _f32(cat(1, "bias"), device)
        out["cam.modcat.w3"], out["cam.modcat.b3"] = _f32(cat(3, "weight"), device), _f32(cat(3, "bias"), device)
    return out
```

Measured before the change: 523.9 forward-passes/s.

## Replace nearest-upsample 3x3 conv with 2x2 sub-pixel phase convolution

Folds the nearest-neighbour 2x upsample into the following 3x3 conv by precomputing four 2x2 phase kernels, so each output parity reads only a 2x2 source window (K=4C instead of 9C). A new AMODE=4 path in the pipelined GEMM kernel loads source pixels directly and scatters outputs to the interleaved parity positions. This cuts the MACs of the up-block convolutions by more than half. It is used only when the bias-only, unsplit, cfg-7 plan applies, and it adds an extra packed weight tensor plus more complex epilogue addressing.

```diff
diff --git a/include/mvd_hip.h b/include/mvd_hip.h
--- a/include/mvd_hip.h
+++ b/include/mvd_hip.h
@@ -102,6 +102,8 @@
 int mvd_op_conv3x3(const void* x, int batch, int in_h, int in_w, int cin, int stride, int upsample, int asym_pad, const void* w,
                    const float* bias, const float* rowvec, int ld_rowvec, const void* res, const void* sc, const void* sc2,
                    int sc_c1, int sc_c2, void* out, int cout, int force_cfg, int splitk, float* splitk_ws, void* stream);
+int mvd_op_conv3x3_up4(const void* x, int batch, int in_h, int in_w, int cin, const void* w4, const float* bias, void* out, int cout,
+                       int force_cfg, void* stream);
 int mvd_op_attention(const void* q, const void* k, const void* v, void* o, int batch, int heads, int nq, int nk, int ldq,
                      int ldk, int ldv, int ldo, float scale, void* stream);
 int64_t mvd_op_attention_split_ws_bytes(int batch, int heads, int nq, int nsplit);
@@ -126,6 +128,7 @@
 int mvd_gemm_num_configs(void);
 int mvd_debug_last_gemm_plan(int* out);
 int mvd_debug_last_attention_plan(int* out);
+long mvd_debug_up4_launches(void);
 int mvd_debug_last_gemm_nowait(void);
 int mvd_debug_pick_splitk(int m, int n, int k, int geglu);
 int mvd_debug_pick_splitk_conv(int m, int n, int k);
diff --git a/mvd_amd/_lib.py b/mvd_amd/_lib.py
--- a/mvd_amd/_lib.py
+++ b/mvd_amd/_lib.py
@@ -98,6 +98,9 @@
                                         C.c_void_p, C.c_int, C.c_void_p]),
     "mvd_gemm_num_configs": (C.c_int, []),
     "mvd_debug_last_gemm_plan": (C.c_int, [C.POINTER(C.c_int)]),
+    "mvd_debug_up4_launches": (C.c_long, []),
+    "mvd_op_conv3x3_up4": (C.c_int, [C.c_void_p, C.c_int, C.c_int, C.c_int, C.c_int, C.c_void_p, C.c_void_p, C.c_void_p, C.c_int, C.c_int,
+                                     C.c_void_p]),
     "mvd_debug_last_gemm_nowait": (C.c_int, []),
     "mvd_debug_last_attention_plan": (C.c_int, [C.POINTER(C.c_int)]),
     "mvd_debug_pick_splitk": (C.c_int, [C.c_int, C.c_int, C.c_int, C.c_int]),
diff --git a/mvd_amd/csrc/engine.hip b/mvd_amd/csrc/engine.hip
--- a/mvd_amd/csrc/engine.hip
+++ b/mvd_amd/csrc/engine.hip
@@ -245,6 +245,15 @@
     static const bool use_sm = MVD_ENV_INT("MVD_GEMM_SM", 1) != 0;
     return use_sm && !(g_debug_flags & 4);
   }
+  void tiled_plan(const MvdGemmArgs& g, int& S, int& fc) {
+    S = mvd_gemm_pick_splitk(g);
+    fc = -1;
+    if (e->dual_now && !e->dual_late && !(g_debug_flags & 32) && !g.geglu && !g.ln_c1 && !g.out_f32 && g.N % 320 == 0 && mvd_gemm_pp_applicable(g)) {
+      const int cfg = mvd_gemm_pick_config(g);
+      const long t7 = (long)((g.M + 255) / 256) * (g.N / 320);
+      if (t7 >= 100) { S = 1; if (cfg != 7) fc = 7; }
+    }
+  }
   int gemm(MvdGemmArgs& g) {
     if (err) return err;
     int sm_tile = 0, sm_ns = 0, sm_S = 1;
@@ -267,13 +276,8 @@
       e->tmp.off = mark;
       return r;
     }
-    int S = mvd_gemm_pick_splitk(g);
-    int fc = -1;
-    if (e->dual_now && !e->dual_late && !(g_debug_flags & 32) && !g.geglu && !g.ln_c1 && !g.out_f32 && g.N % 320 == 0 && mvd_gemm_pp_applicable(g)) {
-      const int cfg = mvd_gemm_pick_config(g);
-      const long t7 = (long)((g.M + 255) / 256) * (g.N / 320);
-      if (t7 >= 100) { S = 1; if (cfg != 7) fc = 7; }
-    }
+    int S = 1, fc = -1;
+    tiled_plan(g, S, fc);
     const size_t mark = e->tmp.off;
     if (S > 1) { g.splitk = S; g.part = talloc<float>((size_t)S * g.M * g.N); } else g.splitk = 1;
     static const bool trace = MVD_ENV_INT("MVD_TRACE_GEMM", 0) != 0;
@@ -392,7 +396,8 @@
   }
 
   int conv3(const Act& x, int stride, int ups, const bf16_t* w, const float* bias, const float* rowvec, int ld_rowvec,
-            const bf16_t* res, const bf16_t* sc0, const bf16_t* sc1, int scc0, int scc1, Act& out, const std::string& ws = std::string()) {
+            const bf16_t* res, const bf16_t* sc0, const bf16_t* sc1, int scc0, int scc1, Act& out, const std::string& ws = std::string(),
+            const std::string& w4 = std::string()) {
     if (!ws.empty() && stride == 1) {
       const int r = try_ws(x, ups, ws, bias, rowvec, ld_rowvec, res, sc0, sc1, scc0, scc1, out);
       if (r) return r < 0 ? r : 0;
@@ -408,6 +413,23 @@
     g.W = w; g.ldw = g.Ktot; g.M = out.rows(); g.N = out.C; g.rows_per_batch = out.hw(); g.outH = out.H; g.outW = out.W;
     g.bias = bias; g.rowvec = rowvec; g.ld_rowvec = ld_rowvec; g.res = res; g.ldres = out.C; g.alpha = 1.f;
     g.out = out.p; g.ldo = out.C;
+    if (!w4.empty() && !dry && !err && ups == 1 && stride == 1 && !sc0 && !res && !rowvec && !(g_debug_flags & 1048576) && has(w4)) {
+      int t_ = 0, n_ = 0, s_ = 1, S = 1, fc = -1;
+      if (!(sm_enabled() && mvd_gemm_sm_plan(g, &t_, &n_, &s_))) {
+        tiled_plan(g, S, fc);
+        MvdGemmArgs u = g;
+        u.splitk = 1;
+        if (S == 1 && (fc >= 0 ? fc : mvd_gemm_pick_config(u)) == 7 && mvd_gemm_pp_applicable(u)) {
+          u.seg[0].ups = 2; u.seg[0].ksize = 4 * x.C; u.Ktot = 4 * x.C; u.ldw = u.Ktot;
+          if (mvd_gemm_pp_up4_applicable(u)) {
+            u.W = WB(w4, (int64_t)4 * out.C * 4 * x.C);
+            if (!u.W) return err;
+            e->prof_M = u.M; e->prof_N = u.N; e->prof_K = u.Ktot; e->prof_tag = 140;
+            return profiled(13, 2.0 * u.M * (double)u.N * u.Ktot, 0.0, [&] { return mvd_launch_gemm(u, s, 7); });
+          }
+        }
+      }
+    }
     return gemm(g);
   }
 
@@ -684,7 +706,7 @@
       }
       if (i + 1 < n) {
         Act u = c.new_act(B, h.H * 2, h.W * 2, co, true);
-        CHECK(c.conv3(h, 1, 1, c.WB(bk + ".up.w", (int64_t)co * 9 * co), c.WF(bk + ".up.b", co), nullptr, 0, nullptr, nullptr, nullptr, 0, 0, u, bk + ".up.ws"));
+        CHECK(c.conv3(h, 1, 1, c.WB(bk + ".up.w", (int64_t)co * 9 * co), c.WF(bk + ".up.b", co), nullptr, 0, nullptr, nullptr, nullptr, 0, 0, u, bk + ".up.ws", bk + ".up.w4"));
         h = u;
       }
       if (o.film) { Act res = h; CHECK(film("up_" + std::to_string(i), h, res)); h = res; }
@@ -1396,6 +1418,18 @@
   return mvd_launch_gemm(g, (hipStream_t)stream, force_cfg);
 }
 
+int mvd_op_conv3x3_up4(const void* x, int batch, int in_h, int in_w, int cin, const void* w4, const float* bias, void* out, int cout,
+                       int force_cfg, void* stream) {
+  if (!x || !w4 || !out || batch <= 0 || in_h <= 0 || in_w <= 0 || cin <= 0 || cout <= 0) { mvd_set_error("mvd_op_conv3x3_up4: bad argument"); return -1; }
+  MvdGemmArgs g; memset(&g, 0, sizeof(g));
+  g.seg[0].p0 = (const bf16_t*)x; g.seg[0].c0 = cin; g.seg[0].mode = MVD_A_CONV3; g.seg[0].ksize = 4 * cin;
+  g.seg[0].inH = in_h; g.seg[0].inW = in_w; g.seg[0].stride = 1; g.seg[0].ups = 2;
+  g.nseg = 1; g.Ktot = 4 * cin; g.W = (const bf16_t*)w4; g.ldw = g.Ktot;
+  g.outH = 2 * in_h; g.outW = 2 * in_w; g.rows_per_batch = g.outH * g.outW; g.M = batch * g.rows_per_batch; g.N = cout;
+  g.bias = bias; g.ldres = cout; g.alpha = 1.f; g.out = out; g.ldo = cout; g.splitk = 1;
+  return mvd_launch_gemm(g, (hipStream_t)stream, force_cfg);
+}
+
 int mvd_op_attention(const void* q, const void* k, const void* v, void* o, int batch, int heads, int nq, int nk, int ldq,
                      int ldk, int ldv, int ldo, float scale, void* stream) {
   MvdAttnArgs a; memset(&a, 0, sizeof(a));
diff --git a/mvd_amd/csrc/gemm.hip b/mvd_amd/csrc/gemm.hip
--- a/mvd_amd/csrc/gemm.hip
+++ b/mvd_amd/csrc/gemm.hip
@@ -507,6 +507,9 @@
   return 0;
 }
 
+std::atomic<long> g_mvd_up4_launches{0};
+extern "C" long mvd_debug_up4_launches(void) { return g_mvd_up4_launches.load(); }
+
 extern "C" int mvd_debug_last_gemm_nowait(void) { return g_mvd_last_gemm.nowait; }
 
 static int deep_conv_split(const MvdGemmArgs& a, long t7) {
@@ -554,7 +557,8 @@
     if (g.mode == MVD_A_DENSE) {
       if (g.c0 % 64 || g.c1 % 64 || g.ksize != g.c0 + g.c1 || !g.p0 || (g.c1 && !g.p1)) { mvd_set_error("gemm: bad dense segment %d (c0=%d c1=%d ksize=%d)", i, g.c0, g.c1, g.ksize); return -1; }
     } else if (g.mode == MVD_A_CONV3) {
-      if (g.c0 % 64 || g.c1 != 0 || g.ksize != 9 * g.c0 || !g.p0 || (g.stride != 1 && g.stride != 2) || (g.ups && g.stride != 1)) { mvd_set_error("gemm: bad conv segment %d", i); return -1; }
+      if (g.ups != 0 && g.ups != 1 && g.ups != 2) { mvd_set_error("gemm: bad conv segment %d (ups=%d)", i, g.ups); return -1; }
+      if (g.c0 % 64 || g.c1 != 0 || g.ksize != (g.ups == 2 ? 4 : 9) * g.c0 || !g.p0 || (g.stride != 1 && g.stride != 2) || (g.ups && g.stride != 1)) { mvd_set_error("gemm: bad conv segment %d", i); return -1; }
       if (g.asym && (g.asym != 1 || g.stride != 2 || (g.inH & 1) || (g.inW & 1))) { mvd_set_error("gemm: bottom/right-only padding needs stride 2 and an even input size"); return -1; }
       const int eh = g.ups ? 2 * g.inH : (g.stride == 2 ? (g.inH + 1) / 2 : g.inH);
       const int ew = g.ups ? 2 * g.inW : (g.stride == 2 ? (g.inW + 1) / 2 : g.inW);
@@ -578,6 +582,15 @@
   static const int dbg = MVD_ENV_INT("MVD_GEMM_DEBUG", 0);
   if (dbg) const_cast<MvdGemmArgs&>(a).dbg = dbg;
 #endif
+  if (a.seg[0].mode == MVD_A_CONV3 && a.seg[0].ups == 2) {
+    if ((force_cfg >= 0 && force_cfg != 7) || (a.dbg & ~32) || !mvd_gemm_pp_up4_applicable(a)) {
+      mvd_set_error("gemm: the 2x2 sub-pixel upsampling convolution does not take this problem (in %dx%d C=%d N=%d cfg=%d): source width a multiple of 16 or 8 (even height), N %% 320 == 0, bias only, unsplit",
+                    a.seg[0].inH, a.seg[0].inW, a.seg[0].c0, a.N, force_cfg);
+      return -1;
+    }
+    g_mvd_last_gemm.cfg = 7; g_mvd_last_gemm.splitk = 1;
+    return mvd_launch_gemm_pp(a, s);
+  }
   int cfg = force_cfg;
   if (cfg >= 1000) { const_cast<MvdGemmArgs&>(a).w_blocked = 1; cfg -= 1000; }
   if (a.w_blocked && cfg < 100) { mvd_set_error("gemm: the blocked weight layout is read by the small-M kernels only"); return -1; }
diff --git a/mvd_amd/csrc/gemm_pp.hip b/mvd_amd/csrc/gemm_pp.hip
--- a/mvd_amd/csrc/gemm_pp.hip
+++ b/mvd_amd/csrc/gemm_pp.hip
@@ -39,6 +39,8 @@
   constexpr bool GEGLU = WM == 4;
   constexpr bool HAS_CONV = AMODE != 0;
   constexpr bool UPS = AMODE == 3;
+  constexpr bool UP4 = AMODE == 4;
+  static_assert(!UP4 || !SPLITK, "the sub-pixel form is unsplit");
   static_assert((WTM * 128) % 2048 == 0 && (WTN % 16) == 0, "fragment rows of a wave share one swizzle pattern");
   extern __shared__ __attribute__((aligned(16))) unsigned char smem[];
   const int tid = threadIdx.x, lane = tid & 63;
@@ -46,14 +48,15 @@
   const int grp = wave >> 2;
   const int wm = wave / WN, wn = wave % WN;
   const int ntn = a.N / BN;
-  const int ntm = (a.M + BM - 1) / BM;
+  const int srcM = UP4 ? a.M >> 2 : a.M;
+  const int ntm = (srcM + BM - 1) / BM;
   const int lrow = tid >> 3;
   const int kc = (tid & 7) ^ ((lrow >> 1) & 7);
   const int w4 = wave & 3;
   const int arow = w4 * 8 + (lane >> 3);
 
   const int S = SPLITK ? a.splitk : 1;
-  const int ntiles = ntn * ntm * S;
+  const int ntiles = ntn * ntm * S * (UP4 ? 4 : 1);
   const int xcd = blockIdx.x & 7, xj = blockIdx.x >> 3;
   const int gx = (gridDim.x >> 3) + ((int)(gridDim.x & 7) > xcd ? 1 : 0);
   const int tq = ntiles >> 3, tr = ntiles & 7;
@@ -75,7 +78,7 @@
 
   const MvdASeg& cs = a.seg[0];
   const MvdASeg& ds = a.seg[AMODE == 2 ? 1 : 0];
-  const int nkt_conv = HAS_CONV ? (9 * cs.c0) / 64 : 0;
+  const int nkt_conv = HAS_CONV ? ((UP4 ? 4 : 9) * cs.c0) / 64 : 0;
   const int nkt = a.Ktot / 64;
   const int conv_c2 = cs.c0 * 2;
   const int conv_rowB = cs.inW * conv_c2;
@@ -83,7 +86,7 @@
   const int limH = conv_ups ? 2 * cs.inH : cs.inH, limW = conv_ups ? 2 * cs.inW : cs.inW;
   const int dc0 = ds.c0, dc1 = LNF ? 0 : ds.c1;
 
-  __amdgpu_buffer_rsrc_t rs_w = __builtin_amdgcn_make_buffer_rsrc(const_cast<bf16_t*>(a.W), 0, (int)((size_t)a.N * a.ldw * 2), 0x00020000);
+  __amdgpu_buffer_rsrc_t rs_w = __builtin_amdgcn_make_buffer_rsrc(const_cast<bf16_t*>(a.W), 0, (int)((size_t)a.N * a.ldw * 2 * (UP4 ? 4 : 1)), 0x00020000);
   __amdgpu_buffer_rsrc_t rs_c = rs_w, rs_d0 = rs_w, rs_d1 = rs_w;
   if (HAS_CONV) {
     const int shift = conv_rowB + conv_c2;
@@ -104,7 +107,28 @@
   auto setup_loader = [&](int work) {
     const int t = S == 1 ? work : work / S;
     tile_mn(t, ld_m0, ld_n0);
-    if (HAS_CONV) {
+    if constexpr (UP4) {
+      const int pr = ntm * BM;
+      const int par = (ld_m0 >= pr ? 1 : 0) + (ld_m0 >= 2 * pr ? 1 : 0) + (ld_m0 >= 3 * pr ? 1 : 0);
+      ld_m0 -= par * pr; ld_n0 += par * a.N;
+      const int py = par >> 1, px = par & 1;
+      const int hw = cs.inH * cs.inW;
+#pragma unroll
+      for (int i = 0; i < A_IT; ++i) {
+        int m = ld_m0 + (2 * grp + (i & 1)) * 64 + arow + (i >> 1) * 32;
+        m = m < srcM ? m : srcM - 1;
+        const int b = m / hw;
+        const int rem = m - b * hw;
+        const int sy = rem / cs.inW, sx = rem - sy * cs.inW;
+        const int wy = sy + py - 1, wx = sx + px - 1;
+        int okm = 0;
+#pragma unroll
+        for (int t = 0; t < 4; ++t)
+          okm |= ((unsigned)(wy + (t >> 1)) < (unsigned)cs.inH && (unsigned)(wx + (t & 1)) < (unsigned)cs.inW) ? (1 << t) : 0;
+        a_yx[i] = okm << 22;
+        a_base[i] = (unsigned)((b * hw + (wy + 1) * cs.inW + (wx + 1)) * conv_c2 + kc * 16);
+      }
+    } else if (HAS_CONV) {
 #pragma unroll
       for (int i = 0; i < A_IT; ++i) {
         int m = ld_m0 + (2 * grp + (i & 1)) * 64 + arow + (i >> 1) * 32;
@@ -128,7 +152,15 @@
 
   auto issue_a = [&](int st, int lk, int i0, int i1) {
     unsigned char* sa = smem + st * STAGE_BYTES + (2 * grp) * 8192 + w4 * 1024;
-    if (HAS_CONV && (AMODE != 2 || lk < nkt_conv)) {
+    if constexpr (UP4) {
+      const int sl = lk >> 2, tap = lk & 3;
+      const unsigned soff = (unsigned)(sl * 128 + (tap >> 1) * conv_rowB + (tap & 1) * conv_c2);
+#pragma unroll
+      for (int i = 0; i < A_IT; ++i) {
+        const bool ok = (a_yx[i] >> (22 + tap)) & 1;
+        if (i >= i0 && i < i1) dma16(rs_c, sa + (i & 1) * 8192 + (i >> 1) * 4096, ok ? a_base[i] : OOB, soff);
+      }
+    } else if (HAS_CONV && (AMODE != 2 || lk < nkt_conv)) {
       const int sl = lk / 9, tap = lk - sl * 9;
 #ifdef PP_ABLATE_A_TAPS
       if (tap != 0) return;
@@ -239,6 +271,12 @@
   const int pair_col = (fq & 1) * 16 + (fq >> 1) * 8;
   auto epilogue = [&](int m0, int n0, int ks) {
     asm volatile("" : "+s"(m0), "+s"(n0));
+    int up_par = 0;
+    if constexpr (UP4) {
+      const int pr = ntm * BM;
+      up_par = (m0 >= pr ? 1 : 0) + (m0 >= 2 * pr ? 1 : 0) + (m0 >= 3 * pr ? 1 : 0);
+      m0 -= up_par * pr;
+    }
     const int row0 = m0 + wm * WTM;
     if (SPLITK) {
       __amdgpu_buffer_rsrc_t rs_p = __builtin_amdgcn_make_buffer_rsrc(a.part + (size_t)ks * a.M * a.N, 0, (int)((size_t)a.M * a.N * 4), 0x00020000);
@@ -256,6 +294,10 @@
       const int el = fresh_lane();
       efr = el & 15; efq = el >> 4;
       vo16 = (efr * a.ldo + (efq & 1) * 16 + (efq >> 1) * 8) * 2; vo8 = (efr * a.ldo + efq * 4) * 2;
+    } else if constexpr (UP4) {
+      const int sh = cs.inW >= 16 ? 4 : 3;
+      const int lr = (fr >> sh) * 2 * a.outW + (fr & ((1 << sh) - 1)) * 2;
+      vo16 = (lr * a.ldo + pair_col) * 2; vo8 = (lr * a.ldo + fq * 4) * 2;
     } else {
       vo16 = (fr * a.ldo + pair_col) * 2; vo8 = (fr * a.ldo + fq * 4) * 2;
     }
@@ -326,7 +368,14 @@
         if (TN & 1) __builtin_amdgcn_raw_buffer_store_b64(one(TN - 1), rs_o, vo8, so + (TN - 1) * 32, 0);
       }
     } else {
-      const bool has_res = a.res != nullptr;
+      const bool has_res = !UP4 && a.res != nullptr;
+      unsigned up_b = 0, up_y = 0, up_x = 0;
+      if constexpr (UP4) {
+        const unsigned hw = (unsigned)(cs.inH * cs.inW);
+        up_b = (unsigned)row0 / hw;
+        const unsigned rem = (unsigned)row0 - up_b * hw;
+        up_y = rem / (unsigned)cs.inW; up_x = rem - up_y * (unsigned)cs.inW;
+      }
       __amdgpu_buffer_rsrc_t rs_r = rs_o;
       if (has_res) rs_r = __builtin_amdgcn_make_buffer_rsrc(const_cast<bf16_t*>(a.res), 0, (int)((size_t)a.M * a.ldres * 2), 0x00020000);
       const int vr16 = (fr * a.ldres + pair_col) * 2, vr8 = (fr * a.ldres + fq * 4) * 2;
@@ -351,7 +400,14 @@
 #pragma unroll
         for (int g = 0; g < RG; ++g) {
           const int i = i0 + g;
-          const int so = ((row0 + i * 16) * a.ldo + n0 + wn * WTN) * 2;
+          int so = ((row0 + i * 16) * a.ldo + n0 + wn * WTN) * 2;
+          if constexpr (UP4) {
+            const int orow = (int)((up_b * 2 * cs.inH + 2 * up_y + (up_par >> 1)) * a.outW + 2 * up_x + (up_par & 1));
+            so = (row0 + i * 16 < srcM ? orow : a.M) * a.ldo * 2 + (n0 + wn * WTN) * 2;
+            up_x += 16;
+            if (up_x >= (unsigned)cs.inW) { up_x = 0; up_y += cs.inW >= 16 ? 1 : 2; }
+            if (up_y >= (unsigned)cs.inH) { up_y = 0; ++up_b; }
+          }
           int mrow = row0 + i * 16 + fr;
           mrow = mrow < a.M ? mrow : a.M - 1;
           const float* rvp = row_rv ? a.rowvec + (size_t)(mrow / a.rows_per_batch) * a.ld_rowvec + n0 + wn * WTN + fq * 4 : nullptr;
@@ -524,11 +580,11 @@
     if (e != hipSuccess) { mvd_set_error("gemm_pp: hipFuncSetAttribute: %s", hipGetErrorString(e)); return -2; }
     init[dev & 15] = true;
   }
-  const int ntm = (a.M + BM - 1) / BM, ntn = a.N / BN;
+  const int ntm = ((AMODE == 4 ? a.M / 4 : a.M) + BM - 1) / BM, ntn = a.N / BN;
   MvdGemmArgs b = a;
   b.walk_cg = SPLITK ? 0 : mvd_gemm_pp_walk(a);
   int grid = 256;
-  const int ntiles = ntm * ntn * (a.splitk > 1 ? a.splitk : 1);
+  const int ntiles = ntm * ntn * (a.splitk > 1 ? a.splitk : 1) * (AMODE == 4 ? 4 : 1);
   if (ntiles < grid) grid = ((ntiles + 7) / 8) * 8;
   g_mvd_last_gemm.tiles = ntiles; g_mvd_last_gemm.grid = grid; g_mvd_last_gemm.per_cu = 1;
   hipLaunchKernelGGL((gemm_pp_kernel<BM, WM, WN, AMODE, SPLITK, LNF>), dim3(grid), dim3(NT), LDS_BYTES, s, b);
@@ -541,6 +597,11 @@
 int launch_pp_mode(const MvdGemmArgs& a, hipStream_t s) {
   const bool sk = a.splitk > 1;
   if (a.seg[0].mode == MVD_A_DENSE) return sk ? launch_pp<BM, WM, WN, 0, true>(a, s) : launch_pp<BM, WM, WN, 0, false>(a, s);
+  if (a.seg[0].ups == 2) {
+    if (!mvd_gemm_pp_up4_applicable(a)) { mvd_set_error("gemm_pp: not a problem of the 2x2 sub-pixel upsampling convolution"); return -1; }
+    g_mvd_up4_launches.fetch_add(1);
+    return launch_pp<BM, WM, WN, 4, false>(a, s);
+  }
   if (a.seg[0].ups) {
     if (a.nseg != 1) { mvd_set_error("gemm_pp: an upsampling convolution takes no shortcut segment"); return -1; }
     return sk ? launch_pp<BM, WM, WN, 3, true>(a, s) : launch_pp<BM, WM, WN, 3, false>(a, s);
@@ -586,6 +647,19 @@
   return true;
 }
 
+bool mvd_gemm_pp_up4_applicable(const MvdGemmArgs& a) {
+  const MvdASeg& g = a.seg[0];
+  if (a.nseg != 1 || g.mode != MVD_A_CONV3 || g.ups != 2 || g.stride != 1 || g.asym || g.c1) return false;
+  if (a.res || a.rowvec || a.splitk > 1 || a.geglu || a.ln_c1 || a.out_f32) return false;
+  if (g.c0 <= 0 || g.c0 % 64 || g.ksize != 4 * g.c0 || a.Ktot != 4 * g.c0 || a.ldw != a.Ktot) return false;
+  if (g.inH <= 0 || g.inW <= 0 || a.outH != 2 * g.inH || a.outW != 2 * g.inW || a.rows_per_batch != a.outH * a.outW || a.M % a.rows_per_batch) return false;
+  if (!(g.inW % 16 == 0 || (g.inW == 8 && g.inH % 2 == 0))) return false;
+  const size_t lim = (size_t)1 << 31;
+  if ((size_t)4 * a.N * a.ldw * 2 >= lim) return false;
+  if ((size_t)(a.M + 2 * a.outW + 16 + 256) * a.ldo * 2 >= lim) return false;
+  return mvd_gemm_pp_applicable(a);
+}
+
 int mvd_launch_gemm_pp(const MvdGemmArgs& a, hipStream_t s) {
   if (a.ln_c1) {
     const MvdASeg& g = a.seg[0];
diff --git a/mvd_amd/csrc/kernels.h b/mvd_amd/csrc/kernels.h
--- a/mvd_amd/csrc/kernels.h
+++ b/mvd_amd/csrc/kernels.h
@@ -1,6 +1,7 @@
 #pragma once
 #include <hip/hip_runtime.h>
 #include <stdint.h>
+#include <atomic>
 #include "common.h"
 
 enum { MVD_A_DENSE = 0, MVD_A_CONV3 = 1 };
@@ -50,7 +51,9 @@
 int mvd_gemm_pick_config(const MvdGemmArgs& a);
 struct MvdLaunchPlan { int cfg, splitk, tiles, grid, per_cu, nowait; };
 extern thread_local MvdLaunchPlan g_mvd_last_gemm;
+extern std::atomic<long> g_mvd_up4_launches;
 bool mvd_gemm_pp_applicable(const MvdGemmArgs& a);
+bool mvd_gemm_pp_up4_applicable(const MvdGemmArgs& a);
 int mvd_gemm_pp_walk(const MvdGemmArgs& a);
 int mvd_debug_flags();
 bool mvd_gemm_ln_fold_ok(const MvdGemmArgs& a);
diff --git a/mvd_amd/ops.py b/mvd_amd/ops.py
--- a/mvd_amd/ops.py
+++ b/mvd_amd/ops.py
@@ -95,6 +95,20 @@
     return out
 
 
+def conv3x3_up4(x, w4, bias=None, force_cfg=-1):
+    _bf16(x, w4)
+    B, H, W, Cin = x.shape
+    assert w4.dim() == 3 and w4.shape[0] == 4 and w4.shape[2] == 4 * Cin and w4.is_contiguous() and x.is_contiguous(), tuple(w4.shape)
+    cout = w4.shape[1]
+    out = torch.empty(B, 2 * H, 2 * W, cout, device=x.device, dtype=torch.bfloat16)
+    L.call("mvd_op_conv3x3_up4", _p(x), B, H, W, Cin, _p(w4), _p(bias), _p(out), cout, force_cfg, _s())
+    return out
+
+
+def up4_launches() -> int:
+    return int(L.lib().mvd_debug_up4_launches())
+
+
 def attention(q, k, v, heads, scale=0.125):
     _bf16(q, k, v)
     B, nq, _ = q.shape
diff --git a/mvd_amd/packing.py b/mvd_amd/packing.py
--- a/mvd_amd/packing.py
+++ b/mvd_amd/packing.py
@@ -94,6 +94,25 @@
         u = wsc.reshape(n // 16, 16, sc // 128, 4, 4, 8)
         parts.append(u.permute(0, 2, 3, 4, 1, 5).reshape(n // 16, -1))
     return torch.cat(parts, 1).to(torch.bfloat16).contiguous().reshape(-1)
+
+
+def up4_weights(w: torch.Tensor) -> torch.Tensor:
+    assert w.dim() == 4 and tuple(w.shape[2:]) == (3, 3), tuple(w.shape)
+    w = w.detach()
+    if w.dtype not in (torch.float32, torch.float64):
+        w = w.float()
+    r = torch.tensor([[[1, 0, 0], [0, 1, 1]], [[1, 1, 0], [0, 0, 1]]], dtype=w.dtype, device=w.device)
+    w4 = torch.einsum("pty,qsx,oiyx->pqoits", r, r, w)
+    return w4.reshape(4, w.shape[0], w.shape[1], 2, 2)
+
+
+def pack_up4(w: torch.Tensor, device=None) -> torch.Tensor:
+    device = device if device is not None else w.device
+    w4 = up4_weights(w.detach().to(device=device, dtype=torch.float32))
+    co, ci = w4.shape[1], w4.shape[2]
+    assert ci % 64 == 0, ci
+    k = w4.reshape(4, co, ci // 64, 64, 2, 2).permute(0, 1, 2, 4, 5, 3).reshape(4, co, 4 * ci)
+    return k.to(torch.bfloat16).contiguous()
 
 
 LN_FOLD_MAX_C = 1 << 30
@@ -219,6 +238,8 @@
         wu = sd[f"up_blocks.{i}.upsamplers.0.conv.weight"]
         if small_batch_twins and wu.shape[0] > cfg.block_out_channels[0] and wu.shape[0] % 128 == 0 and wu.shape[1] % 128 == 0:
             out[f"up_blocks.{i}.up.ws"] = pack_ws(wu, None, device)
+        if wu.shape[1] % 64 == 0:
+            out[f"up_blocks.{i}.up.w4"] = pack_up4(wu, device)
         out[f"up_blocks.{i}.up.b"] = _f32(sd[f"up_blocks.{i}.upsamplers.0.conv.bias"], device)
     out["conv_norm_out.g"] = _f32(sd["conv_norm_out.weight"], device)
     out["conv_norm_out.b"] = _f32(sd["conv_norm_out.bias"], device)
```

Measured after the change: 538.6 forward-passes/s, median of 6. +2.8%, better.
